# KTH-RPL/HiMo

Hardware: AMD Instinct MI355X
Metric: lidar_frames_per_sec_120k (higher is better)
Workload: dtype f16x2 (two-term split fp16, x = h + l with exact subnormals, on the matrix cores; float32 accumulate; ~22-bit products); 1 GPU; per-frame pipeline: pillarise 3 sweeps (512x512 grid) -> SeFlow++-style encoder/decoder + GRU head (random-init, self-specified: reference network source absent) -> per-point flow -> ego-motion removal + dt0 + flow2compDis -> comp_dis; points_per_frame=120000, sweeps_per_frame=3, parallelism=frames sharded x1, refined_output=False, batches_in_flight=3, matrix_arithmetic=f16x2, samples_per_backbone_launch=16, collectives=none (single process)

## Files before the change

himo_amd/csrc/conv_common.h:

```cpp
#pragma once
#include "himo_common.h"
#include "bf16x3.h"
#include <math.h>

namespace himo {

typedef float floatx16 __attribute__((ext_vector_type(16)));

enum Epilogue {
    kEpiBias = 0,
    kEpiBiasBnGelu = 1,
    kEpiBiasGelu = 2,
    kEpiGruZR = 3,
    kEpiGruQ = 4,
    kEpiBiasRelu = 5,
    kEpiReluMask = 6
};

struct ConvArgs {
    const float* x; int64_t x_batch_stride; int x_pitch;
    const float* w;
    const float* bias; const float* scale; const float* shift;
    float* y; int64_t y_batch_stride; int y_pitch;
    int N, H, W, Cin, Cout;
    int n_inner; int64_t x_outer_stride, y_outer_stride;
    int Ho, Wo;
    const float* aux_in; int aux_in_pitch;
    float* aux_out; int aux_out_pitch;
    int act_flags;
    unsigned* range_seen;
};
enum ActFlags { kActSplitIn = 1, kActSplitOut = 2, kActVecStore = 4, kActAccumulate = 8, kActStuffedIn = 16 };

__device__ inline int64_t image_offset(int img, int n_inner, int64_t batch_stride, int64_t outer_stride) {
    return (int64_t)(img % n_inner) * batch_stride + (int64_t)(img / n_inner) * outer_stride;
}

__device__ inline int xcd_block_id(int bid, int n_blocks) {
    const int per = n_blocks >> 3, rem = n_blocks & 7;
    const int xcd = bid & 7, idx = bid >> 3;
    return xcd * per + (xcd < rem ? xcd : rem) + idx;
}

__device__ inline float gelu_exact(float v) {
    const float hv = 0.5f * v;
    const float t = __builtin_amdgcn_rcpf(fmaf(0.3275911f * 0.70710678118654752440f, fabsf(v), 1.0f));
    float p = fmaf(1.061405429f, t, -1.453152027f);
    p = fmaf(p, t, 1.421413741f);
    p = fmaf(p, t, -0.284496736f);
    p = fmaf(p, t, 0.254829592f);
    const float ex = __builtin_amdgcn_exp2f((v * v) * (-0.5f * 1.44269504088896340736f));
    const float e = fmaf(-(p * t), ex, 1.0f);
    return fmaf(fabsf(hv), e, hv);
}
__device__ inline float gelu_grad_exact(float v) {
    const float t = __builtin_amdgcn_rcpf(fmaf(0.3275911f * 0.70710678118654752440f, fabsf(v), 1.0f));
    float p = fmaf(1.061405429f, t, -1.453152027f);
    p = fmaf(p, t, 1.421413741f);
    p = fmaf(p, t, -0.284496736f);
    p = fmaf(p, t, 0.254829592f);
    const float ex = __builtin_amdgcn_exp2f((v * v) * (-0.5f * 1.44269504088896340736f));
    const float e = fmaf(-(p * t), ex, 1.0f);
    return fmaf(v * 0.39894228040143267794f, ex, 0.5f + copysignf(0.5f * e, v));
}
__device__ inline float sigmoid_f(float v) { return __builtin_amdgcn_rcpf(1.0f + __expf(-v)); }
__device__ inline float tanh_f(float v) {
    const float e = __expf(-2.0f * fabsf(v));
    const float t = (1.0f - e) * __builtin_amdgcn_rcpf(1.0f + e);
    return copysignf(t, v);
}


template <int EPI> constexpr bool kEpiAffine = EPI == kEpiBias || EPI == kEpiBiasBnGelu || EPI == kEpiBiasGelu;
template <int EPI>
__device__ inline void epi_affine(float k, float bias, float sc, float sh, float& A, float& B) {
    if (EPI == kEpiBiasBnGelu) { A = k * sc; B = fmaf(bias, sc, sh); } else { A = k; B = bias; }
}
template <int EPI>
__device__ inline float epi_activate(float acc, float A, float B) {
    const float v = fmaf(acc, A, B);
    return EPI == kEpiBias ? v : gelu_exact(v);
}

template <int EPI>
__device__ inline void epilogue_store(const ConvArgs& a, float* __restrict__ yout, int64_t pix, int co, float v, float sc, float sh) {
    if (EPI == kEpiBias) {
        yout[pix * a.y_pitch + co] = v;
    } else if (EPI == kEpiBiasBnGelu) {
        v = v * sc + sh;
        yout[pix * a.y_pitch + co] = gelu_exact(v);
    } else if (EPI == kEpiBiasGelu) {
        yout[pix * a.y_pitch + co] = gelu_exact(v);
    } else if (EPI == kEpiGruZR) {
        const int half = a.Cout / 2;
        const float g = sigmoid_f(v);
        if (co < half) yout[pix * a.y_pitch + co] = g;
        else a.aux_out[pix * a.aux_out_pitch + (co - half)] = g * a.aux_in[pix * a.aux_in_pitch + (co - half)];
    } else if (EPI == kEpiBiasRelu) {
        yout[pix * a.y_pitch + co] = fmaxf(v, 0.f);
    } else if (EPI == kEpiReluMask) {
        yout[pix * a.y_pitch + co] = a.aux_in[pix * a.aux_in_pitch + co] > 0.f ? v : 0.f;
    } else if (EPI == kEpiGruQ) {
        const float q = tanh_f(v);
        const float z = a.aux_in[pix * a.aux_in_pitch + co];
        const float h = a.aux_out[pix * a.aux_out_pitch + co];
        a.aux_out[pix * a.aux_out_pitch + co] = (1.0f - z) * h + z * q;
    }
}

__device__ inline unsigned split_word(float v, bool odd);
template <int EPI, bool PAIRED>
__device__ inline void split_store(const ConvArgs& a, float* __restrict__ yout, int64_t pix, int co, float v, float sc, float sh) {
    if (EPI == kEpiBiasBnGelu) v = gelu_exact(v * sc + sh);
    else if (EPI == kEpiBiasGelu) v = gelu_exact(v);
    else if (EPI == kEpiBiasRelu) v = fmaxf(v, 0.f);
    if (PAIRED) {
        const bool odd = co & 1;
        unsigned* rec = reinterpret_cast<unsigned*>(yout + pix * a.y_pitch + (co & ~15));
        rec[(odd ? 8 : 0) + ((co & 15) >> 1)] = split_word(v, odd);
        return;
    }
    unsigned h, l;
    split2_rounded(v, h, l);
    {
        unsigned short* rec = reinterpret_cast<unsigned short*>(yout + pix * a.y_pitch + (co & ~15));
        rec[co & 15] = (unsigned short)h;
        rec[16 + (co & 15)] = (unsigned short)l;
    }
}

constexpr float kSplitRangeGuard = 0.015625f;
__device__ inline void note_range(const ConvArgs& a, float v) {
    if (a.range_seen && __ballot(fabsf(v) >= kSplitRangeGuard) != 0ull && (threadIdx.x & 63) == 0 &&
        __hip_atomic_load(a.range_seen, __ATOMIC_RELAXED, __HIP_MEMORY_SCOPE_AGENT) == 0u)
        __hip_atomic_store(a.range_seen, 1u, __ATOMIC_RELAXED, __HIP_MEMORY_SCOPE_AGENT);
}

inline bool vec_store_ok(const ConvArgs& a) {
    return (reinterpret_cast<uintptr_t>(a.y) & 15u) == 0 && !(a.y_pitch & 3) && !(a.y_batch_stride & 3) && !(a.y_outer_stride & 3) && !(a.Cout & 3) &&
           (int64_t)a.Ho * a.Wo * a.y_pitch < ((int64_t)1 << 29);
}

template <bool OSPLIT, bool MASK = false, bool ACC = false>
__device__ inline void store_block_vec(const ConvArgs& a, float* __restrict__ yout, unsigned char* stg, const unsigned (&word)[16],
                                       int lane, int64_t pix0, int n_valid_px, int ch0) {
    const int li = lane & 31, lh = lane >> 5;
    const int widx = OSPLIT ? (li >> 4) * 16 + ((li & 1) ? 8 : 0) + ((li & 15) >> 1) : li;
#pragma unroll
    for (int r = 0; r < 16; ++r) {
        const int px = (r & 3) + 8 * (r >> 2) + 4 * lh;
        const int slot = px ^ ((px >> 2) & 1);
        *reinterpret_cast<unsigned*>(stg + slot * 128 + widx * 4) = word[r];
    }
    __builtin_amdgcn_wave_barrier();
#pragma unroll
    for (int t = 0; t < 4; ++t) {
        const int q = t * 64 + lane;
        const int slot = q >> 3, piece = q & 7;
        const int px = slot ^ ((slot >> 2) & 1);
        uint4 d = *reinterpret_cast<const uint4*>(stg + q * 16);
        const int ch = ch0 + (OSPLIT ? (piece >> 2) * 16 : piece * 4);
        if (px < n_valid_px && ch < a.Cout) {
            if (MASK) {
                const float4 m = *reinterpret_cast<const float4*>(a.aux_in + (pix0 + px) * (int64_t)a.aux_in_pitch + ch0 + piece * 4);
                d.x = m.x > 0.f ? d.x : 0u; d.y = m.y > 0.f ? d.y : 0u; d.z = m.z > 0.f ? d.z : 0u; d.w = m.w > 0.f ? d.w : 0u;
            }
            float* dst = yout + (((unsigned)pix0 + (unsigned)px) * (unsigned)a.y_pitch + (unsigned)(ch0 + piece * 4));
            if (ACC) {
                const float4 o = *reinterpret_cast<const float4*>(dst);
                d.x = __builtin_bit_cast(unsigned, o.x + __builtin_bit_cast(float, d.x)); d.y = __builtin_bit_cast(unsigned, o.y + __builtin_bit_cast(float, d.y));
                d.z = __builtin_bit_cast(unsigned, o.z + __builtin_bit_cast(float, d.z)); d.w = __builtin_bit_cast(unsigned, o.w + __builtin_bit_cast(float, d.w));
            }
            *reinterpret_cast<uint4*>(dst) = d;
        }
    }
    __builtin_amdgcn_wave_barrier();
}

template <int EPI>
__device__ inline float epilogue_value(float v, float sc, float sh) {
    if (EPI == kEpiBiasBnGelu) return gelu_exact(v * sc + sh);
    if (EPI == kEpiBiasGelu) return gelu_exact(v);
    if (EPI == kEpiBiasRelu) return fmaxf(v, 0.f);
    return v;
}
__device__ inline unsigned split_word(float v, bool odd) {
    const unsigned p = split2_packed(v);
    const unsigned q = (unsigned)__builtin_amdgcn_mov_dpp((int)p, 0xB1, 0xF, 0xF, true);
    return __builtin_amdgcn_perm(q, p, odd ? 0x03020706u : 0x05040100u);
}

}
```

himo_amd/csrc/conv_plan.h:

```cpp
#pragma once
#include "conv_common.h"

namespace himo {

enum ConvFamily {
    kConvF32,
    kConvStaged,
    kConvFromL2,
    kConvPresplit3,
    kConvPresplit1
};

struct ConvPlan {
    ConvFamily family;
    ConvArgs args;
    int ks, stride, epi, fmt;
    int bn, mi, ph, nt;
    const void* w_packed;
    dim3 grid;
    const char* prof_name;
};

void launch_conv_f32(const ConvPlan& p, hipStream_t s);
void launch_conv_staged(const ConvPlan& p, hipStream_t s);
void launch_conv_from_l2(const ConvPlan& p, hipStream_t s);
void launch_conv_presplit3(const ConvPlan& p, hipStream_t s);
void launch_conv_presplit1(const ConvPlan& p, hipStream_t s);

inline int64_t blocks_for(const ConvArgs& a, int th, int tw, int bn) {
    const int64_t tiles = th ? (int64_t)((a.Ho + th - 1) / th) * ((a.Wo + tw - 1) / tw) : ((int64_t)a.Ho * a.Wo + tw - 1) / tw;
    return (int64_t)a.N * tiles * ((a.Cout + bn - 1) / bn);
}

inline bool below_2gb(int64_t pixels, int pitch) { return pixels * pitch * 4 < ((int64_t)1 << 31); }

inline const char* conv_prof_name(int ks, int stride, int fmt) {
    static const char* const names[3][4] = {
        {"conv1x1_mfma_kernel", "conv1x1_bf16x3_kernel", "conv1x1_f16x2_kernel", "conv1x1_bf16x2_kernel"},
        {"conv3x3_mfma_kernel", "conv3x3_bf16x3_kernel", "conv3x3_f16x2_kernel", "conv3x3_bf16x2_kernel"},
        {"conv3x3s2_mfma_kernel", "conv3x3s2_bf16x3_kernel", "conv3x3s2_f16x2_kernel", "conv3x3s2_bf16x2_kernel"}};
    return names[ks == 1 ? 0 : stride == 2 ? 2 : 1][fmt < 0 ? 0 : fmt == 1 ? 2 : fmt == 2 ? 3 : 1];
}

inline void plan_staged_tile(ConvPlan& p, int rows_per_mi, int tw, bool keep128, int hint) {
    const ConvArgs& a = p.args;
    auto blocks = [&](int bn, int mi) { return p.ks == 1 ? blocks_for(a, 0, 64 * mi, bn) : blocks_for(a, rows_per_mi * mi, tw, bn); };
    const bool can128 = a.Cout >= 128 && (a.Cout % 128) == 0;
    int bn = can128 ? 128 : 64, mi = 2;
    if (blocks(bn, mi) < 512) mi = 1;
    if (blocks(bn, mi) < 512 && bn == 128 && !keep128) bn = 64;
    const int hb = hint >> 4, hm = hint & 15;
    if ((hb == 64 || (hb == 128 && can128)) && (hm == 1 || hm == 2)) { bn = hb; mi = hm; }
    p.bn = bn; p.mi = mi;
    p.grid = dim3((unsigned)blocks(bn, mi));
}

inline void plan_rows_tile(ConvPlan& p, int ph, int mi, int nt) {
    p.ph = ph; p.mi = mi; p.nt = nt; p.bn = (4 / ph) * 32 * nt;
    p.grid = dim3((unsigned)(p.ks == 1 ? blocks_for(p.args, 0, mi * ph * 32, p.bn) : blocks_for(p.args, mi * ph, 32, p.bn)));
}

inline bool plan_from_l2(ConvPlan& p, int rows_hint) {
    ConvArgs& a = p.args;
    const bool vec = vec_store_ok(a);
    if (p.epi == kEpiGruZR || p.epi == kEpiGruQ) return false;
    if (p.fmt == 2 && (p.epi != kEpiBias || (a.act_flags & ~(kActAccumulate | kActStuffedIn)))) return false;
    if ((a.act_flags & kActAccumulate) && (p.fmt != 2 || !vec)) return false;
    if ((a.act_flags & kActStuffedIn) && (p.fmt != 2 || p.stride != 1)) return false;
    if (!below_2gb((int64_t)a.H * a.W, a.x_pitch)) return false;
    const bool ph_ok = p.stride == 1 && p.fmt != 0;
    const int ph_hint = (ph_ok && (rows_hint == 5 || rows_hint == 6)) ? 2 : (ph_ok && (rows_hint == 9 || rows_hint == 10)) ? 4 : 0;
    if (!ph_hint && rows_hint > 4) return false;
    const bool wide = a.Cout > 64 && ph_hint == 0;
    const int ph = ph_hint ? ph_hint : (wide ? 1 : 2);
    int mi = blocks_for(a, 4 * ph, 32, (4 / ph) * 32) >= 1024 ? 4 : 2;
    if (rows_hint == 4 || rows_hint == 2 || rows_hint == 1) mi = rows_hint;
    if (ph_hint) mi = rows_hint & 3;
    if (p.stride == 2) mi = (rows_hint == 1 || rows_hint == 2) ? rows_hint : (wide ? 2 : 1);
    p.family = kConvFromL2;
    plan_rows_tile(p, ph, mi, 1);
    p.prof_name = conv_prof_name(3, p.stride, p.fmt);
    if (vec && (!(a.act_flags & kActSplitOut) || !(a.Cout & 15))) a.act_flags |= kActVecStore;
    return true;
}

inline int plan_presplit(ConvPlan& p, int rows_hint) {
    ConvArgs& a = p.args;
    if (!below_2gb((int64_t)a.H * a.W, a.x_pitch)) return HIMO_ERR_UNSUPPORTED;
    const bool wide = a.Cout > 64, vec = vec_store_ok(a), pinned = rows_hint == 4 || rows_hint == 2 || rows_hint == 1;
    const int ph = wide ? 1 : 2;
    p.family = p.ks == 1 ? kConvPresplit1 : kConvPresplit3;
    p.prof_name = conv_prof_name(p.ks, p.stride, 1);
    if (vec) a.act_flags |= kActVecStore;
    if (p.ks == 1) {
        int mi = wide ? 4 : 2;
        while (mi > 1 && blocks_for(a, 0, mi * ph * 32, (4 / ph) * 32) < 2048) mi >>= 1;
        if (pinned) mi = rows_hint;
        plan_rows_tile(p, ph, !wide && mi == 4 ? 2 : mi, 1);
    } else if (p.stride == 2) {
        plan_rows_tile(p, ph, wide ? 2 : 1, 1);
    } else if (!wide && rows_hint == 8 && vec) {
        plan_rows_tile(p, 4, 2, 2);
    } else if (wide && rows_hint == 12 && vec) {
        plan_rows_tile(p, a.Cout % 256 == 0 ? 1 : 2, 4, 2);
    } else {
        int mi = blocks_for(a, 4 * ph, 32, (4 / ph) * 32) >= 1024 ? 4 : 2;
        if (pinned) mi = rows_hint;
        plan_rows_tile(p, ph, !wide && mi == 4 ? 2 : mi, 1);
    }
    return HIMO_OK;
}

inline int plan_conv(const himo_conv_desc& d, ConvPlan& p) {
    if (!d.x || !d.w || !d.y) return HIMO_ERR_INVALID_ARGUMENT;
    if (d.n < 1 || d.h < 1 || d.w_in < 1 || d.cin < 1 || d.cout < 1) return HIMO_ERR_INVALID_ARGUMENT;
    if (!(d.ksize == 1 || d.ksize == 3) || !(d.stride == 1 || d.stride == 2)) return HIMO_ERR_UNSUPPORTED;
    if (d.ksize == 1 && d.stride != 1) return HIMO_ERR_UNSUPPORTED;
    if (d.epilogue < 0 || d.epilogue > kEpiReluMask) return HIMO_ERR_INVALID_ARGUMENT;
    if (d.epilogue == kEpiBiasBnGelu && (!d.scale || !d.shift)) return HIMO_ERR_INVALID_ARGUMENT;
    const bool gru = d.epilogue == kEpiGruZR || d.epilogue == kEpiGruQ;
    if (gru && (!d.aux_in || !d.aux_out)) return HIMO_ERR_INVALID_ARGUMENT;
    if (d.epilogue == kEpiReluMask && !d.aux_in) return HIMO_ERR_INVALID_ARGUMENT;
    if ((d.cin & 3) || (d.cout & 3) || (d.x_pitch & 3) || (d.x_batch_stride & 3) || !aligned16(d.x) || !aligned16(d.w))
        return HIMO_ERR_UNSUPPORTED;
    const int n_outer = d.n_outer > 1 ? d.n_outer : 1;
    if (n_outer > 1 && ((d.x_outer_stride & 3) || (d.y_outer_stride & 3))) return HIMO_ERR_INVALID_ARGUMENT;
    p = ConvPlan{};
    p.ks = d.ksize; p.stride = d.stride; p.epi = d.epilogue; p.fmt = d.packed_format; p.w_packed = d.w_packed;
    ConvArgs& a = p.args;
    a.x = d.x; a.x_batch_stride = d.x_batch_stride; a.x_pitch = d.x_pitch;
    a.w = d.w; a.bias = d.bias; a.scale = d.scale; a.shift = d.shift;
    a.y = d.y; a.y_batch_stride = d.y_batch_stride; a.y_pitch = d.y_pitch;
    a.N = d.n * n_outer; a.n_inner = d.n; a.x_outer_stride = d.x_outer_stride; a.y_outer_stride = d.y_outer_stride;
    a.H = d.h; a.W = d.w_in; a.Cin = d.cin; a.Cout = d.cout;
    a.Ho = d.stride == 2 ? (d.h + 1) / 2 : d.h;
    a.Wo = d.stride == 2 ? (d.w_in + 1) / 2 : d.w_in;
    a.aux_in = d.aux_in; a.aux_in_pitch = d.aux_in_pitch; a.aux_out = d.aux_out; a.aux_out_pitch = d.aux_out_pitch;
    a.act_flags = d.act_layout;
    a.range_seen = (d.act_layout & kActSplitOut) ? d.d_range_seen : nullptr;

    const bool gemm_acc = d.act_layout == kActAccumulate && d.w_packed && d.ksize == 1 && d.epilogue == kEpiBias && (d.packed_format == 0 || d.packed_format == 2);
    if (d.act_layout & (kActAccumulate | kActStuffedIn)) {
        if (!gemm_acc && ((d.act_layout & ~(kActAccumulate | kActStuffedIn)) || !d.w_packed || d.packed_format != 2 || d.ksize != 3 ||
                          d.stride != 1 || d.epilogue != kEpiBias))
            return HIMO_ERR_UNSUPPORTED;
        if ((d.act_layout & kActStuffedIn) && ((d.h & 1) || (d.w_in & 1) || !below_2gb((int64_t)(d.h / 2) * (d.w_in / 2), d.x_pitch)))
            return HIMO_ERR_UNSUPPORTED;
    } else if (d.act_layout) {
        if ((d.act_layout & ~(kActSplitIn | kActSplitOut)) || !d.w_packed || d.packed_format != 1) return HIMO_ERR_UNSUPPORTED;
        if (d.ksize == 1 && !(d.act_layout & kActSplitIn)) return HIMO_ERR_UNSUPPORTED;
        if (d.epilogue != kEpiBias && d.epilogue != kEpiBiasBnGelu) return HIMO_ERR_UNSUPPORTED;
        if (((d.act_layout & kActSplitIn) && ((d.cin & 15) || (d.x_pitch & 15))) ||
            ((d.act_layout & kActSplitOut) && ((d.cout & 15) || (d.y_pitch & 15))))
            return HIMO_ERR_UNSUPPORTED;
    }

    const int hint = d.tile_hint, rows_hint = hint & 15;
    const bool l2_hint = hint == 0 || (hint & 0x1000);
    if (!d.w_packed || (d.stride == 2 && (gru || !l2_hint))) {
        p.family = kConvF32;
        plan_staged_tile(p, 4, 16, d.epilogue == kEpiGruZR, hint);
        p.prof_name = conv_prof_name(d.ksize, d.stride, -1);
        if (d.ksize == 1 && vec_store_ok(a) && !(a.Cout & 31) && (d.epilogue != kEpiReluMask || (aligned16(a.aux_in) && !(a.aux_in_pitch & 3))))
            a.act_flags |= kActVecStore;
        return HIMO_OK;
    }
    if (a.act_flags & kActSplitIn) return plan_presplit(p, rows_hint);
    const bool gemm_accumulate = gemm_acc && (int64_t)a.Ho * a.Wo * a.y_pitch < (1ll << 30);
    const bool from_l2 = d.ksize == 3 && l2_hint;
    if (a.act_flags && !gemm_accumulate && !from_l2) return HIMO_ERR_UNSUPPORTED;
    if (from_l2 && plan_from_l2(p, rows_hint)) return HIMO_OK;
    if (d.ksize == 3 && (hint & 0x1000) && rows_hint > 4) return HIMO_ERR_UNSUPPORTED;
    if (d.stride != 1) return HIMO_ERR_UNSUPPORTED;
    if (!below_2gb((int64_t)a.H * a.W, a.x_pitch)) return HIMO_ERR_UNSUPPORTED;
    if (d.packed_format == 2 && (d.ksize != 1 || (d.epilogue != kEpiBias && d.epilogue != kEpiReluMask) || (a.act_flags && !gemm_accumulate)))
        return HIMO_ERR_UNSUPPORTED;
    p.family = kConvStaged;
    plan_staged_tile(p, 2, 32, false, hint);
    p.prof_name = conv_prof_name(d.ksize, 1, d.packed_format);
    return HIMO_OK;
}

}
```

himo_amd/csrc/convsg.hip:

```cpp
#include "conv_plan.h"
#include "bf16x3.h"

namespace himo {

__device__ __attribute__((aligned(64))) unsigned char g_zero_page[64];


__device__ inline void glds16(const void* gsrc, unsigned lds_dst) {
    unsigned keep;
    asm volatile("s_mov_b32 %0, m0\n\ts_mov_b32 m0, %2\n\ts_nop 0\n\tglobal_load_lds_dwordx4 %1, off\n\ts_mov_b32 m0, %0"
                 : "=&s"(keep) : "v"(gsrc), "s"(lds_dst) : "memory");
}

template <int EPI, int PH, int MI, bool OSPLIT, int S, int NT = 1>
__global__ __launch_bounds__(256, NT == 2 ? (MI == 2 ? 3 : 2) : (S == 2 || MI == 4) ? 3 : 4)
void conv3_presplit_kernel(ConvArgs a, const unsigned short* __restrict__ wpk) {
    constexpr int TW = 32, TH = MI * PH, PHt = S == 1 ? TH + 2 : 2 * TH + 1, PWP = S == 1 ? 40 : 80, UPR = PWP / 16;
    constexpr int kRow = PWP * 64, kBuf = (PHt * kRow + 1023) / 1024 * 1024;
    constexpr int kUnits = S == 1 ? (PHt * PWP + 15) / 16 : PHt * UPR, kUPW = (kUnits + 3) / 4;
    constexpr int BN = (4 / PH) * 32 * NT;
    __shared__ __attribute__((aligned(1024))) unsigned char patch[2 * kBuf];

    const int n_tiles_n = (a.Cout + BN - 1) / BN;
    int bid = xcd_block_id(blockIdx.x, gridDim.x);
    const int tn = bid % n_tiles_n; bid /= n_tiles_n;
    const int tx = (a.Wo + TW - 1) / TW, ty = (a.Ho + TH - 1) / TH;
    const int ox0 = (bid % tx) * TW; bid /= tx;
    const int oy0 = (bid % ty) * TH;
    const int img = bid / ty;
    const unsigned char* __restrict__ xin = reinterpret_cast<const unsigned char*>(a.x + image_offset(img, a.n_inner, a.x_batch_stride, a.x_outer_stride));
    const int slabs = a.Cin >> 4;

    const int wave = __builtin_amdgcn_readfirstlane(threadIdx.x >> 6), lane = threadIdx.x & 63;
    const int wp = wave % PH, wc = wave / PH;
    const int li = lane & 31, lh = lane >> 5;
    const int co = tn * BN + wc * NT * 32 + li;
    const bool co_ok = co < a.Cout;
    const int iy0 = oy0 * S - 1, ix0 = ox0 * S - 1;
    const unsigned lds_base = (unsigned)(uintptr_t)(__attribute__((address_space(3))) unsigned char*)(&patch[0]);

    int src[kUPW];
#pragma unroll
    for (int k = 0; k < kUPW; ++k) {
        const int u = wave + 4 * k;
        const int q = u * 16 + (lane >> 2);
        const int row = S == 1 ? q / PWP : u / UPR, px = S == 1 ? q - row * PWP : (u % UPR) * 16 + (lane >> 2);
        const int col = S == 1 ? px : px < 48 ? 2 * px : 2 * (px - 48) + 1;
        const int iy = iy0 + row, ix = ix0 + col;
        const bool ok = u < kUnits && row < PHt && (S == 1 ? px < TW + 2 : px <= 32 || px >= 48) && iy >= 0 && iy < a.H && ix >= 0 && ix < a.W;
        const int sl = (lane & 3) ^ ((px >> 2) & 3);
        src[k] = ok ? (int)((((int64_t)iy * a.W + ix) * a.x_pitch) * 4 + sl * 16) : -1;
    }
    const unsigned char* zero = g_zero_page + (lane & 3) * 16;
    auto stage = [&](int slab, int buf) {
#pragma unroll
        for (int k = 0; k < kUPW; ++k) {
            const int u = wave + 4 * k;
            if (u < kUnits)
                glds16(src[k] >= 0 ? xin + (unsigned)(src[k] + slab * 64) : zero,
                       lds_base + buf * kBuf + (S == 1 ? u * 1024 : ((u / UPR) * PWP + (u % UPR) * 16) * 64));
        }
    };

    floatx16 acc[MI][NT];
#pragma unroll
    for (int mi = 0; mi < MI; ++mi)
#pragma unroll
        for (int nt = 0; nt < NT; ++nt)
#pragma unroll
            for (int r = 0; r < 16; ++r) acc[mi][nt][r] = 0.f;

    const unsigned char* __restrict__ wb = reinterpret_cast<const unsigned char*>(wpk);
    unsigned b_lane[NT];
#pragma unroll
    for (int nt = 0; nt < NT; ++nt) {
        const int c = co + nt * 32 < a.Cout ? co + nt * 32 : a.Cout - 1;
        b_lane[nt] = (unsigned)c * 32u + (unsigned)lh * 16u;
    }
    const unsigned b_plane = (unsigned)a.Cout * 32u, b_block = 2u * b_plane;
    auto load_b = [&](int tap, int slab, uint4 (&b)[NT][2]) {
#pragma unroll
        for (int nt = 0; nt < NT; ++nt) {
            const unsigned off = (unsigned)(tap * slabs + slab) * b_block + b_lane[nt];
            b[nt][0] = *reinterpret_cast<const uint4*>(wb + off);
            b[nt][1] = *reinterpret_cast<const uint4*>(wb + (off + b_plane));
        }
    };

    int rd[3][2];
#pragma unroll
    for (int kx = 0; kx < 3; ++kx) {
        const int p = S == 1 ? li + kx : (kx & 1) * 48 + li + (kx >> 1), f = (p >> 2) & 3;
#pragma unroll
        for (int s = 0; s < 2; ++s) rd[kx][s] = wp * MI * S * kRow + p * 64 + (((2 * s + lh) ^ f) << 4);
    }

    uint4 bq[3][NT][2];
    stage(0, 0);
    load_b(0, 0, bq[0]);
    load_b(1, 0, bq[1]);
    asm volatile("s_waitcnt vmcnt(0)" ::: "memory");
    __syncthreads();

#pragma unroll 1
    for (int slab = 0; slab < slabs; ++slab) {
        const int buf = slab & 1;
        const bool more = slab + 1 < slabs;
        const int nslab = more ? slab + 1 : slab;
        if (more) stage(slab + 1, buf ^ 1);
#pragma unroll 1
        for (int ky = 0; ky < 3; ++ky) {
            const int rowoff = buf * kBuf + ky * kRow;
#pragma unroll
            for (int kx = 0; kx < 3; ++kx) {
                const int tap = ky * 3 + kx;
                const int t2 = tap + 2;
                load_b(t2 < 9 ? t2 : t2 - 9, t2 < 9 ? slab : nslab, bq[(kx + 2) % 3]);
                f16x8 af[MI][2];
#pragma unroll
                for (int s = 0; s < 2; ++s)
#pragma unroll
                    for (int mi = 0; mi < MI; ++mi)
                        af[mi][s] = *reinterpret_cast<const f16x8*>(&patch[rd[kx][s] + rowoff + mi * S * kRow]);
                const uint4 (&bcur)[NT][2] = bq[kx];
#define HIMO_TERM16(SA, SB)                                                                                        \
    _Pragma("unroll") for (int mi = 0; mi < MI; ++mi) _Pragma("unroll") for (int nt = 0; nt < NT; ++nt)              \
        acc[mi][nt] = __builtin_amdgcn_mfma_f32_32x32x16_f16(af[mi][SA], __builtin_bit_cast(f16x8, bcur[nt][SB]), acc[mi][nt], 0, 0, 0);
                { HIMO_TERM16(1, 0) HIMO_TERM16(0, 1) HIMO_TERM16(0, 0) }
#undef HIMO_TERM16
                __builtin_amdgcn_sched_group_barrier(0x020, 2 * NT, 0);
                __builtin_amdgcn_sched_group_barrier(0x100, MI * 2, 0);
                __builtin_amdgcn_sched_group_barrier(0x008, MI * NT * 3, 0);
            }
        }
        if (more) {
            if (NT == 2) asm volatile("s_waitcnt vmcnt(8)" ::: "memory");
            else asm volatile("s_waitcnt vmcnt(4)" ::: "memory");
            __syncthreads();
        }
    }

    float* __restrict__ yout = a.y + image_offset(img, a.n_inner, a.y_batch_stride, a.y_outer_stride);
    float eA[NT], eB[NT];
#pragma unroll
    for (int nt = 0; nt < NT; ++nt) {
        const int c = co + nt * 32 < a.Cout ? co + nt * 32 : a.Cout - 1;
        epi_affine<EPI>(kF16AccScale, a.bias ? a.bias[c] : 0.f, EPI == kEpiBiasBnGelu ? a.scale[c] : 1.f, EPI == kEpiBiasBnGelu ? a.shift[c] : 0.f,
                        eA[nt], eB[nt]);
    }
    if (NT > 1 || (a.act_flags & kActVecStore)) {
        __syncthreads();
        unsigned char* stg = patch + wave * 4096;
        const int n_px = a.Wo - ox0 < 32 ? a.Wo - ox0 : 32;
#pragma unroll
        for (int mi = 0; mi < MI; ++mi) {
            const int oy = oy0 + wp * MI + mi;
#pragma unroll
            for (int nt = 0; nt < NT; ++nt) {
                unsigned word[16];
#pragma unroll
                for (int r = 0; r < 16; ++r) {
                    const float v = epi_activate<EPI>(acc[mi][nt][r], eA[nt], eB[nt]);
                    word[r] = OSPLIT ? split_word(v, li & 1) : __builtin_bit_cast(unsigned, v);
                    if (OSPLIT && mi == 0 && nt == 0 && r == 0)
                        note_range(a, (oy < a.Ho && 4 * lh < n_px && tn * BN + wc * NT * 32 + li < a.Cout) ? v : 0.f);
                }
                store_block_vec<OSPLIT>(a, yout, stg, word, lane, (int64_t)oy * a.Wo + ox0, oy < a.Ho ? n_px : 0, tn * BN + (wc * NT + nt) * 32);
            }
        }
        return;
    }
    if (!co_ok) return;
#pragma unroll
    for (int mi = 0; mi < MI; ++mi) {
        const int oy = oy0 + wp * MI + mi;
#pragma unroll
        for (int r = 0; r < 16; ++r) {
            const int ox = ox0 + (r & 3) + 8 * (r >> 2) + 4 * lh;
            if (oy < a.Ho && ox < a.Wo) {
                const float v = epi_activate<EPI>(acc[mi][0][r], eA[0], eB[0]);
                if (OSPLIT) split_store<kEpiBias, true>(a, yout, (int64_t)oy * a.Wo + ox, co, v, 1.f, 0.f);
                else yout[((int64_t)oy * a.Wo + ox) * a.y_pitch + co] = v;
            }
        }
    }
}

template <int EPI, int PH, int MI, bool OSPLIT>
__global__ __launch_bounds__(256, 4)
void conv1_presplit_kernel(ConvArgs a, const unsigned short* __restrict__ wpk) {
    constexpr int G = 2, TH = MI * PH, BM = TH * 32;
    constexpr int kSeg = 32 * 64, kSlab = TH * kSeg, kBuf = G * kSlab;
    constexpr int kUnits = G * TH * 2, kUPW = (kUnits + 3) / 4;
    constexpr int BN = (4 / PH) * 32;
    __shared__ __attribute__((aligned(1024))) unsigned char patch[2 * kBuf < 16384 ? 16384 : 2 * kBuf];

    const int n_tiles_n = (a.Cout + BN - 1) / BN;
    int bid = xcd_block_id(blockIdx.x, gridDim.x);
    const int tn = bid % n_tiles_n; bid /= n_tiles_n;
    const int64_t rows = (int64_t)a.Ho * a.Wo;
    const int tiles = (int)((rows + BM - 1) / BM);
    const int img = bid / tiles;
    const int64_t row0 = (int64_t)(bid % tiles) * BM;
    const unsigned char* __restrict__ xin = reinterpret_cast<const unsigned char*>(a.x + image_offset(img, a.n_inner, a.x_batch_stride, a.x_outer_stride));
    const int slabs = a.Cin >> 4, steps = (slabs + G - 1) / G;

    const int wave = __builtin_amdgcn_readfirstlane(threadIdx.x >> 6), lane = threadIdx.x & 63;
    const int wp = wave % PH, wc = wave / PH;
    const int li = lane & 31, lh = lane >> 5;
    const int co = tn * BN + wc * 32 + li;
    const bool co_ok = co < a.Cout;
    const unsigned lds_base = (unsigned)(uintptr_t)(__attribute__((address_space(3))) unsigned char*)(&patch[0]);

    int src[kUPW];
#pragma unroll
    for (int k = 0; k < kUPW; ++k) {
        const int u = wave + 4 * k;
        const int g = u / (2 * TH), seg = (u >> 1) % TH, px = (u & 1) * 16 + (lane >> 2);
        const int64_t pix = row0 + seg * 32 + px;
        const int sl = (lane & 3) ^ ((px >> 2) & 3);
        src[k] = (u < kUnits && pix < rows) ? (int)(pix * a.x_pitch * 4 + sl * 16 + g * 64) : -1;
    }
    const unsigned char* zero = g_zero_page + (lane & 3) * 16;
    auto stage = [&](int step, int buf) {
#pragma unroll
        for (int k = 0; k < kUPW; ++k) {
            const int u = wave + 4 * k;
            if (u < kUnits) {
                const int g = u / (2 * TH);
                const bool ok = src[k] >= 0 && step * G + g < slabs;
                glds16(ok ? xin + (unsigned)(src[k] + step * (G * 64)) : zero, lds_base + buf * kBuf + g * kSlab + ((u >> 1) % TH) * kSeg + (u & 1) * 1024);
            }
        }
    };

    floatx16 acc[MI];
#pragma unroll
    for (int mi = 0; mi < MI; ++mi)
#pragma unroll
        for (int r = 0; r < 16; ++r) acc[mi][r] = 0.f;

    const int co_ld = co_ok ? co : a.Cout - 1;
    const unsigned char* __restrict__ wb = reinterpret_cast<const unsigned char*>(wpk);
    const unsigned b_lane = (unsigned)co_ld * 32u + (unsigned)lh * 16u, b_plane = (unsigned)a.Cout * 32u;
    auto load_b = [&](int slab, uint4 (&b)[2]) {
        const unsigned off = (unsigned)slab * (2u * b_plane) + b_lane;
        b[0] = *reinterpret_cast<const uint4*>(wb + off);
        b[1] = *reinterpret_cast<const uint4*>(wb + (off + b_plane));
    };
    int rd[2];
#pragma unroll
    for (int s = 0; s < 2; ++s) rd[s] = wp * MI * kSeg + li * 64 + (((2 * s + lh) ^ ((li >> 2) & 3)) << 4);

    uint4 bq[2][2];
    stage(0, 0);
    load_b(0, bq[0]);
    asm volatile("s_waitcnt vmcnt(0)" ::: "memory");
    __syncthreads();

#pragma unroll 1
    for (int step = 0; step < steps; ++step) {
        const int buf = step & 1;
        const bool more = step + 1 < steps;
        if (more) stage(step + 1, buf ^ 1);
#pragma unroll
        for (int g = 0; g < G; ++g) {
            const int nslab = step * G + g + 1;
            load_b(nslab < slabs ? nslab : slabs - 1, bq[(g + 1) & 1]);
            f16x8 af[MI][2];
#pragma unroll
            for (int s = 0; s < 2; ++s)
#pragma unroll
                for (int mi = 0; mi < MI; ++mi)
                    af[mi][s] = *reinterpret_cast<const f16x8*>(&patch[rd[s] + buf * kBuf + g * kSlab + mi * kSeg]);
            const uint4 (&bcur)[2] = bq[g & 1];
#define HIMO_TERM16(SA, SB)                                                                                        \
    _Pragma("unroll") for (int mi = 0; mi < MI; ++mi)                                                                \
        acc[mi] = __builtin_amdgcn_mfma_f32_32x32x16_f16(af[mi][SA], __builtin_bit_cast(f16x8, bcur[SB]), acc[mi], 0, 0, 0);
            HIMO_TERM16(1, 0) HIMO_TERM16(0, 1) HIMO_TERM16(0, 0)
#undef HIMO_TERM16
        }
        if (more) {
            asm volatile("s_waitcnt vmcnt(2)" ::: "memory");
            __syncthreads();
        }
    }

    float* __restrict__ yout = a.y + image_offset(img, a.n_inner, a.y_batch_stride, a.y_outer_stride);
    float eA, eB;
    epi_affine<EPI>(kF16AccScale, a.bias ? a.bias[co_ld] : 0.f, EPI == kEpiBiasBnGelu ? a.scale[co_ld] : 1.f, EPI == kEpiBiasBnGelu ? a.shift[co_ld] : 0.f, eA, eB);
    if (a.act_flags & kActVecStore) {
        __syncthreads();
        unsigned char* stg = patch + wave * 4096;
#pragma unroll
        for (int mi = 0; mi < MI; ++mi) {
            const int64_t pix0 = row0 + (wp * MI + mi) * 32;
            const int64_t left = rows - pix0;
            unsigned word[16];
#pragma unroll
            for (int r = 0; r < 16; ++r) {
                const float v = epi_activate<EPI>(acc[mi][r], eA, eB);
                word[r] = OSPLIT ? split_word(v, li & 1) : __builtin_bit_cast(unsigned, v);
                if (OSPLIT && mi == 0 && r == 0) note_range(a, (4 * lh < left && tn * BN + wc * 32 + li < a.Cout) ? v : 0.f);
            }
            store_block_vec<OSPLIT>(a, yout, stg, word, lane, pix0, left < 0 ? 0 : left > 32 ? 32 : (int)left, tn * BN + wc * 32);
        }
        return;
    }
    if (!co_ok) return;
#pragma unroll
    for (int mi = 0; mi < MI; ++mi) {
#pragma unroll
        for (int r = 0; r < 16; ++r) {
            const int64_t pix = row0 + (wp * MI + mi) * 32 + (r & 3) + 8 * (r >> 2) + 4 * lh;
            if (pix < rows) {
                const float v = epi_activate<EPI>(acc[mi][r], eA, eB);
                if (OSPLIT) split_store<kEpiBias, true>(a, yout, pix, co, v, 1.f, 0.f);
                else yout[pix * a.y_pitch + co] = v;
            }
        }
    }
}

#define HIMO_SG(KERNEL, E, O, ...) hipLaunchKernelGGL((KERNEL<E, PH, MI, O, ##__VA_ARGS__>), p.grid, dim3(256), 0, s, p.args, (const unsigned short*)p.w_packed)
#define HIMO_SG_EPI(KERNEL, ...)                                                                                                          \
    do {                                                                                                                                  \
        const bool osplit = (p.args.act_flags & kActSplitOut) != 0;                                                                       \
        if (p.epi == kEpiBias) { if (osplit) HIMO_SG(KERNEL, kEpiBias, true, ##__VA_ARGS__); else HIMO_SG(KERNEL, kEpiBias, false, ##__VA_ARGS__); } \
        else { if (osplit) HIMO_SG(KERNEL, kEpiBiasBnGelu, true, ##__VA_ARGS__); else HIMO_SG(KERNEL, kEpiBiasBnGelu, false, ##__VA_ARGS__); }       \
    } while (0)

template <int PH, int MI>
static void launch_sg1(const ConvPlan& p, hipStream_t s) { HIMO_SG_EPI(conv1_presplit_kernel); }

template <int PH, int MI, int S = 1, int NT = 1>
static void launch_sg(const ConvPlan& p, hipStream_t s) { HIMO_SG_EPI(conv3_presplit_kernel, S, NT); }
#undef HIMO_SG_EPI
#undef HIMO_SG

void launch_conv_presplit1(const ConvPlan& p, hipStream_t s) {
    if (p.ph == 1) {
        if (p.mi == 4) launch_sg1<1, 4>(p, s);
        else if (p.mi == 2) launch_sg1<1, 2>(p, s);
        else launch_sg1<1, 1>(p, s);
    } else {
        if (p.mi == 2) launch_sg1<2, 2>(p, s);
        else launch_sg1<2, 1>(p, s);
    }
}

void launch_conv_presplit3(const ConvPlan& p, hipStream_t s) {
    if (p.stride == 2) { if (p.ph == 1) launch_sg<1, 2, 2>(p, s); else launch_sg<2, 1, 2>(p, s); }
    else if (p.nt == 2) {
        if (p.ph == 4) launch_sg<4, 2, 1, 2>(p, s);
        else if (p.ph == 1) launch_sg<1, 4, 1, 2>(p, s);
        else launch_sg<2, 4, 1, 2>(p, s);
    }
    else if (p.ph == 1) {
        if (p.mi == 4) launch_sg<1, 4>(p, s);
        else if (p.mi == 2) launch_sg<1, 2>(p, s);
        else launch_sg<1, 1>(p, s);
    } else {
        if (p.mi == 2) launch_sg<2, 2>(p, s);
        else launch_sg<2, 1>(p, s);
    }
}

}
```

himo_amd/csrc/pillar.hip:

```cpp
#include "himo_common.h"
#include "bf16x3.h"
#include <math.h>
#include <algorithm>
#include <vector>

namespace himo {

struct GridSpec {
    float xmin, ymin, zmin;
    float vx, vy, vz;
    float cx0, cy0, cz0;
    int W, H;
};

struct PillarArgs {
    int64_t n;
    const float* pts; int stride;
    float R[9], t[3];
    GridSpec g;
    const float* pfn_w;
    const float* pfn_scale;
    const float* pfn_shift;
    float* xyz_t;
    int* pid;
    float* offsets;
    float* image; int image_pitch;
    int image_split;
    int* cell_count;
    int* block_sum;
    int* cell_cursor;
    int* order2;
    float4* cell_rec;
    unsigned long long* occ;
};

constexpr int kMaxSweeps = 12;
struct PillarBatch { PillarArgs s[kMaxSweeps]; };

__global__ __launch_bounds__(256) void pillar_clear_kernel(PillarBatch m, int n_vec4) {
    int4* p = reinterpret_cast<int4*>(m.s[blockIdx.y].cell_count);
    for (int i = blockIdx.x * 256 + threadIdx.x; i < n_vec4; i += gridDim.x * 256) p[i] = make_int4(0, 0, 0, 0);
}

__global__ __launch_bounds__(256) void pillar_assign_kernel(PillarBatch m) {
    const PillarArgs& a = m.s[blockIdx.y];
    const int64_t i = (int64_t)blockIdx.x * 256 + threadIdx.x;
    if (i >= a.n) return;
    const float* p = a.pts + i * a.stride;
    const float x = p[0], y = p[1], z = p[2];
    const float tx = ((x * a.R[0] + y * a.R[1]) + z * a.R[2]) + a.t[0];
    const float ty = ((x * a.R[3] + y * a.R[4]) + z * a.R[5]) + a.t[1];
    const float tz = ((x * a.R[6] + y * a.R[7]) + z * a.R[8]) + a.t[2];
    a.xyz_t[i * 3] = tx; a.xyz_t[i * 3 + 1] = ty; a.xyz_t[i * 3 + 2] = tz;
    const float fx = floorf((tx - a.g.xmin) / a.g.vx);
    const float fy = floorf((ty - a.g.ymin) / a.g.vy);
    const float fz = floorf((tz - a.g.zmin) / a.g.vz);
    const bool ok = fx >= 0.f && fx < (float)a.g.W && fy >= 0.f && fy < (float)a.g.H && fz >= 0.f && fz < 1.f;
    int cell = -1;
    if (ok) {
        cell = (int)fy * a.g.W + (int)fx;
        a.order2[i] = atomicAdd(&a.cell_count[cell], 1);
    } else {
        a.offsets[i * 3] = 0.f; a.offsets[i * 3 + 1] = 0.f; a.offsets[i * 3 + 2] = 0.f;
    }
    a.pid[i] = cell;
}

constexpr int kScanBlock = 1024;

__global__ __launch_bounds__(256) void cell_scan_local_kernel(PillarBatch m) {
    int* v = m.s[blockIdx.y].cell_count;
    int* block_sum = m.s[blockIdx.y].block_sum;
    const int n = m.s[blockIdx.y].g.W * m.s[blockIdx.y].g.H;
    __shared__ int wsum[4];
    const int base = blockIdx.x * kScanBlock + threadIdx.x * 4;
    int x[4];
#pragma unroll
    for (int k = 0; k < 4; ++k) x[k] = base + k < n ? v[base + k] : 0;
    const int mine = x[0] + x[1] + x[2] + x[3];
    int incl = mine;
    const int lane = threadIdx.x & 63;
    for (int off = 1; off < 64; off <<= 1) {
        const int y = __shfl_up(incl, off, 64);
        if (lane >= off) incl += y;
    }
    if (lane == 63) wsum[threadIdx.x >> 6] = incl;
    __syncthreads();
    int run = incl - mine;
    for (int w = 0; w < (int)(threadIdx.x >> 6); ++w) run += wsum[w];
#pragma unroll
    for (int k = 0; k < 4; ++k) { if (base + k < n) v[base + k] = run; run += x[k]; }
    if (threadIdx.x == 255) block_sum[blockIdx.x] = run;
}

__global__ __launch_bounds__(1024) void cell_scan_top_kernel(PillarBatch m, int nblk) {
    int* block_sum = m.s[blockIdx.y].block_sum;
    __shared__ int part[1024];
    const int x = (int)threadIdx.x < nblk ? block_sum[threadIdx.x] : 0;
    part[threadIdx.x] = x;
    __syncthreads();
    for (int off = 1; off < 1024; off <<= 1) {
        const int y = threadIdx.x >= off ? part[threadIdx.x - off] : 0;
        __syncthreads();
        part[threadIdx.x] += y;
        __syncthreads();
    }
    if ((int)threadIdx.x < nblk) block_sum[threadIdx.x] = part[threadIdx.x] - x;
    if (threadIdx.x == 1023) block_sum[nblk] = part[1023];
}

__device__ inline int cell_offset(const PillarArgs& a, int cell);

__device__ inline int cell_offset(const PillarArgs& a, int cell) {
    const int n_cells = a.g.W * a.g.H;
    return cell >= n_cells ? a.block_sum[(n_cells + kScanBlock - 1) / kScanBlock]
                           : a.cell_count[cell] + a.block_sum[cell / kScanBlock];
}

__global__ __launch_bounds__(256) void pillar_fill_kernel(PillarBatch m) {
    const PillarArgs& a = m.s[blockIdx.y];
    const int64_t i = (int64_t)blockIdx.x * 256 + threadIdx.x;
    if (i >= a.n) return;
    const int cell = a.pid[i];
    if (cell < 0) return;
    const int at = cell_offset(a, cell) + a.order2[i];
    a.cell_rec[at] = make_float4(a.xyz_t[i * 3], a.xyz_t[i * 3 + 1], a.xyz_t[i * 3 + 2], __int_as_float((int)i));
}

constexpr int kCellsPerBlock = 8;

constexpr int kFeatCells = 64;

__device__ inline float shfl32(float v, int src) { return __shfl(v, src, 32); }
__device__ inline int shfl32(int v, int src) { return __shfl(v, src, 32); }

__global__ __launch_bounds__(256) void pillar_feature_kernel(PillarBatch m) {
    const PillarArgs& a = m.s[blockIdx.y];
    __shared__ int s_beg[kFeatCells + 1];
    __shared__ int s_list[kFeatCells];
    __shared__ int s_nlist;
    const int sub = threadIdx.x >> 5, c = threadIdx.x & 31;
    const int n_cells = a.g.W * a.g.H;
    const int cell0 = blockIdx.x * kFeatCells;
    static_assert(kFeatCells == 64, "one 64-bit occupancy word per block");
    const unsigned long long was = a.occ ? a.occ[blockIdx.x] : ~0ull;
    if (threadIdx.x <= kFeatCells) s_beg[threadIdx.x] = cell_offset(a, min(cell0 + (int)threadIdx.x, n_cells));
    __syncthreads();
    if (threadIdx.x < 64) {
        const int cnt = cell0 + (int)threadIdx.x < n_cells ? s_beg[threadIdx.x + 1] - s_beg[threadIdx.x] : 0;
        const unsigned long long one = __ballot(cnt == 1), many = __ballot(cnt > 1);
        const unsigned long long below = (1ull << threadIdx.x) - 1ull;
        if (cnt == 1) s_list[__popcll(one & below)] = threadIdx.x;
        if (cnt > 1) s_list[__popcll(one) + __popcll(many & below)] = threadIdx.x;
        if (threadIdx.x == 0) { s_nlist = __popcll(one | many); if (a.occ) a.occ[blockIdx.x] = one | many; }
    }
#pragma unroll
    for (int i = 0; i < kFeatCells / 32; ++i) {
        const int lc = i * 32 + (threadIdx.x >> 3);
        if (cell0 + lc < n_cells && s_beg[lc + 1] == s_beg[lc] && ((was >> lc) & 1ull))
            *reinterpret_cast<float4*>(a.image + (int64_t)(cell0 + lc) * a.image_pitch + (threadIdx.x & 7) * 4) = make_float4(0.f, 0.f, 0.f, 0.f);
    }
    __syncthreads();
    const int nlist = s_nlist;
    float w[9];
#pragma unroll
    for (int k = 0; k < 9; ++k) w[k] = a.pfn_w[k * 32 + c];
    const float scale = a.pfn_scale[c], shift = a.pfn_shift[c];

    for (int k = sub; k < nlist; k += kCellsPerBlock) {
        const int lc = s_list[k];
        const int cell = cell0 + lc;
        const int beg = s_beg[lc];
        const int cnt = s_beg[lc + 1] - beg;
        const int iy = cell / a.g.W, ix = cell - iy * a.g.W;
        const float ccx = (float)ix * a.g.vx + a.g.cx0, ccy = (float)iy * a.g.vy + a.g.cy0, ccz = 0.f * a.g.vz + a.g.cz0;
        const float fc = (float)cnt;
        float acc = 0.f;
        if (cnt == 1) {
            const float4 rc = a.cell_rec[beg];
            const int pj = __float_as_int(rc.w);
            const float x = rc.x, y = rc.y, z = rc.z;
            if (c == 0) a.order2[beg] = pj;
            const float f6[3] = {x - ccx, y - ccy, z - ccz};
            float v = x * w[0];
            v = fmaf(y, w[1], v); v = fmaf(z, w[2], v);
            v = fmaf(x - x, w[3], v); v = fmaf(y - y, w[4], v); v = fmaf(z - z, w[5], v);
            v = fmaf(f6[0], w[6], v); v = fmaf(f6[1], w[7], v); v = fmaf(f6[2], w[8], v);
            v = v * scale + shift;
            acc = 0.f + fmaxf(v, 0.f);
            if (c < 3) a.offsets[(int64_t)pj * 3 + c] = f6[c];
        } else if (cnt <= 32) {
            const bool have = c < cnt;
            const float4 rc = a.cell_rec[beg + (have ? c : 0)];
            const int idx = have ? __float_as_int(rc.w) : 0x7fffffff;
            const float ux = rc.x, uy = rc.y, uz = rc.z;
            int rank = 0;
            for (int j = 0; j < cnt; ++j) rank += shfl32(idx, j) < idx;
            int src = 0;
            for (int j = 0; j < cnt; ++j)
                if (shfl32(rank, j) == c) src = j;
            const int sidx = shfl32(idx, src);
            const float px = shfl32(ux, src), py = shfl32(uy, src), pz = shfl32(uz, src);
            if (have) a.order2[beg + c] = sidx;
            float sx = 0.f, sy = 0.f, sz = 0.f;
            for (int j = 0; j < cnt; ++j) { sx += shfl32(px, j); sy += shfl32(py, j); sz += shfl32(pz, j); }
            const float mx = sx / fc, my = sy / fc, mz = sz / fc;
            for (int j = 0; j < cnt; ++j) {
                const float x = shfl32(px, j), y = shfl32(py, j), z = shfl32(pz, j);
                const int pj = shfl32(sidx, j);
                const float f[9] = {x, y, z, x - mx, y - my, z - mz, x - ccx, y - ccy, z - ccz};
                float v = f[0] * w[0];
#pragma unroll
                for (int q = 1; q < 9; ++q) v = fmaf(f[q], w[q], v);
                v = v * scale + shift;
                acc += fmaxf(v, 0.f);
                if (c < 3) a.offsets[(int64_t)pj * 3 + c] = f[6 + c];
            }
        } else {
            for (int j0 = 0; j0 < cnt; j0 += 32) {
                const bool have = j0 + c < cnt;
                const int idx = have ? __float_as_int(a.cell_rec[beg + j0 + c].w) : 0x7fffffff;
                int rank = 0;
                for (int k0 = 0; k0 < cnt; k0 += 32) {
                    const int other = k0 + c < cnt ? __float_as_int(a.cell_rec[beg + k0 + c].w) : 0x7fffffff;
                    const int lim = min(32, cnt - k0);
                    for (int j = 0; j < lim; ++j) rank += shfl32(other, j) < idx;
                }
                if (have) a.order2[beg + rank] = idx;
            }
            __threadfence_block();
            float sx = 0.f, sy = 0.f, sz = 0.f;
            for (int j0 = 0; j0 < cnt; j0 += 32) {
                const bool have = j0 + c < cnt;
                const float* p = a.xyz_t + (int64_t)(have ? a.order2[beg + j0 + c] : 0) * 3;
                const float ux = have ? p[0] : 0.f, uy = have ? p[1] : 0.f, uz = have ? p[2] : 0.f;
                const int lim = min(32, cnt - j0);
                for (int j = 0; j < lim; ++j) { sx += shfl32(ux, j); sy += shfl32(uy, j); sz += shfl32(uz, j); }
            }
            const float mx = sx / fc, my = sy / fc, mz = sz / fc;
            for (int j0 = 0; j0 < cnt; j0 += 32) {
                const bool have = j0 + c < cnt;
                const int pidx = have ? a.order2[beg + j0 + c] : 0;
                const float* p = a.xyz_t + (int64_t)pidx * 3;
                const float ux = have ? p[0] : 0.f, uy = have ? p[1] : 0.f, uz = have ? p[2] : 0.f;
                const int lim = min(32, cnt - j0);
                for (int j = 0; j < lim; ++j) {
                    const float x = shfl32(ux, j), y = shfl32(uy, j), z = shfl32(uz, j);
                    const int pj = shfl32(pidx, j);
                    const float f[9] = {x, y, z, x - mx, y - my, z - mz, x - ccx, y - ccy, z - ccz};
                    float v = f[0] * w[0];
#pragma unroll
                    for (int q = 1; q < 9; ++q) v = fmaf(f[q], w[q], v);
                    v = v * scale + shift;
                    acc += fmaxf(v, 0.f);
                    if (c < 3) a.offsets[(int64_t)pj * 3 + c] = f[6 + c];
                }
            }
        }
        const float feat = acc / fc;
        if (a.image_split) {
            unsigned h, l;
            split2_rounded(feat, h, l);
            const bool odd = c & 1;
            const unsigned recv = (unsigned)__builtin_amdgcn_mov_dpp((int)(odd ? h : l), 0xB1, 0xF, 0xF, true);
            unsigned* rec = reinterpret_cast<unsigned*>(a.image + (int64_t)cell * a.image_pitch + (c & ~15));
            rec[(odd ? 8 : 0) + ((c & 15) >> 1)] = odd ? (recv | (l << 16)) : (h | (recv << 16));
        } else {
            a.image[(int64_t)cell * a.image_pitch + c] = feat;
        }
    }
}

struct PillarBwdArgs {
    GridSpec g;
    const int* cell_count; const int* block_sum; const int* order2;
    const float4* cell_rec;
    const float* xyz_t;
    const float* pfn_w; const float* pfn_scale; const float* pfn_shift;
    const float* d_image; int image_pitch;
    float* partial;
    const float* dhx; int dhx_pitch;
    float* d_b0; int b0_pitch; int group0, group1, n_groups;
    float* d_dec; int dec_pitch;
};

__device__ inline int cell_offset_b(const PillarBwdArgs& a, int cell) {
    const int n_cells = a.g.W * a.g.H;
    return cell >= n_cells ? a.block_sum[(n_cells + kScanBlock - 1) / kScanBlock]
                           : a.cell_count[cell] + a.block_sum[cell / kScanBlock];
}

__global__ __launch_bounds__(1024) void pfn_backward_reduce_kernel(const float* __restrict__ partial, int n_blocks, float* __restrict__ dw,
                                                                   int accumulate) {
    __shared__ float sh[32][32];
    const int c = threadIdx.x & 31, grp = threadIdx.x >> 5, k = blockIdx.x;
    {
        float t[4] = {0.f, 0.f, 0.f, 0.f};
        int b = grp;
        for (; b + 96 < n_blocks; b += 128) {
#pragma unroll
            for (int q = 0; q < 4; ++q) t[q] += partial[(int64_t)(b + 32 * q) * 288 + k * 32 + c];
        }
        for (; b < n_blocks; b += 32) t[0] += partial[(int64_t)b * 288 + k * 32 + c];
        sh[grp][c] = (t[0] + t[1]) + (t[2] + t[3]);
    }
    __syncthreads();
    if (grp == 0) {
        float r = sh[0][c];
#pragma unroll
        for (int g = 1; g < 32; ++g) r += sh[g][c];
        dw[k * 32 + c] = accumulate ? dw[k * 32 + c] + r : r;
    }
}

struct PfnBnArgs {
    PillarBwdArgs b;
    double* partial;
    const float* mean; const float* invstd;
    const float* coef;
};

struct PfnBnBatch { PfnBnArgs s[kMaxSweeps]; };
template <int KIND>
__global__ __launch_bounds__(256) void pfn_walk_kernel(PfnBnBatch m) {
    const PfnBnArgs& p = m.s[blockIdx.y];
    const PillarBwdArgs& a = p.b;
    constexpr int kChunk = 256;
    __shared__ int s_beg[kChunk + 1];
    __shared__ int s_list[kChunk];
    __shared__ int s_wn[4];
    constexpr bool kStats = KIND < 2;
    __shared__ double red_d[kStats ? 2 : 1][kStats ? kCellsPerBlock : 1][32];
    __shared__ float red_f[kStats ? 1 : kCellsPerBlock][kStats ? 1 : 9][32];
    const int sub = threadIdx.x >> 5, c = threadIdx.x & 31, wv = threadIdx.x >> 6, lane = threadIdx.x & 63;
    const int n_cells = a.g.W * a.g.H;
    float w[9], dw[9];
#pragma unroll
    for (int k = 0; k < 9; ++k) { w[k] = a.pfn_w[k * 32 + c]; dw[k] = 0.f; }
    const float scale = KIND ? a.pfn_scale[c] : 0.f, shift = KIND ? a.pfn_shift[c] : 0.f;
    const float mean = (KIND == 1 || KIND == 2) ? p.mean[c] : 0.f, invstd = (KIND == 1 || KIND == 2) ? p.invstd[c] : 0.f;
    const float k2 = KIND == 2 ? p.coef[c] : 0.f, k3 = KIND == 2 ? p.coef[32 + c] : 0.f;
    double s0 = 0.0, s1 = 0.0;
    for (int cell0 = blockIdx.x * kChunk; cell0 < n_cells; cell0 += gridDim.x * kChunk) {
        s_beg[threadIdx.x] = cell_offset_b(a, min(cell0 + (int)threadIdx.x, n_cells));
        if (threadIdx.x == 0) s_beg[kChunk] = cell_offset_b(a, min(cell0 + kChunk, n_cells));
        __syncthreads();
        const int my_cnt = cell0 + (int)threadIdx.x < n_cells ? s_beg[threadIdx.x + 1] - s_beg[threadIdx.x] : 0;
        const unsigned long long occ = __ballot(my_cnt > 0);
        if (lane == 0) s_wn[wv] = __popcll(occ);
        __syncthreads();
        int base = 0, nlist = 0;
#pragma unroll
        for (int u = 0; u < 4; ++u) { if (u < wv) base += s_wn[u]; nlist += s_wn[u]; }
        if (my_cnt > 0) s_list[base + __popcll(occ & ((1ull << lane) - 1ull))] = threadIdx.x;
        __syncthreads();
        for (int k = sub; k < nlist; k += kCellsPerBlock) {
            const int lc = s_list[k];
            const int cell = cell0 + lc;
            const int beg = s_beg[lc], cnt = s_beg[lc + 1] - beg;
            const float fc = (float)cnt;
            const float gi = KIND ? a.d_image[(int64_t)cell * a.image_pitch + c] / fc : 0.f;
            const int iy = cell / a.g.W, ix = cell - iy * a.g.W;
            const float ccx = (float)ix * a.g.vx + a.g.cx0, ccy = (float)iy * a.g.vy + a.g.cy0, ccz = 0.f * a.g.vz + a.g.cz0;
            auto point = [&](float x, float y, float z, float mx, float my, float mz) {
                const float f[9] = {x, y, z, x - mx, y - my, z - mz, x - ccx, y - ccy, z - ccz};
                float v = f[0] * w[0];
#pragma unroll
                for (int q = 1; q < 9; ++q) v = fmaf(f[q], w[q], v);
                if (KIND == 0) {
                    s0 += v; s1 += (double)v * v;
                } else if (KIND == 1) {
                    const float g = (v * scale + shift) > 0.f ? gi : 0.f;
                    s0 += g; s1 += (double)g * ((v - mean) * invstd);
                } else if (KIND == 2) {
                    const float g = (v * scale + shift) > 0.f ? gi : 0.f;
                    const float dy = scale * ((g - k2) - ((v - mean) * invstd) * k3);
#pragma unroll
                    for (int q = 0; q < 9; ++q) dw[q] += f[q] * dy;
                } else {
                    if ((v * scale + shift) > 0.f) {
                        const float g = gi * scale;
#pragma unroll
                        for (int q = 0; q < 9; ++q) dw[q] += f[q] * g;
                    }
                }
            };
            if (cnt == 1) {
                const float4 rc = a.cell_rec[beg];
                point(rc.x, rc.y, rc.z, rc.x, rc.y, rc.z);
                continue;
            }
            float sx = 0.f, sy = 0.f, sz = 0.f;
            float ux = 0.f, uy = 0.f, uz = 0.f;
            for (int j0 = 0; j0 < cnt; j0 += 32) {
                const bool have = j0 + c < cnt;
                const float* q = a.xyz_t + (int64_t)(have ? a.order2[beg + j0 + c] : 0) * 3;
                ux = have ? q[0] : 0.f; uy = have ? q[1] : 0.f; uz = have ? q[2] : 0.f;
                const int lim = min(32, cnt - j0);
                for (int j = 0; j < lim; ++j) { sx += shfl32(ux, j); sy += shfl32(uy, j); sz += shfl32(uz, j); }
            }
            const float mx = sx / fc, my = sy / fc, mz = sz / fc;
            for (int j0 = 0; j0 < cnt; j0 += 32) {
                if (cnt > 32) {
                    const bool have = j0 + c < cnt;
                    const float* q = a.xyz_t + (int64_t)(have ? a.order2[beg + j0 + c] : 0) * 3;
                    ux = have ? q[0] : 0.f; uy = have ? q[1] : 0.f; uz = have ? q[2] : 0.f;
                }
                const int lim = min(32, cnt - j0);
                for (int j = 0; j < lim; ++j) point(shfl32(ux, j), shfl32(uy, j), shfl32(uz, j), mx, my, mz);
            }
        }
        __syncthreads();
    }
    if (kStats) {
        red_d[0][sub][c] = s0; red_d[1][sub][c] = s1;
        __syncthreads();
        if (threadIdx.x < 64) {
            const int which = threadIdx.x >> 5;
            double t = red_d[which][0][c];
#pragma unroll
            for (int q = 1; q < kCellsPerBlock; ++q) t += red_d[which][q][c];
            p.partial[((int64_t)blockIdx.x * 2 + which) * 32 + c] = t;
        }
    } else {
#pragma unroll
        for (int k = 0; k < 9; ++k) red_f[sub][k][c] = dw[k];
        __syncthreads();
        for (int e = threadIdx.x; e < 9 * 32; e += 256) {
            float t = 0.f;
#pragma unroll
            for (int q = 0; q < kCellsPerBlock; ++q) t += red_f[q][e / 32][e % 32];
            a.partial[(int64_t)blockIdx.x * 288 + e] = t;
        }
    }
}

constexpr int kMaxGroup = 16;
struct PfnGroup { const double* partial[kMaxGroup]; const int* block_sum[kMaxGroup]; int n; };

template <int MODE>
__global__ __launch_bounds__(1024) void pfn_bn_finalize_kernel(PfnGroup grp_src, int n_blocks, int n_cells, const float* __restrict__ gamma,
                                                              const float* __restrict__ beta, float eps, float momentum,
                                                              float* __restrict__ running_mean, float* __restrict__ running_var,
                                                              float* __restrict__ out0, float* __restrict__ out1, float* __restrict__ out2,
                                                              float* __restrict__ out3, int accumulate) {
    __shared__ double sh[2][16][32];
    const int c = threadIdx.x & 31, which = (threadIdx.x >> 5) & 1, grp = threadIdx.x >> 6;
    {
        double all = 0.0;
        for (int m = 0; m < grp_src.n; ++m) {
            const double* __restrict__ partial = grp_src.partial[m];
            double t[4] = {0, 0, 0, 0};
            int b = grp;
            for (; b + 48 < n_blocks; b += 64) {
#pragma unroll
                for (int k = 0; k < 4; ++k) t[k] += partial[((int64_t)(b + 16 * k) * 2 + which) * 32 + c];
            }
            for (; b < n_blocks; b += 16) t[0] += partial[((int64_t)b * 2 + which) * 32 + c];
            all += (t[0] + t[1]) + (t[2] + t[3]);
        }
        sh[which][grp][c] = all;
    }
    __syncthreads();
    if (threadIdx.x >= 32) return;
    double count = 0.0;
    for (int m = 0; m < grp_src.n; ++m) count += (double)grp_src.block_sum[m][(n_cells + kScanBlock - 1) / kScanBlock];
    double a0 = 0.0, a1 = 0.0;
#pragma unroll
    for (int g = 0; g < 16; ++g) { a0 += sh[0][g][c]; a1 += sh[1][g][c]; }
    if (MODE == 0) {
        if (count < 1.0) {
            const float sc = gamma[c] / sqrtf((running_var ? running_var[c] : 1.f) + eps);
            out0[c] = sc; out1[c] = beta[c] - (running_mean ? running_mean[c] : 0.f) * sc; out2[c] = 0.f; out3[c] = 0.f;
            return;
        }
        const double mean = a0 / count;
        double var = a1 / count - mean * mean;
        if (var < 0.0) var = 0.0;
        const float invstd = (float)(1.0 / sqrt(var + (double)eps));
        const float sc = gamma[c] * invstd;
        out0[c] = sc;
        out1[c] = beta[c] - (float)mean * sc;
        out2[c] = (float)mean;
        out3[c] = invstd;
        if (running_mean) {
            const double unbiased = count > 1.0 ? var * count / (count - 1.0) : var;
            running_mean[c] = (float)((1.0 - (double)momentum) * (double)running_mean[c] + (double)momentum * mean);
            running_var[c] = (float)((1.0 - (double)momentum) * (double)running_var[c] + (double)momentum * unbiased);
        }
    } else {
        out0[c] = accumulate ? out0[c] + (float)a1 : (float)a1;
        out1[c] = accumulate ? out1[c] + (float)a0 : (float)a0;
        out2[c] = count > 0.0 ? (float)(a0 / count) : 0.f;
        out3[c] = count > 0.0 ? (float)(a1 / count) : 0.f;
    }
}

__global__ __launch_bounds__(256) void head_scatter_kernel(PillarBwdArgs a) {
    const int sub = threadIdx.x >> 5, c = threadIdx.x & 31;
    const int cell = blockIdx.x * kCellsPerBlock + sub;
    if (cell >= a.g.W * a.g.H) return;
    const int beg = cell_offset_b(a, cell);
    const int cnt = cell_offset_b(a, cell + 1) - beg;
    float s0 = 0.f, s1 = 0.f, s2 = 0.f, s3 = 0.f;
    for (int j = 0; j < cnt; ++j) {
        const float* r = a.dhx + (int64_t)a.order2[beg + j] * a.dhx_pitch;
        s0 += r[c]; s1 += r[32 + c]; s2 += r[64 + c]; s3 += r[96 + c];
    }
    float* b0 = a.d_b0 + (int64_t)cell * a.b0_pitch;
    for (int g = 0; g < a.n_groups; ++g) b0[g * 32 + c] = g == a.group0 ? s0 : g == a.group1 ? s1 : 0.f;
    float* dec = a.d_dec + (int64_t)cell * a.dec_pitch;
    dec[c] = s2; dec[32 + c] = s3;
}

}

using namespace himo;

static size_t ws_cells(int cells) { return round_up((size_t)cells * 4, 16); }
static size_t ws_blocks(int cells) { return round_up(((size_t)(cells + kScanBlock - 1) / kScanBlock + 1) * 4, 16); }
static size_t ws_points(int64_t n) { return round_up((size_t)(n > 0 ? n : 1) * 4, 16); }
static size_t pillar_ws(int64_t n, int cells) { return 2 * ws_cells(cells) + ws_blocks(cells) + 2 * ws_points(n) + 3 * ws_points(n); }
static size_t ws_occ(int cells) { return round_up(((size_t)cells + 63) / 64 * 8, 16); }

constexpr int64_t kMaxCells = (int64_t)kScanBlock * 1024;
static int64_t grid_cells(int grid_w, int grid_h) { return (int64_t)grid_w * (int64_t)grid_h; }
static int grid_status(int grid_w, int grid_h) {
    if (grid_w < 1 || grid_h < 1) return HIMO_ERR_INVALID_ARGUMENT;
    return grid_cells(grid_w, grid_h) > kMaxCells ? HIMO_ERR_UNSUPPORTED : HIMO_OK;
}

extern "C" size_t himo_pillar_workspace_bytes(int64_t max_points, int grid_w, int grid_h) {
    if (max_points < 0 || max_points > 0x7fffffff || grid_status(grid_w, grid_h) != HIMO_OK) return 0;
    const int cells = (int)grid_cells(grid_w, grid_h);
    return pillar_ws(max_points, cells) + 64 + ws_occ(cells);
}

extern "C" int himo_pillar_occupancy_reset(void* d_workspace, size_t workspace_bytes, int grid_w, int grid_h, void* stream) {
    if (!d_workspace || grid_w < 1 || grid_h < 1) return HIMO_ERR_INVALID_ARGUMENT;
    if (grid_status(grid_w, grid_h) != HIMO_OK) return HIMO_ERR_UNSUPPORTED;
    const int cells = (int)grid_cells(grid_w, grid_h);
    if (workspace_bytes < ws_occ(cells)) return HIMO_ERR_INVALID_ARGUMENT;
    const size_t nb = ws_occ(cells);
    HIMO_HIP(hipMemsetAsync(reinterpret_cast<char*>(d_workspace) + (workspace_bytes - nb), 0xFF, nb, (hipStream_t)stream));
    return HIMO_OK;
}

static int pillar_args(PillarArgs& a, int64_t n, const float* d_pts, int pc_stride, const float* h_transform, const float* h_range,
                       const float* h_voxel, const float* h_centre_offset, int grid_w, int grid_h, const float* d_pfn_weight,
                       const float* d_pfn_scale, const float* d_pfn_shift, float* d_xyz_t, int32_t* d_pid, float* d_offsets,
                       float* d_image, int image_pitch, void* d_workspace, size_t workspace_bytes, bool incremental = false) {
    if (n < 0 || pc_stride < 3 || grid_w < 1 || grid_h < 1 || !h_transform || !h_range || !h_voxel || !h_centre_offset)
        return HIMO_ERR_INVALID_ARGUMENT;
    if (!d_pfn_weight || !d_pfn_scale || !d_pfn_shift || !d_image || !d_workspace) return HIMO_ERR_INVALID_ARGUMENT;
    if (n > 0 && (!d_pts || !d_xyz_t || !d_pid || !d_offsets)) return HIMO_ERR_INVALID_ARGUMENT;
    if (n > 0x7fffffff || image_pitch < 32) return HIMO_ERR_UNSUPPORTED;
    if ((image_pitch & 3) || (reinterpret_cast<uintptr_t>(d_image) & 15)) return HIMO_ERR_UNSUPPORTED;
    if (grid_cells(grid_w, grid_h) > kMaxCells) return HIMO_ERR_UNSUPPORTED;
    const int cells = (int)grid_cells(grid_w, grid_h);
    if (workspace_bytes < pillar_ws(n, cells) || !aligned16(d_workspace)) return HIMO_ERR_WORKSPACE;
    if (incremental && ((workspace_bytes & 15) || workspace_bytes < pillar_ws(n, cells) + ws_occ(cells))) return HIMO_ERR_WORKSPACE;
    a = PillarArgs{};
    a.n = n; a.pts = d_pts; a.stride = pc_stride;
    for (int i = 0; i < 9; ++i) a.R[i] = h_transform[(i / 3) * 4 + (i % 3)];
    for (int i = 0; i < 3; ++i) a.t[i] = h_transform[i * 4 + 3];
    a.g.xmin = h_range[0]; a.g.ymin = h_range[1]; a.g.zmin = h_range[2];
    a.g.vx = h_voxel[0]; a.g.vy = h_voxel[1]; a.g.vz = h_voxel[2];
    a.g.cx0 = h_centre_offset[0]; a.g.cy0 = h_centre_offset[1]; a.g.cz0 = h_centre_offset[2];
    a.g.W = grid_w; a.g.H = grid_h;
    a.pfn_w = d_pfn_weight; a.pfn_scale = d_pfn_scale; a.pfn_shift = d_pfn_shift;
    a.xyz_t = d_xyz_t; a.pid = d_pid; a.offsets = d_offsets; a.image = d_image; a.image_pitch = image_pitch;
    char* ws = reinterpret_cast<char*>(d_workspace);
    a.cell_count = reinterpret_cast<int*>(ws);
    a.cell_cursor = reinterpret_cast<int*>(ws + ws_cells(cells));
    a.block_sum = reinterpret_cast<int*>(ws + 2 * ws_cells(cells));
    a.cell_rec = reinterpret_cast<float4*>(ws + 2 * ws_cells(cells) + ws_blocks(cells));
    a.order2 = reinterpret_cast<int*>(ws + 2 * ws_cells(cells) + ws_blocks(cells) + 4 * ws_points(n));
    if (incremental) a.occ = reinterpret_cast<unsigned long long*>(ws + (workspace_bytes - ws_occ(cells)));
    return HIMO_OK;
}

static int sweeps_status(int n_sweeps, const himo_sweep* h_sweeps, int image_pitch, int image_split, bool check_shared) {
    if (n_sweeps < 1 || n_sweeps > kMaxSweeps || !h_sweeps) return HIMO_ERR_INVALID_ARGUMENT;
    if (image_split && (image_pitch & 15)) return HIMO_ERR_INVALID_ARGUMENT;
    for (int i = 0; i < n_sweeps; ++i) {
        if (image_split && (reinterpret_cast<uintptr_t>(h_sweeps[i].d_image) & 63)) return HIMO_ERR_INVALID_ARGUMENT;
        for (int j = 0; check_shared && j < i; ++j)
            if (h_sweeps[j].d_workspace == h_sweeps[i].d_workspace) return HIMO_ERR_INVALID_ARGUMENT;
    }
    return HIMO_OK;
}

static int pillar_launch(const PillarBatch& m, int count, hipStream_t s) {
    const int cells = m.s[0].g.W * m.s[0].g.H;
    const int nblk = (cells + kScanBlock - 1) / kScanBlock;
    int64_t nmax = 0;
    for (int i = 0; i < count; ++i)
        if (m.s[i].n > nmax) nmax = m.s[i].n;
    {
        const int n_vec4 = (int)(ws_cells(cells) / 16);
        hipLaunchKernelGGL(pillar_clear_kernel, dim3(std::min((n_vec4 + 255) / 256, 512), count), dim3(256), 0, s, m, n_vec4);
    }
    HIMO_LAUNCH_CHECK("pillar_clear_kernel");
    const unsigned pblocks = (unsigned)((nmax + 255) / 256);
    if (nmax > 0) {
        ProfScope ps("pillar_assign_kernel", s);
        hipLaunchKernelGGL(pillar_assign_kernel, dim3(pblocks, count), dim3(256), 0, s, m);
    }
    HIMO_LAUNCH_CHECK("pillar_assign_kernel");
    {
        ProfScope ps("cell_scan_kernels", s);
        hipLaunchKernelGGL(cell_scan_local_kernel, dim3(nblk, count), dim3(256), 0, s, m);
        hipLaunchKernelGGL(cell_scan_top_kernel, dim3(1, count), dim3(1024), 0, s, m, nblk);
    }
    HIMO_LAUNCH_CHECK("cell_scan_kernels");
    if (nmax > 0) {
        ProfScope ps("pillar_fill_kernel", s);
        hipLaunchKernelGGL(pillar_fill_kernel, dim3(pblocks, count), dim3(256), 0, s, m);
    }
    HIMO_LAUNCH_CHECK("pillar_fill_kernel");
    {
        ProfScope ps("pillar_feature_kernel", s);
        hipLaunchKernelGGL(pillar_feature_kernel, dim3((cells + kFeatCells - 1) / kFeatCells, count), dim3(256), 0, s, m);
    }
    HIMO_LAUNCH_CHECK("pillar_feature_kernel");
    return HIMO_OK;
}

extern "C" int himo_pillarize(int64_t n, const float* d_pts, int pc_stride, const float* h_transform,
                              const float* h_range, const float* h_voxel, const float* h_centre_offset,
                              int grid_w, int grid_h,
                              const float* d_pfn_weight, const float* d_pfn_scale, const float* d_pfn_shift,
                              float* d_xyz_t, int32_t* d_pid, float* d_offsets, float* d_image, int image_pitch,
                              void* d_workspace, size_t workspace_bytes, void* stream) {
    PillarBatch m{};
    const int st = pillar_args(m.s[0], n, d_pts, pc_stride, h_transform, h_range, h_voxel, h_centre_offset, grid_w, grid_h, d_pfn_weight,
                               d_pfn_scale, d_pfn_shift, d_xyz_t, d_pid, d_offsets, d_image, image_pitch, d_workspace, workspace_bytes);
    if (st != HIMO_OK) return st;
    return pillar_launch(m, 1, (hipStream_t)stream);
}

extern "C" int himo_pillarize_multi(int n_sweeps, const himo_sweep* h_sweeps, const float* h_range, const float* h_voxel,
                                    const float* h_centre_offset, int grid_w, int grid_h, const float* d_pfn_weight,
                                    const float* d_pfn_scale, const float* d_pfn_shift, int image_pitch, size_t workspace_bytes,
                                    void* stream) {
    return himo_pillarize_multi_ex(n_sweeps, h_sweeps, h_range, h_voxel, h_centre_offset, grid_w, grid_h, d_pfn_weight, d_pfn_scale,
                                   d_pfn_shift, image_pitch, workspace_bytes, 0, stream);
}

extern "C" int himo_pillarize_multi_ex(int n_sweeps, const himo_sweep* h_sweeps, const float* h_range, const float* h_voxel,
                                       const float* h_centre_offset, int grid_w, int grid_h, const float* d_pfn_weight,
                                       const float* d_pfn_scale, const float* d_pfn_shift, int image_pitch, size_t workspace_bytes,
                                       int image_split, void* stream) {
    const bool incremental = (image_split & 2) != 0;
    image_split &= 1;
    const int st0 = sweeps_status(n_sweeps, h_sweeps, image_pitch, image_split, true);
    if (st0 != HIMO_OK) return st0;
    PillarBatch m{};
    for (int i = 0; i < n_sweeps; ++i) {
        const himo_sweep& w = h_sweeps[i];
        const int st = pillar_args(m.s[i], w.n, w.d_pts, w.pc_stride, w.transform, h_range, h_voxel, h_centre_offset, grid_w, grid_h,
                                   d_pfn_weight, d_pfn_scale, d_pfn_shift, w.d_xyz_t, w.d_pid, w.d_offsets, w.d_image, image_pitch,
                                   w.d_workspace, workspace_bytes, incremental);
        if (st != HIMO_OK) return st;
        m.s[i].image_split = image_split ? 1 : 0;
    }
    return pillar_launch(m, n_sweeps, (hipStream_t)stream);
}

static void carve_bwd(PillarBwdArgs& a, int64_t n, int cells, void* d_workspace) {
    char* ws = reinterpret_cast<char*>(d_workspace);
    a.cell_count = reinterpret_cast<const int*>(ws);
    a.block_sum = reinterpret_cast<const int*>(ws + 2 * ws_cells(cells));
    a.cell_rec = reinterpret_cast<const float4*>(ws + 2 * ws_cells(cells) + ws_blocks(cells));
    a.order2 = reinterpret_cast<const int*>(ws + 2 * ws_cells(cells) + ws_blocks(cells) + 4 * ws_points(n));
}

constexpr int kPfnBwdBlocks = 1024;

extern "C" size_t himo_pfn_backward_workspace_bytes(void) { return (size_t)kPfnBwdBlocks * 288 * 4 + 64; }

extern "C" int himo_pfn_backward(int64_t n, const float* h_voxel, const float* h_centre_offset, int grid_w, int grid_h,
                                 const float* d_pfn_weight, const float* d_pfn_scale, const float* d_pfn_shift,
                                 const float* d_xyz_t, const void* d_pillar_workspace, const float* d_dimage, int image_pitch,
                                 float* d_dweight, unsigned flags, void* d_workspace, size_t workspace_bytes, void* stream) {
    if (n < 0 || !h_voxel || !h_centre_offset || grid_w < 1 || grid_h < 1 || !d_pfn_weight || !d_pfn_scale || !d_pfn_shift ||
        !d_pillar_workspace || !d_dimage || !d_dweight || !d_workspace || image_pitch < 32)
        return HIMO_ERR_INVALID_ARGUMENT;
    if (n > 0 && !d_xyz_t) return HIMO_ERR_INVALID_ARGUMENT;
    if (n > 0x7fffffff || grid_status(grid_w, grid_h) != HIMO_OK) return HIMO_ERR_UNSUPPORTED;
    if (workspace_bytes < himo_pfn_backward_workspace_bytes()) return HIMO_ERR_WORKSPACE;
    PillarBwdArgs a{};
    a.g.vx = h_voxel[0]; a.g.vy = h_voxel[1]; a.g.vz = h_voxel[2];
    a.g.cx0 = h_centre_offset[0]; a.g.cy0 = h_centre_offset[1]; a.g.cz0 = h_centre_offset[2];
    a.g.W = grid_w; a.g.H = grid_h;
    carve_bwd(a, n, grid_w * grid_h, const_cast<void*>(d_pillar_workspace));
    a.xyz_t = d_xyz_t; a.pfn_w = d_pfn_weight; a.pfn_scale = d_pfn_scale; a.pfn_shift = d_pfn_shift;
    a.d_image = d_dimage; a.image_pitch = image_pitch;
    a.partial = reinterpret_cast<float*>(d_workspace);
    hipStream_t s = (hipStream_t)stream;
    {
        ProfScope ps("pfn_backward_kernel", s);
        PfnBnBatch m{};
        m.s[0].b = a;
        hipLaunchKernelGGL(pfn_walk_kernel<3>, dim3(kPfnBwdBlocks), dim3(256), 0, s, m);
    }
    hipLaunchKernelGGL(pfn_backward_reduce_kernel, dim3(9), dim3(1024), 0, s, a.partial, kPfnBwdBlocks, d_dweight, (flags & 1u) ? 1 : 0);
    HIMO_LAUNCH_CHECK("pfn_backward kernels");
    return HIMO_OK;
}

extern "C" size_t himo_pfn_bn_workspace_bytes(void) {
    return round_up((size_t)kPfnBwdBlocks * 288 * 4, 64) + (size_t)kPfnBwdBlocks * 2 * 32 * sizeof(double) + 64 * sizeof(float) + 64;
}

static int pfn_bn_args(PfnBnArgs& p, int64_t n, const float* h_voxel, const float* h_centre_offset, int grid_w, int grid_h,
                       const float* d_pfn_weight, const float* d_xyz_t, const void* d_pillar_workspace, void* d_workspace,
                       size_t workspace_bytes) {
    if (n < 0 || !h_voxel || !h_centre_offset || grid_w < 1 || grid_h < 1 || !d_pfn_weight || !d_pillar_workspace || !d_workspace)
        return HIMO_ERR_INVALID_ARGUMENT;
    if (n > 0 && !d_xyz_t) return HIMO_ERR_INVALID_ARGUMENT;
    if (n > 0x7fffffff || grid_status(grid_w, grid_h) != HIMO_OK) return HIMO_ERR_UNSUPPORTED;
    if (workspace_bytes < himo_pfn_bn_workspace_bytes() || !aligned16(d_workspace)) return HIMO_ERR_WORKSPACE;
    p = PfnBnArgs{};
    PillarBwdArgs& a = p.b;
    a.g.vx = h_voxel[0]; a.g.vy = h_voxel[1]; a.g.vz = h_voxel[2];
    a.g.cx0 = h_centre_offset[0]; a.g.cy0 = h_centre_offset[1]; a.g.cz0 = h_centre_offset[2];
    a.g.W = grid_w; a.g.H = grid_h;
    carve_bwd(a, n, grid_w * grid_h, const_cast<void*>(d_pillar_workspace));
    a.xyz_t = d_xyz_t; a.pfn_w = d_pfn_weight;
    a.partial = reinterpret_cast<float*>(d_workspace);
    p.partial = reinterpret_cast<double*>(reinterpret_cast<char*>(d_workspace) + round_up((size_t)kPfnBwdBlocks * 288 * 4, 64));
    return HIMO_OK;
}

extern "C" int himo_pfn_bn_stats_groups(int n_sweeps, int n_groups, const int64_t* h_n, const float* const* h_xyz_t,
                                        const void* const* h_pillar_workspace, const float* h_voxel, const float* h_centre_offset, int grid_w,
                                        int grid_h, const float* d_pfn_weight, const float* d_gamma, const float* d_beta, float eps,
                                        float momentum, float* d_running_mean, float* d_running_var, float* d_scale, float* d_shift,
                                        float* d_mean, float* d_invstd, void* d_workspace, size_t workspace_bytes, void* stream) {
    if (n_sweeps < 1 || n_groups < 1 || n_sweeps % n_groups || n_sweeps / n_groups > kMaxGroup || !h_n || !h_xyz_t || !h_pillar_workspace)
        return HIMO_ERR_INVALID_ARGUMENT;
    if (!d_gamma || !d_beta || !d_scale || !d_shift || !d_mean || !d_invstd || (d_running_mean == nullptr) != (d_running_var == nullptr))
        return HIMO_ERR_INVALID_ARGUMENT;
    if (grid_w < 1 || grid_h < 1) return HIMO_ERR_INVALID_ARGUMENT;
    if (n_groups > kMaxSweeps * kMaxGroup || grid_status(grid_w, grid_h) != HIMO_OK) return HIMO_ERR_UNSUPPORTED;
    const size_t one = himo_pfn_bn_workspace_bytes();
    if (workspace_bytes < one * n_sweeps) return HIMO_ERR_WORKSPACE;
    std::vector<PfnBnArgs> args((size_t)n_sweeps);
    PfnGroup groups[kMaxSweeps * kMaxGroup];
    for (int g = 0; g < n_groups; ++g) groups[g].n = 0;
    for (int i = 0; i < n_sweeps; ++i) {
        const int st = pfn_bn_args(args[i], h_n[i], h_voxel, h_centre_offset, grid_w, grid_h, d_pfn_weight, h_xyz_t[i], h_pillar_workspace[i],
                                   reinterpret_cast<char*>(d_workspace) + one * i, one);
        if (st != HIMO_OK) return st;
        PfnGroup& G = groups[i % n_groups];
        G.partial[G.n] = args[i].partial; G.block_sum[G.n] = args[i].b.block_sum; ++G.n;
    }
    hipStream_t s = (hipStream_t)stream;
    ProfScope ps("pfn_bn_stats_kernel", s);
    for (int lo = 0; lo < n_sweeps; lo += kMaxSweeps) {
        const int cnt = n_sweeps - lo < kMaxSweeps ? n_sweeps - lo : kMaxSweeps;
        PfnBnBatch m{};
        for (int j = 0; j < cnt; ++j) m.s[j] = args[lo + j];
        hipLaunchKernelGGL(pfn_walk_kernel<0>, dim3(kPfnBwdBlocks, cnt), dim3(256), 0, s, m);
    }
    for (int g = 0; g < n_groups; ++g)
        hipLaunchKernelGGL(pfn_bn_finalize_kernel<0>, dim3(1), dim3(1024), 0, s, groups[g], kPfnBwdBlocks, grid_w * grid_h, d_gamma, d_beta, eps,
                           momentum, d_running_mean, d_running_var, d_scale + 32 * g, d_shift + 32 * g, d_mean + 32 * g, d_invstd + 32 * g, 0);
    HIMO_LAUNCH_CHECK("pfn_bn_stats kernels");
    return HIMO_OK;
}

extern "C" int himo_pfn_bn_stats_multi(int n_sweeps, const int64_t* h_n, const float* const* h_xyz_t, const void* const* h_pillar_workspace,
                                       const float* h_voxel, const float* h_centre_offset, int grid_w, int grid_h,
                                       const float* d_pfn_weight, const float* d_gamma, const float* d_beta, float eps, float momentum,
                                       float* d_running_mean, float* d_running_var, float* d_scale, float* d_shift, float* d_mean,
                                       float* d_invstd, void* d_workspace, size_t workspace_bytes, void* stream) {
    if (n_sweeps > kMaxSweeps) return HIMO_ERR_INVALID_ARGUMENT;
    return himo_pfn_bn_stats_groups(n_sweeps, n_sweeps, h_n, h_xyz_t, h_pillar_workspace, h_voxel, h_centre_offset, grid_w, grid_h, d_pfn_weight,
                                    d_gamma, d_beta, eps, momentum, d_running_mean, d_running_var, d_scale, d_shift, d_mean, d_invstd,
                                    d_workspace, workspace_bytes, stream);
}

extern "C" int himo_pfn_bn_stats(int64_t n, const float* h_voxel, const float* h_centre_offset, int grid_w, int grid_h,
                                 const float* d_pfn_weight, const float* d_xyz_t, const void* d_pillar_workspace, const float* d_gamma,
                                 const float* d_beta, float eps, float momentum, float* d_running_mean, float* d_running_var,
                                 float* d_scale, float* d_shift, float* d_mean, float* d_invstd, void* d_workspace, size_t workspace_bytes,
                                 void* stream) {
    return himo_pfn_bn_stats_multi(1, &n, &d_xyz_t, &d_pillar_workspace, h_voxel, h_centre_offset, grid_w, grid_h, d_pfn_weight, d_gamma,
                                   d_beta, eps, momentum, d_running_mean, d_running_var, d_scale, d_shift, d_mean, d_invstd, d_workspace,
                                   workspace_bytes, stream);
}

extern "C" int himo_pillar_features_multi(int n_sweeps, const himo_sweep* h_sweeps, const float* h_range, const float* h_voxel,
                                          const float* h_centre_offset, int grid_w, int grid_h, const float* d_pfn_weight,
                                          const float* d_scale, const float* d_shift, int image_pitch, size_t workspace_bytes,
                                          int image_split, void* stream) {
    const bool incremental = (image_split & 2) != 0;
    image_split &= 1;
    if (!d_scale || !d_shift) return HIMO_ERR_INVALID_ARGUMENT;
    const int st0 = sweeps_status(n_sweeps, h_sweeps, image_pitch, image_split, false);
    if (st0 != HIMO_OK) return st0;
    PillarBatch m{};
    for (int i = 0; i < n_sweeps; ++i) {
        const himo_sweep& w = h_sweeps[i];
        const int st = pillar_args(m.s[i], w.n, w.d_pts, w.pc_stride, w.transform, h_range, h_voxel, h_centre_offset, grid_w, grid_h,
                                   d_pfn_weight, d_scale + 32 * i, d_shift + 32 * i, w.d_xyz_t, w.d_pid, w.d_offsets, w.d_image, image_pitch,
                                   w.d_workspace, workspace_bytes, incremental);
        if (st != HIMO_OK) return st;
        m.s[i].image_split = image_split ? 1 : 0;
    }
    hipStream_t s = (hipStream_t)stream;
    const int cells = grid_w * grid_h;
    {
        ProfScope ps("pillar_feature_kernel", s);
        hipLaunchKernelGGL(pillar_feature_kernel, dim3((cells + kFeatCells - 1) / kFeatCells, n_sweeps), dim3(256), 0, s, m);
    }
    HIMO_LAUNCH_CHECK("pillar_feature_kernel");
    return HIMO_OK;
}

extern "C" int himo_pfn_backward_bn_groups(int n_sweeps, int n_groups, const int64_t* h_n, const float* const* h_xyz_t,
                                           const void* const* h_pillar_workspace, const float* const* h_dimage, int image_pitch,
                                           const float* h_voxel, const float* h_centre_offset, int grid_w, int grid_h, const float* d_pfn_weight,
                                           const float* d_scale, const float* d_shift, const float* d_mean, const float* d_invstd,
                                           float* d_dweight, float* d_dgamma, float* d_dbeta, unsigned flags, void* d_workspace,
                                           size_t workspace_bytes, void* stream) {
    if (n_sweeps < 1 || n_groups < 1 || n_sweeps % n_groups || n_sweeps / n_groups > kMaxGroup || n_groups > kMaxSweeps * kMaxGroup ||
        n_sweeps > kMaxSweeps * kMaxGroup || !h_n || !h_xyz_t || !h_pillar_workspace || !h_dimage)
        return HIMO_ERR_INVALID_ARGUMENT;
    if (!d_scale || !d_shift || !d_mean || !d_invstd || !d_dweight || !d_dgamma || !d_dbeta || image_pitch < 32) return HIMO_ERR_INVALID_ARGUMENT;
    if (grid_w < 1 || grid_h < 1) return HIMO_ERR_INVALID_ARGUMENT;
    if (grid_status(grid_w, grid_h) != HIMO_OK) return HIMO_ERR_UNSUPPORTED;
    const size_t one = himo_pfn_bn_workspace_bytes();
    if (workspace_bytes < one * n_sweeps) return HIMO_ERR_WORKSPACE;
    static thread_local PfnBnArgs args[kMaxSweeps * kMaxGroup];
    PfnGroup groups[kMaxSweeps * kMaxGroup];
    for (int g = 0; g < n_groups; ++g) groups[g].n = 0;
    for (int i = 0; i < n_sweeps; ++i) {
        if (!h_dimage[i]) return HIMO_ERR_INVALID_ARGUMENT;
        PfnBnArgs& p = args[i];
        const int st = pfn_bn_args(p, h_n[i], h_voxel, h_centre_offset, grid_w, grid_h, d_pfn_weight, h_xyz_t[i], h_pillar_workspace[i],
                                   reinterpret_cast<char*>(d_workspace) + one * i, one);
        if (st != HIMO_OK) return st;
        const int g = i % n_groups;
        p.b.pfn_scale = d_scale + 32 * g; p.b.pfn_shift = d_shift + 32 * g; p.b.d_image = h_dimage[i]; p.b.image_pitch = image_pitch;
        p.mean = d_mean + 32 * g; p.invstd = d_invstd + 32 * g;
        p.coef = i < n_groups ? reinterpret_cast<float*>(p.partial + (size_t)kPfnBwdBlocks * 2 * 32) : args[g].coef;
        PfnGroup& G = groups[g];
        G.partial[G.n] = p.partial; G.block_sum[G.n] = p.b.block_sum; ++G.n;
    }
    hipStream_t s = (hipStream_t)stream;
    ProfScope ps("pfn_backward_kernel", s);
    auto walk = [&](auto kernel) {
        for (int lo = 0; lo < n_sweeps; lo += kMaxSweeps) {
            const int cnt = n_sweeps - lo < kMaxSweeps ? n_sweeps - lo : kMaxSweeps;
            PfnBnBatch m{};
            for (int j = 0; j < cnt; ++j) m.s[j] = args[lo + j];
            hipLaunchKernelGGL(kernel, dim3(kPfnBwdBlocks, cnt), dim3(256), 0, s, m);
        }
    };
    walk(pfn_walk_kernel<1>);
    for (int g = 0; g < n_groups; ++g) {
        float* coef = const_cast<float*>(args[g].coef);
        hipLaunchKernelGGL(pfn_bn_finalize_kernel<1>, dim3(1), dim3(1024), 0, s, groups[g], kPfnBwdBlocks, grid_w * grid_h, (const float*)nullptr,
                           (const float*)nullptr, 0.f, 0.f, (float*)nullptr, (float*)nullptr, d_dgamma, d_dbeta, coef, coef + 32,
                           (g > 0 || (flags & 1u)) ? 1 : 0);
    }
    walk(pfn_walk_kernel<2>);
    for (int i = 0; i < n_sweeps; ++i)
        hipLaunchKernelGGL(pfn_backward_reduce_kernel, dim3(9), dim3(1024), 0, s, args[i].b.partial, kPfnBwdBlocks, d_dweight,
                           (i > 0 || (flags & 1u)) ? 1 : 0);
    HIMO_LAUNCH_CHECK("pfn_backward_bn kernels");
    return HIMO_OK;
}

extern "C" int himo_pfn_backward_bn_multi(int n_sweeps, const int64_t* h_n, const float* const* h_xyz_t, const void* const* h_pillar_workspace,
                                          const float* const* h_dimage, int image_pitch, const float* h_voxel, const float* h_centre_offset,
                                          int grid_w, int grid_h, const float* d_pfn_weight, const float* d_scale, const float* d_shift,
                                          const float* d_mean, const float* d_invstd, float* d_dweight, float* d_dgamma, float* d_dbeta,
                                          unsigned flags, void* d_workspace, size_t workspace_bytes, void* stream) {
    if (n_sweeps > kMaxSweeps) return HIMO_ERR_INVALID_ARGUMENT;
    return himo_pfn_backward_bn_groups(n_sweeps, n_sweeps, h_n, h_xyz_t, h_pillar_workspace, h_dimage, image_pitch, h_voxel, h_centre_offset,
                                       grid_w, grid_h, d_pfn_weight, d_scale, d_shift, d_mean, d_invstd, d_dweight, d_dgamma, d_dbeta, flags,
                                       d_workspace, workspace_bytes, stream);
}

extern "C" int himo_pfn_backward_bn(int64_t n, const float* h_voxel, const float* h_centre_offset, int grid_w, int grid_h,
                                    const float* d_pfn_weight, const float* d_scale, const float* d_shift, const float* d_mean,
                                    const float* d_invstd, const float* d_xyz_t, const void* d_pillar_workspace, const float* d_dimage,
                                    int image_pitch, float* d_dweight, float* d_dgamma, float* d_dbeta, unsigned flags, void* d_workspace,
                                    size_t workspace_bytes, void* stream) {
    return himo_pfn_backward_bn_multi(1, &n, &d_xyz_t, &d_pillar_workspace, &d_dimage, image_pitch, h_voxel, h_centre_offset, grid_w, grid_h,
                                      d_pfn_weight, d_scale, d_shift, d_mean, d_invstd, d_dweight, d_dgamma, d_dbeta, flags, d_workspace,
                                      workspace_bytes, stream);
}

extern "C" int himo_head_scatter(int64_t n, int grid_w, int grid_h, const void* d_pillar_workspace, const float* d_dhx, int dhx_pitch,
                                 float* d_db0, int b0_pitch, int group0, int group1, int n_groups, float* d_ddec, int dec_pitch,
                                 void* stream) {
    if (n < 0 || grid_w < 1 || grid_h < 1 || !d_pillar_workspace || !d_db0 || !d_ddec || dhx_pitch < 128 || n_groups < 1 ||
        b0_pitch < 32 * n_groups || dec_pitch < 64 || (n > 0 && !d_dhx))
        return HIMO_ERR_INVALID_ARGUMENT;
    if (group0 < 0 || group0 >= n_groups || group1 < 0 || group1 >= n_groups || group0 == group1) return HIMO_ERR_INVALID_ARGUMENT;
    if (n > 0x7fffffff || grid_status(grid_w, grid_h) != HIMO_OK) return HIMO_ERR_UNSUPPORTED;
    PillarBwdArgs a{};
    a.g.W = grid_w; a.g.H = grid_h;
    carve_bwd(a, n, grid_w * grid_h, const_cast<void*>(d_pillar_workspace));
    a.dhx = d_dhx; a.dhx_pitch = dhx_pitch; a.d_b0 = d_db0; a.b0_pitch = b0_pitch; a.group0 = group0; a.group1 = group1;
    a.n_groups = n_groups; a.d_dec = d_ddec; a.dec_pitch = dec_pitch;
    hipStream_t s = (hipStream_t)stream;
    ProfScope ps("head_scatter_kernel", s);
    hipLaunchKernelGGL(head_scatter_kernel, dim3((grid_w * grid_h + kCellsPerBlock - 1) / kCellsPerBlock), dim3(256), 0, s, a);
    HIMO_LAUNCH_CHECK("head_scatter_kernel");
    return HIMO_OK;
}
```

himo_amd/pipeline.py:

```python
from __future__ import annotations

from dataclasses import dataclass

import numpy as np
import torch

from . import _lib
from .compdis import CompDisEngine, FrameBatch
from .seflow.model import SeFlowNet


@dataclass
class Sample:
    pch1: torch.Tensor
    pc0: torch.Tensor
    pc1: torch.Tensor
    pose_h1: np.ndarray
    pose0: np.ndarray
    pose1: np.ndarray
    lidar_dt: torch.Tensor
    scene_id: str = ""
    timestamp: int = 0

    @classmethod
    def from_frames(cls, fh: dict, f0: dict, f1: dict | None = None, device=None):
        dev = device if device is not None else _lib.require_gpu()
        up = lambda a: torch.from_numpy(np.ascontiguousarray(a, dtype=np.float32)).to(dev)
        pc1 = f1["pc0"] if f1 is not None else f0["pc1"]
        return cls(up(fh["pc0"]), up(f0["pc0"]), up(pc1), np.asarray(fh["pose0"], np.float64), np.asarray(f0["pose0"], np.float64),
                   np.asarray(f0["pose1"], np.float64), up(f0["lidar_dt"]), f0.get("scene_id", ""), int(f0.get("timestamp", 0)))


class HiMoPipeline:
    def __init__(self, net: SeFlowNet | None = None, device=None, max_points: int = 140_000, max_batch: int = 8,
                 precision: str = "auto", params: dict | None = None):
        self.device = device if device is not None else _lib.require_gpu()
        self.auto = net is None and precision == "auto"
        self._net_args = dict(params=params, device=self.device, max_points=max_points, max_batch=max_batch)
        self.net = net if net is not None else SeFlowNet(precision="f16x2" if self.auto else precision, **self._net_args)
        self.compdis = CompDisEngine(device=self.device)
        self._batch = None
        self._bufs, self._turn = {}, 0
        self._finite = None

    def _upload_small(self, host_bytes: np.ndarray) -> torch.Tensor:
        if not hasattr(self, "_pin_ring"):
            self._pin_ring, self._pin_next = [[torch.empty(1 << 16, dtype=torch.uint8, pin_memory=True), None] for _ in range(4)], 0
        n = host_bytes.size
        slot = self._pin_ring[self._pin_next]
        self._pin_next = (self._pin_next + 1) % len(self._pin_ring)
        if slot[0].numel() < n:
            slot[0] = _lib.pinned_empty(n)
        elif slot[1] is not None:
            slot[1].synchronize()
        np.copyto(slot[0].numpy()[:n], host_bytes)
        out = slot[0][:n].to(self.device, non_blocking=True)
        slot[1] = torch.cuda.Event()
        slot[1].record(torch.cuda.current_stream(self.device))
        return out

    def _rows(self, name: str, total: int, width: int | None, dtype=torch.float32) -> torch.Tensor:
        key = (name, width, self._turn)
        buf = self._bufs.get(key)
        if buf is None or buf.shape[0] < total:
            cap = max(total, int(1.25 * buf.shape[0]) if buf is not None else 0)
            buf = torch.empty((cap,) if width is None else (cap, width), dtype=dtype, device=self.device)
            self._bufs[key] = buf
        return buf[:total]

    def _batch_for(self, samples) -> FrameBatch:
        self._turn ^= 1
        counts = [int(s.pc0.shape[0]) for s in samples]
        offsets = np.zeros(len(samples) + 1, dtype=np.int64)
        np.cumsum(counts, out=offsets[1:])
        T, F = int(offsets[-1]), len(samples)
        width = int(samples[0].pc0.shape[1])
        meta = np.concatenate([offsets.view(np.uint8), np.stack([s.pose0 for s in samples]).astype(np.float64).reshape(-1).view(np.uint8),
                               np.stack([s.pose1 for s in samples]).astype(np.float64).reshape(-1).view(np.uint8)])
        meta_dev = self._upload_small(meta)
        o_end, p_len = (F + 1) * 8, F * 128
        pc0, dt = self._rows("pc0", T, width), self._rows("lidar_dt", T, None)
        if F:
            torch.cat([s.pc0 for s in samples], dim=0, out=pc0)
            torch.cat([s.lidar_dt for s in samples], dim=0, out=dt)
        self._batch = FrameBatch(
            offsets_host=offsets, offsets=meta_dev[:o_end].view(torch.int64),
            pose0=meta_dev[o_end:o_end + p_len].view(torch.float64).view(F, 4, 4),
            pose1=meta_dev[o_end + p_len:o_end + 2 * p_len].view(torch.float64).view(F, 4, 4),
            pc0=pc0, lidar_dt=dt, flow=self._rows("flow", T, 3),
            meta=[(s.scene_id, s.timestamp) for s in samples])
        return self._batch

    def _forward(self, samples, outs) -> None:
        mb = self.net.max_batch
        for lo in range(0, len(samples), mb):
            grp = samples[lo:lo + mb]
            self.net.forward_batch([(s.pch1, s.pc0, s.pc1, s.pose_h1, s.pose0, s.pose1) for s in grp], outs[lo:lo + mb])

    def _fall_back(self):
        self.net = SeFlowNet(precision="bf16x3", **self._net_args)

    def _guard_begin(self):
        if self.net.precision == "f16x2":
            if not self.net.fused_head:
                raise RuntimeError("precision='f16x2' needs the fused head: its output stage carries the finite-flow guard")
            self.net.clear_nonfinite()

    def _guard_now(self) -> bool:
        if self.net.precision != "f16x2":
            return True
        self._guard_why = self.net.guard_verdict(self.net.guard.cpu().tolist())
        return self._guard_why is None

    def _guard_later(self):
        if self.net.precision != "f16x2":
            return
        if not hasattr(self, "_flag_ring"):
            self._flag_ring, self._flag_next = [torch.zeros(self.net.guard.numel(), dtype=torch.int32).pin_memory() for _ in range(2)], 0
        host = self._flag_ring[self._flag_next]
        self._flag_next ^= 1
        host.copy_(self.net.guard, non_blocking=True)
        ev = torch.cuda.Event()
        ev.record(torch.cuda.current_stream(self.device))
        self._finite = (host, ev, self.net)

    @staticmethod
    def _guard_error(why: str) -> FloatingPointError:
        if why == "overflow":
            return FloatingPointError("non-finite flow: activations left the fp16 range of precision='f16x2'; "
                                      "use precision='bf16x3' (or 'auto') for these weights")
        return FloatingPointError("a layer's activations stayed below 2^-6, on the absolute floor (2^-25) of precision='f16x2''s "
                                  "two-term fp16 split: the flow may miss 1e-4; use precision='bf16x3' (or 'auto') for these weights")

    def flows(self, samples) -> list:
        _, outs = self._flows_launch(samples)
        return self._flows_check(samples, outs)

    def _flows_launch(self, samples):
        counts = [int(s.pc0.shape[0]) for s in samples]
        flat = torch.empty((sum(counts), 3), dtype=torch.float32, device=self.device)
        outs = list(torch.split(flat, counts)) if counts else []
        self._guard_begin()
        self._forward(samples, outs)
        return flat, outs

    def _flows_check(self, samples, outs):
        if not self._guard_now():
            if not self.auto:
                raise self._guard_error(self._guard_why)
            self._fall_back()
            self._forward(samples, outs)
        return outs

    def sync_check(self):
        if self._finite is not None:
            (host, ev, net), self._finite = self._finite, None
            ev.synchronize()
            why = net.guard_verdict(host.tolist())
            if why is not None:
                raise self._guard_error(why)

    def flow(self, s: Sample, out: torch.Tensor | None = None) -> torch.Tensor:
        return self.net.forward_device(s.pch1, s.pc0, s.pc1, s.pose_h1, s.pose0, s.pose1, out=out)

    def run(self, samples, sensor_dt: float = 0.1, refined: bool = False, copy: bool = False) -> dict:
        batch = self._batch_for(samples)
        o = batch.offsets_host
        self.sync_check()

        outs = [batch.flow[int(o[k]):int(o[k + 1])] for k in range(len(samples))]
        self._guard_begin()
        self._forward(samples, outs)
        if not self.auto:
            self._guard_later()
        elif not self._guard_now():
            self._fall_back()
            self._forward(samples, outs)
        T = batch.total_points
        out = {"comp_dis": self._rows("comp_dis", T, 3)}
        if refined:
            out["refined"] = self._rows("refined", T, 3)
        res = self.compdis.run(batch, sensor_dt=sensor_dt, refined=refined, out=out)
        out = {"flow": batch.flow, "comp_dis": res["comp_dis"], "refined": res.get("refined"), "batch": batch}
        if copy:
            out.update({k: out[k].clone() for k in ("flow", "comp_dis", "refined") if out[k] is not None})
        return out


class OverlappedPipeline:

    def __init__(self, params: dict | None = None, device=None, max_points: int = 140_000, max_batch: int = 8, precision: str = "auto",
                 in_flight: int = 3, nets=None):
        self.device = device if device is not None else _lib.require_gpu()
        if nets is not None:
            self.pipes = [HiMoPipeline(net, device=self.device) for net in nets]
        else:
            self.pipes = [HiMoPipeline(None, device=self.device, max_points=max_points, max_batch=max_batch, precision=precision, params=params)
                          for _ in range(in_flight)]
        for p in self.pipes[1:]:
            if hasattr(p.net, "tiles") and hasattr(self.pipes[0].net, "tiles"):
                p.net.tiles = self.pipes[0].net.tiles
        self.streams = _lib.shared_streams(self.device, "batch", len(self.pipes))
        self._turn = 0

    @property
    def net(self):
        return self.pipes[0].net

    def _next(self):
        i = self._turn
        self._turn = (self._turn + 1) % len(self.pipes)
        st = self.streams[i]
        st.wait_stream(torch.cuda.current_stream(self.device))
        return self.pipes[i], st

    def run(self, samples, **kw) -> dict:
        pipe, st = self._next()
        with torch.cuda.stream(st):
            out = pipe.run(samples, **kw)
            ev = torch.cuda.Event()
            ev.record(st)
        seen = set()
        for smp in samples:
            for t in (smp.pch1, smp.pc0, smp.pc1, smp.lidar_dt):
                if t.is_cuda and t.numel():
                    key = t.untyped_storage().data_ptr()
                    if key not in seen:
                        seen.add(key)
                        t.record_stream(st)
        out["ready"], out["stream"] = ev, st
        return out

    def wait(self, result: dict) -> dict:
        torch.cuda.current_stream(self.device).wait_event(result["ready"])
        return result

    def flows_stream(self, batches):
        pending = []
        for samples in batches:
            pipe, st = self._next()
            with torch.cuda.stream(st):
                flat, outs = pipe._flows_launch(samples)
            pending.append((samples, pipe, st, flat, outs))
            if len(pending) == len(self.pipes):
                done = pending.pop(0)
                yield done[0], self._flows_finish(*done)
        for done in pending:
            yield done[0], self._flows_finish(*done)

    def _flows_finish(self, samples, pipe, st, flat, outs):
        with torch.cuda.stream(st):
            outs = pipe._flows_check(samples, outs)
        cur = torch.cuda.current_stream(self.device)
        cur.wait_stream(st)
        flat.record_stream(cur)
        return outs

    def sync_check(self):
        for p in self.pipes:
            p.sync_check()
```

himo_amd/seflow/model.py:

```python
from __future__ import annotations

import ctypes

import numpy as np
import torch

from .. import _lib
from . import spec

EPI_BIAS, EPI_BIAS_BN_GELU, EPI_BIAS_GELU, EPI_GRU_ZR, EPI_GRU_Q = range(5)


class ConvDesc(ctypes.Structure):
    _fields_ = [("x", ctypes.c_void_p), ("x_batch_stride", ctypes.c_int64), ("x_pitch", ctypes.c_int),
                ("w", ctypes.c_void_p), ("bias", ctypes.c_void_p), ("scale", ctypes.c_void_p), ("shift", ctypes.c_void_p),
                ("y", ctypes.c_void_p), ("y_batch_stride", ctypes.c_int64), ("y_pitch", ctypes.c_int),
                ("n", ctypes.c_int), ("h", ctypes.c_int), ("w_in", ctypes.c_int), ("cin", ctypes.c_int),
                ("cout", ctypes.c_int), ("ksize", ctypes.c_int), ("stride", ctypes.c_int), ("epilogue", ctypes.c_int),
                ("aux_in", ctypes.c_void_p), ("aux_in_pitch", ctypes.c_int),
                ("aux_out", ctypes.c_void_p), ("aux_out_pitch", ctypes.c_int), ("w_packed", ctypes.c_void_p),
                ("tile_hint", ctypes.c_int), ("packed_format", ctypes.c_int),
                ("n_outer", ctypes.c_int), ("x_outer_stride", ctypes.c_int64), ("y_outer_stride", ctypes.c_int64),
                ("act_layout", ctypes.c_int), ("range_seen", ctypes.c_void_p)]


ACT_SPLIT_IN, ACT_SPLIT_OUT = 1, 2
ACT_ACCUMULATE = 8
ACT_STUFFED_2X = 16


_lib.register({
    "himo_pillar_workspace_bytes": (ctypes.c_size_t, [ctypes.c_int64, ctypes.c_int, ctypes.c_int]),
    "himo_pillar_occupancy_reset": (ctypes.c_int, [ctypes.c_void_p, ctypes.c_size_t, ctypes.c_int, ctypes.c_int, ctypes.c_void_p]),
    "himo_pillarize": (ctypes.c_int, [ctypes.c_int64, ctypes.c_void_p, ctypes.c_int, ctypes.POINTER(ctypes.c_float),
                                      ctypes.POINTER(ctypes.c_float), ctypes.POINTER(ctypes.c_float),
                                      ctypes.POINTER(ctypes.c_float), ctypes.c_int, ctypes.c_int,
                                      ctypes.c_void_p, ctypes.c_void_p, ctypes.c_void_p,
                                      ctypes.c_void_p, ctypes.c_void_p, ctypes.c_void_p, ctypes.c_void_p,
                                      ctypes.c_int, ctypes.c_void_p, ctypes.c_size_t, ctypes.c_void_p]),
    "himo_conv2d": (ctypes.c_int, [ctypes.POINTER(ConvDesc), ctypes.c_void_p]),
    "himo_conv_packed_weight_bytes": (ctypes.c_size_t, [ctypes.c_int, ctypes.c_int, ctypes.c_int]),
    "himo_conv_pack_weights": (ctypes.c_int, [ctypes.c_void_p, ctypes.c_int, ctypes.c_int, ctypes.c_int, ctypes.c_void_p,
                                              ctypes.c_void_p]),
    "himo_upsample2x": (ctypes.c_int, [ctypes.c_void_p, ctypes.c_int, ctypes.c_int, ctypes.c_int, ctypes.c_int,
                                       ctypes.c_void_p, ctypes.c_int, ctypes.c_void_p]),
    "himo_upsample2x_batch": (ctypes.c_int, [ctypes.c_int, ctypes.c_void_p, ctypes.c_int64, ctypes.c_int, ctypes.c_int, ctypes.c_int,
                                             ctypes.c_int, ctypes.c_void_p, ctypes.c_int64, ctypes.c_int, ctypes.c_void_p]),
    "himo_upsample2x_batch_ex": (ctypes.c_int, [ctypes.c_int, ctypes.c_void_p, ctypes.c_int64, ctypes.c_int, ctypes.c_int, ctypes.c_int,
                                                ctypes.c_int, ctypes.c_void_p, ctypes.c_int64, ctypes.c_int, ctypes.c_int, ctypes.c_void_p]),
    "himo_conv_pack_weights_ex": (ctypes.c_int, [ctypes.c_void_p, ctypes.c_int, ctypes.c_int, ctypes.c_int, ctypes.c_int, ctypes.c_void_p,
                                                 ctypes.c_void_p]),
    "himo_gru_head": (ctypes.c_int, [ctypes.c_int64] + [ctypes.c_void_p] * 4 + [ctypes.c_int, ctypes.c_void_p, ctypes.c_int]
                      + [ctypes.c_void_p] * 12 + [ctypes.c_int, ctypes.c_void_p, ctypes.c_int, ctypes.c_int, ctypes.c_void_p]),
    "himo_gru_head_batch": (ctypes.c_int, [ctypes.c_int, ctypes.c_void_p, ctypes.c_int, ctypes.c_int] + [ctypes.c_void_p] * 10
                            + [ctypes.c_int, ctypes.c_int, ctypes.c_int, ctypes.c_void_p]),
    "himo_gru_head_batch_folded": (ctypes.c_int, [ctypes.c_int, ctypes.c_void_p, ctypes.c_int, ctypes.c_int] + [ctypes.c_void_p] * 8
                                   + [ctypes.c_int, ctypes.c_int, ctypes.c_int, ctypes.c_void_p]),
    "himo_gru_head_batch_guarded": (ctypes.c_int, [ctypes.c_int, ctypes.c_void_p, ctypes.c_int, ctypes.c_int] + [ctypes.c_void_p] * 10
                                    + [ctypes.c_int, ctypes.c_int, ctypes.c_int, ctypes.c_void_p, ctypes.c_void_p]),
    "himo_clear_u32": (ctypes.c_int, [ctypes.c_void_p, ctypes.c_int, ctypes.c_void_p]),
    "himo_head_gather": (ctypes.c_int, [ctypes.c_int64, ctypes.c_void_p, ctypes.c_void_p, ctypes.c_void_p, ctypes.c_void_p,
                                        ctypes.c_int, ctypes.c_void_p, ctypes.c_int, ctypes.c_void_p, ctypes.c_void_p,
                                        ctypes.c_void_p, ctypes.c_void_p, ctypes.c_int, ctypes.c_void_p]),
    "himo_head_final": (ctypes.c_int, [ctypes.c_int64, ctypes.c_void_p, ctypes.c_int, ctypes.c_void_p, ctypes.c_void_p,
                                       ctypes.c_void_p, ctypes.c_void_p, ctypes.c_void_p, ctypes.c_int, ctypes.c_void_p,
                                       ctypes.c_void_p]),
})


class HimoHeadSample(ctypes.Structure):
    _fields_ = [("n", ctypes.c_int64), ("d_pid", ctypes.c_void_p), ("d_offsets", ctypes.c_void_p), ("d_img0", ctypes.c_void_p),
                ("d_img1", ctypes.c_void_p), ("d_dec", ctypes.c_void_p), ("d_xyz_t", ctypes.c_void_p), ("d_pts", ctypes.c_void_p),
                ("pc_stride", ctypes.c_int), ("d_flow", ctypes.c_void_p)]


class HimoSweep(ctypes.Structure):
    _fields_ = [("n", ctypes.c_int64), ("d_pts", ctypes.c_void_p), ("pc_stride", ctypes.c_int), ("transform", ctypes.c_float * 16),
                ("d_xyz_t", ctypes.c_void_p), ("d_pid", ctypes.c_void_p), ("d_offsets", ctypes.c_void_p), ("d_image", ctypes.c_void_p),
                ("d_workspace", ctypes.c_void_p)]


class HimoOp(ctypes.Structure):
    _fields_ = [("kind", ctypes.c_int), ("conv", ConvDesc),
                ("up_x", ctypes.c_void_p), ("up_x_pitch", ctypes.c_int), ("up_h", ctypes.c_int), ("up_w", ctypes.c_int),
                ("up_c", ctypes.c_int), ("up_y", ctypes.c_void_p), ("up_y_pitch", ctypes.c_int),
                ("up_n", ctypes.c_int), ("up_x_batch_stride", ctypes.c_int64), ("up_y_batch_stride", ctypes.c_int64),
                ("up_out_split", ctypes.c_int)]


_lib.register({
    "himo_pillarize_multi": (ctypes.c_int, [ctypes.c_int, ctypes.c_void_p, ctypes.c_void_p, ctypes.c_void_p, ctypes.c_void_p, ctypes.c_int,
                                            ctypes.c_int, ctypes.c_void_p, ctypes.c_void_p, ctypes.c_void_p, ctypes.c_int, ctypes.c_size_t,
                                            ctypes.c_void_p]),
    "himo_pillarize_multi_ex": (ctypes.c_int, [ctypes.c_int, ctypes.c_void_p, ctypes.c_void_p, ctypes.c_void_p, ctypes.c_void_p, ctypes.c_int,
                                               ctypes.c_int, ctypes.c_void_p, ctypes.c_void_p, ctypes.c_void_p, ctypes.c_int, ctypes.c_size_t,
                                               ctypes.c_int, ctypes.c_void_p]),
    "himo_run_ops": (ctypes.c_int, [ctypes.c_void_p, ctypes.c_int, ctypes.c_uint, ctypes.c_void_p]),
    "himo_ops_release": (None, [ctypes.c_void_p]),
})


def _f32x(values):
    return (ctypes.c_float * len(values))(*[float(v) for v in values])


def fastest_tile_hint(lib, d: "ConvDesc", hints, warmup: int) -> int:
    stream = _lib.stream_handle()
    times = {}
    for _round in range(2):
        for hint in hints:
            d.tile_hint = hint
            if lib.himo_conv2d(ctypes.byref(d), stream) != 0:
                continue
            for _ in range(warmup - 1):
                lib.himo_conv2d(ctypes.byref(d), stream)
            e0, e1 = torch.cuda.Event(enable_timing=True), torch.cuda.Event(enable_timing=True)
            e0.record()
            for _ in range(3):
                lib.himo_conv2d(ctypes.byref(d), stream)
            e1.record()
            e1.synchronize()
            times[hint] = min(times.get(hint, float("inf")), e0.elapsed_time(e1))
    return min(times, key=times.get) if times else 0


class SeFlowNet:

    def __init__(self, params: dict | None = None, device=None, max_points: int = 140_000, seed: int = 0,
                 precision: str = "bf16x3", autotune: bool = True, max_batch: int = 1):
        if precision not in ("bf16x3", "f16x2", "f32"):
            raise ValueError(precision)
        if max_batch < 1:
            raise ValueError("max_batch")
        self.max_batch = max_batch
        self.precision = precision
        self.autotune = autotune
        self.keep_cell_lists = False
        self.fused_head = precision != "f32"
        self._incremental_images = True
        self.use_plan = True
        self.use_graph = True
        self._plans = {}
        self._recording = None
        self._nb = 1
        self.packed_format = 1 if precision == "f16x2" else 0
        self._split_acts = precision == "f16x2"
        self.tiles = {}
        self.lib = _lib.load()
        self.device = device if device is not None else _lib.require_gpu()
        params = spec.init_params(seed) if params is None else params
        shapes = spec.param_shapes()
        for k, shp in shapes.items():
            if k not in params or tuple(params[k].shape) != tuple(shp):
                raise KeyError(f"parameter {k} missing or of wrong shape (want {shp})")
        cpu = {k: torch.from_numpy(np.ascontiguousarray(params[k], dtype=np.float32)) for k in shapes}
        def fold(prefix, eps):
            scale = cpu[f"{prefix}.gamma"] / torch.sqrt(cpu[f"{prefix}.var"] + eps)
            return scale, cpu[f"{prefix}.beta"] - cpu[f"{prefix}.mean"] * scale
        derived = {}
        derived["pfn.scale"], derived["pfn.shift"] = fold("pfn.bn", spec.BN_EPS_PFN)
        for name, *_ in spec.ENCODER:
            derived[f"{name}.scale"], derived[f"{name}.shift"] = fold(f"{name}.bn", spec.BN_EPS)
        self.fold_decoder = True
        for a, b in (("dec1", "dec2"), ("dec2", "dec3")):
            w5, b5 = cpu[f"{a}.u5.weight"].double().numpy(), cpu[f"{a}.u5.bias"].double().numpy()
            w1, b1 = cpu[f"{b}.u1.weight"].double().numpy()[0, 0], cpu[f"{b}.u1.bias"].double().numpy()
            derived[f"{a}.u5>{b}.u1.weight"] = torch.from_numpy(np.ascontiguousarray(w5 @ w1, dtype=np.float32))
            derived[f"{a}.u5>{b}.u1.bias"] = torch.from_numpy(np.ascontiguousarray(b5 @ w1 + b1, dtype=np.float32))
        derived["head.gru.zr.weight"] = torch.cat([cpu["head.gru.z.weight"], cpu["head.gru.r.weight"]], dim=1).contiguous()
        derived["head.gru.zr.bias"] = torch.cat([cpu["head.gru.z.bias"], cpu["head.gru.r.bias"]]).contiguous()
        self.p = {k: v.to(self.device) for k, v in {**cpu, **derived}.items()}
        self.packed = {}
        if precision != "f32":
            for k, v in self.p.items():
                if k.endswith(".weight") and k != "pfn.weight" and not k.startswith("head.offset") and k != "head.dec2.weight":
                    w = v if v.dim() == 4 else v.reshape(1, 1, *v.shape)
                    ks, _, cin, cout = w.shape
                    fmt = self.packed_format
                    buf = torch.empty(int(self.lib.himo_conv_packed_weight_bytes(ks, cin, cout)), dtype=torch.uint8, device=self.device)
                    _lib.check(self.lib.himo_conv_pack_weights_ex(w.contiguous().data_ptr(), ks, cin, cout, fmt, buf.data_ptr(),
                                                                  _lib.stream_handle()), "himo_conv_pack_weights_ex")
                    self.packed[k] = buf

        self.fold_head = precision != "f32"
        if self.fold_head:
            w_off, b_off = cpu["head.offset.weight"].double().numpy(), cpu["head.offset.bias"].double().numpy()
            for name in ("head.gru.zr", "head.gru.q", "head.dec1"):
                wfull = (derived if name.endswith("zr") else cpu)[f"{name}.weight"].double().numpy()
                wh, wx = wfull[:spec.HIDDEN], wfull[spec.HIDDEN:]
                folded = np.concatenate([wh, w_off @ wx, (b_off @ wx)[None], np.zeros((12, wfull.shape[1]))], axis=0)
                wdev = torch.from_numpy(np.ascontiguousarray(folded, dtype=np.float32)).to(self.device)
                buf = torch.empty(int(self.lib.himo_conv_packed_weight_bytes(1, 144, wdev.shape[1])), dtype=torch.uint8, device=self.device)
                _lib.check(self.lib.himo_conv_pack_weights_ex(wdev.data_ptr(), 1, 144, wdev.shape[1], self.packed_format, buf.data_ptr(),
                                                              _lib.stream_handle()), "himo_conv_pack_weights_ex")
                torch.cuda.synchronize(self.device)
                self.packed[f"{name}.weight.h"] = buf

        H, W = spec.GRID
        F = spec.NUM_FRAMES
        self.H, self.W, self.F = H, W, F
        dev = self.device
        B = self.max_batch
        buf = lambda *shape: torch.empty((B, *shape), dtype=torch.float32, device=dev)
        self._B0 = buf(H * W, 32 * F)
        self.E1 = [buf(F, (H // 2) * (W // 2), 64) for _ in range(2)]
        self.F1 = buf((H // 2) * (W // 2), 64 * F)
        self.E2 = [buf(F, (H // 4) * (W // 4), 128) for _ in range(2)]
        self.F2 = buf((H // 4) * (W // 4), 128 * F)
        self.E3 = [buf(F, (H // 8) * (W // 8), 256) for _ in range(2)]
        self.F3 = buf((H // 8) * (W // 8), 256 * F)
        self.T1 = buf((H // 8) * (W // 8), 256)
        self.CAT1 = buf((H // 4) * (W // 4), 512)
        self.S = [buf((H // 4) * (W // 4), 256) for _ in range(2)]
        self.T2 = buf((H // 4) * (W // 4), 128)
        self.CAT2 = buf((H // 2) * (W // 2), 256)
        self.T = [buf((H // 2) * (W // 2), 128) for _ in range(2)]
        self.T3 = buf((H // 2) * (W // 2), 64)
        self.CAT3 = buf(H * W, 128)
        self.U = [buf(H * W, 64) for _ in range(2)]
        self.DEC = buf(H * W, 64)
        self.max_points = 0
        self._reserve_points(max_points)
        self.guard = torch.zeros(2 + self.MAX_RANGE_SLOTS, dtype=torch.int32, device=dev)
        self.nonfinite = self.guard[:1]
        self._ran_word = self.guard[-1:]
        self._range_slots = {}
        self._range = _f32x(spec.POINT_CLOUD_RANGE[:3])
        self._voxel = _f32x(spec.VOXEL_SIZE)
        r, v = spec.POINT_CLOUD_RANGE, spec.VOXEL_SIZE
        self._centre = _f32x([v[0] / 2 + r[0], v[1] / 2 + r[1], v[2] / 2 + r[2]])

    def _reserve_points(self, n: int):
        if n <= self.max_points:
            return
        dev = self.device
        self.max_points = n
        need = int(self.lib.himo_pillar_workspace_bytes(n, self.W, self.H))
        self._pt = [{"ws_slots": [torch.empty(need + 64, dtype=torch.uint8, device=dev) for _ in range(self.F)],
                     "xyz_t": torch.empty((self.F, n, 3), dtype=torch.float32, device=dev),
                     "pid": torch.empty((self.F, n), dtype=torch.int32, device=dev),
                     "offsets": torch.empty((self.F, n, 3), dtype=torch.float32, device=dev)} for _ in range(self.max_batch)]
        for st in self._pt:
            for ws in st["ws_slots"]:
                _lib.check(self.lib.himo_pillar_occupancy_reset(ws.data_ptr(), ws.numel(), self.W, self.H, _lib.stream_handle()),
                           "himo_pillar_occupancy_reset")
        self._use_sample(0)
        self.hx = torch.empty((n, 192), dtype=torch.float32, device=dev)
        self.rhx = torch.empty((n, 192), dtype=torch.float32, device=dev)
        self.zbuf = torch.empty((n, 128), dtype=torch.float32, device=dev)
        self.y1 = torch.empty((n, 32), dtype=torch.float32, device=dev)

    @property
    def incremental_images(self) -> bool:
        return self._incremental_images

    @incremental_images.setter
    def incremental_images(self, on: bool):
        on = bool(on)
        if on != self._incremental_images:
            self._incremental_images = on
            self.reset_images()

    @property
    def split_acts(self) -> bool:
        return self._split_acts

    @split_acts.setter
    def split_acts(self, on: bool):
        on = bool(on)
        if on != self._split_acts:
            self._split_acts = on
            self.drop_plan()
            self.reset_images()

    @property
    def B0(self):
        return self._B0

    @B0.setter
    def B0(self, buf):
        self._B0 = buf
        self.drop_plan()
        self.reset_images()

    MAX_RANGE_SLOTS = 63

    def clear_nonfinite(self):
        _lib.check(self.lib.himo_clear_u32(self.guard.data_ptr(), self.guard.numel(), _lib.stream_handle()), "himo_clear_u32")

    def _range_word(self, wname: str) -> int:
        k = self._range_slots.setdefault(wname, len(self._range_slots))
        if k >= self.MAX_RANGE_SLOTS:
            raise RuntimeError("more split-output layers than guard words")
        return self.guard.data_ptr() + 4 * (1 + k)

    def guard_verdict(self, words) -> str | None:
        w = [int(v) for v in words]
        if w[0] != 0:
            return "overflow"
        if w[-1] != 0 and any(w[1 + k] == 0 for k in self._range_slots.values()):
            return "underflow"
        return None

    def reset_images(self):
        for st in getattr(self, "_pt", ()):
            for ws in st["ws_slots"]:
                _lib.check(self.lib.himo_pillar_occupancy_reset(ws.data_ptr(), ws.numel(), self.W, self.H, _lib.stream_handle()),
                           "himo_pillar_occupancy_reset")

    def _use_sample(self, i: int):
        st = self._pt[i]
        self._sample = i
        self.ws_slots, self.xyz_t, self.pid, self.offsets = st["ws_slots"], st["xyz_t"], st["pid"], st["offsets"]

    def _conv(self, x, x_bs, x_pitch, wname, y, y_bs, y_pitch, n, h, w, cin, cout, ks, stride, epi, x_off=0, y_off=0,
              scale=None, shift=None, aux_in=None, aux_in_pitch=0, aux_out=None, aux_out_pitch=0, bias=None, batched=True,
              act=0):
        d = ConvDesc()
        d.x = x.data_ptr() + 4 * x_off; d.x_batch_stride = x_bs; d.x_pitch = x_pitch
        if batched and self._nb > 1:
            d.n_outer, d.x_outer_stride, d.y_outer_stride = self._nb, x.stride(0), y.stride(0)
        d.w = self.p[f"{wname}.weight"].data_ptr()
        d.bias = (self.p[f"{wname}.bias"] if bias is None else bias).data_ptr()
        d.scale = None if scale is None else scale.data_ptr()
        d.shift = None if shift is None else shift.data_ptr()
        d.y = y.data_ptr() + 4 * y_off; d.y_batch_stride = y_bs; d.y_pitch = y_pitch
        d.n, d.h, d.w_in, d.cin, d.cout, d.ksize, d.stride, d.epilogue = n, h, w, cin, cout, ks, stride, epi
        d.aux_in = None if aux_in is None else aux_in.data_ptr(); d.aux_in_pitch = aux_in_pitch
        d.aux_out = None if aux_out is None else aux_out.data_ptr(); d.aux_out_pitch = aux_out_pitch
        pk = self.packed.get(f"{wname}.weight")
        d.w_packed = None if pk is None else pk.data_ptr()
        d.packed_format = self.packed_format
        d.act_layout = act if self.split_acts else 0
        if (d.act_layout & ACT_SPLIT_OUT) and self.packed_format == 1 and epi in (EPI_BIAS, EPI_BIAS_BN_GELU):
            d.range_seen = self._range_word(wname)
        key = (n * max(d.n_outer, 1), h, w, cin, cout, ks, stride, epi, pk is not None, d.act_layout)
        if self.autotune and key not in self.tiles:
            self.tiles[key] = self._tune(d)
        d.tile_hint = self.tiles.get(key, 0)
        if self._recording is not None and epi not in (EPI_GRU_ZR, EPI_GRU_Q):
            op = HimoOp(); op.kind = 0; op.conv = d
            self._recording.append(op)
        _lib.check(self.lib.himo_conv2d(ctypes.byref(d), _lib.stream_handle()), f"himo_conv2d({wname})")

    def _tune(self, d: "ConvDesc") -> int:
        if d.epilogue in (EPI_GRU_ZR, EPI_GRU_Q):
            return 0
        cands = [(bn << 4) | mi for bn in (128, 64) if not (bn == 128 and d.cout % 128) for mi in (2, 1)]
        if d.act_layout:
            if d.stride == 2 and (d.act_layout & ACT_SPLIT_IN):
                return 0
            cands = [0x1000 | 4, 0x1000 | 2, 0x1000 | 1] if d.ksize == 1 else []
        if d.w_packed and d.ksize == 3:
            cands += [0x1000 | 4, 0x1000 | 2, 0x1000 | 1] if d.stride == 1 else [0x1000 | 2, 0x1000 | 1]
            if d.stride == 1 and (d.act_layout & ACT_SPLIT_IN) and self.packed_format == 1:
                cands.append(0x1000 | (8 if d.cout <= 64 else 12))
        if len(cands) < 2:
            return cands[0] if cands else 0
        return fastest_tile_hint(self.lib, d, cands, warmup=2)

    def _up(self, x, x_pitch, h, w, c, y, y_pitch, out_split=False):
        nb = self._nb
        osp = 1 if (out_split and self.split_acts) else 0
        if self._recording is not None:
            op = HimoOp(); op.kind = 1
            op.up_x, op.up_x_pitch, op.up_h, op.up_w, op.up_c, op.up_y, op.up_y_pitch = x.data_ptr(), x_pitch, h, w, c, y.data_ptr(), y_pitch
            op.up_n, op.up_x_batch_stride, op.up_y_batch_stride = nb, x.stride(0), y.stride(0)
            op.up_out_split = osp
            self._recording.append(op)
        _lib.check(self.lib.himo_upsample2x_batch_ex(nb, x.data_ptr(), x.stride(0) if nb > 1 else 0, x_pitch, h, w, c, y.data_ptr(),
                                                     y.stride(0) if nb > 1 else 0, y_pitch, osp, _lib.stream_handle()), "himo_upsample2x_batch_ex")

    def backbone(self, n_samples: int = 1):
        if not 1 <= n_samples <= self.max_batch:
            raise ValueError(f"n_samples must be in 1..{self.max_batch}")
        self._nb = n_samples
        if self.packed_format == 1:
            self._ran_word.fill_(1)
        plan = self._plans.get(n_samples)
        if self.use_plan and plan is not None:
            ops, n = plan
            _lib.check(self.lib.himo_run_ops(ctypes.addressof(ops), n, 1 if self.use_graph else 0, _lib.stream_handle()), "himo_run_ops")
            return self.DEC
        self._recording = [] if self.use_plan else None
        self.encoder()
        self.decoder()
        if self._recording is not None:
            rec, self._recording = self._recording, None
            self._plans[n_samples] = ((HimoOp * len(rec))(*rec), len(rec))
        return self.DEC

    def __del__(self):
        try:
            self.drop_plan()
        except Exception:
            pass

    def drop_plan(self):
        for plan in self._plans.values():
            self.lib.himo_ops_release(ctypes.addressof(plan[0]))
        self._plans = {}

    def encoder(self):
        H, W, F = self.H, self.W, self.F
        p = self.p
        stages = [("enc1", 4, 32, 64, H, W, self.E1, self.F1), ("enc2", 6, 64, 128, H // 2, W // 2, self.E2, self.F2),
                  ("enc3", 6, 128, 256, H // 4, W // 4, self.E3, self.F3)]
        src, src_bs, src_pitch = self.B0, 32, 32 * F
        for stage, n_conv, cin, cout, h, w, pingpong, catbuf in stages:
            ho, wo = h // 2, w // 2
            for i in range(n_conv):
                name = f"{stage}.{i}"
                last = i == n_conv - 1
                dst = catbuf if last else pingpong[i % 2]
                dst_bs, dst_pitch = (cout, cout * F) if last else (ho * wo * cout, cout)
                act = ACT_SPLIT_IN | ACT_SPLIT_OUT
                if i == 0:
                    self._conv(src, src_bs, src_pitch, name, dst, dst_bs, dst_pitch, F, h, w, cin, cout, 3, 2,
                               EPI_BIAS_BN_GELU, scale=p[f"{name}.scale"], shift=p[f"{name}.shift"], act=act)
                else:
                    self._conv(src, src_bs, src_pitch, name, dst, dst_bs, dst_pitch, F, ho, wo, cout, cout, 3, 1,
                               EPI_BIAS_BN_GELU, scale=p[f"{name}.scale"], shift=p[f"{name}.shift"], act=act)
                src, src_bs, src_pitch = dst, dst_bs, dst_pitch

    def decoder(self):
        H, W, F = self.H, self.W, self.F
        IN, IO = ACT_SPLIT_IN, ACT_SPLIT_IN | ACT_SPLIT_OUT
        fold = self.fold_decoder
        def block(name, coarse, c_in, ch, cw, tmp, cat, skip, skip_c, lat, out, work, nxt=None):
            if coarse is not None:
                self._conv(coarse, 0, c_in, f"{name}.u1", tmp, 0, lat, 1, 1, ch * cw, c_in, lat, 1, 1, EPI_BIAS, act=IN)
            self._up(tmp, lat, ch, cw, lat, cat, 2 * lat, out_split=True)
            self._conv(skip, 0, skip_c, f"{name}.u3", cat, 0, 2 * lat, 1, 1, 4 * ch * cw, skip_c, lat, 1, 1, EPI_BIAS, y_off=lat, act=IO)
            self._conv(cat, 0, 2 * lat, f"{name}.u4", work[0], 0, out, 1, 2 * ch, 2 * cw, 2 * lat, out, 3, 1, EPI_BIAS, act=IO)
            if fold and nxt is not None:
                nname, ntmp, nlat = nxt
                self._conv(work[0], 0, out, f"{name}.u5>{nname}.u1", ntmp, 0, nlat, 1, 2 * ch, 2 * cw, out, nlat, 3, 1, EPI_BIAS, act=IN)
                return None
            self._conv(work[0], 0, out, f"{name}.u5", work[1], 0, out, 1, 2 * ch, 2 * cw, out, out, 3, 1, EPI_BIAS, act=IO)
            return work[1]
        s = block("dec1", self.F3, 256 * F, H // 8, W // 8, self.T1, self.CAT1, self.F2, 128 * F, 256, 256, self.S, ("dec2", self.T2, 128))
        t = block("dec2", s, 256, H // 4, W // 4, self.T2, self.CAT2, self.F1, 64 * F, 128, 128, self.T, ("dec3", self.T3, 64))
        u = block("dec3", t, 128, H // 2, W // 2, self.T3, self.CAT3, self.B0, 32 * F, 64, 64, self.U)
        self._conv(u, 0, 64, "dec4", self.DEC, 0, 64, 1, H, W, 64, 64, 3, 1, EPI_BIAS, act=IN)
        return self.DEC

    def head(self, pc0: torch.Tensor, slot0: int = 1, slot1: int = 2, out: torch.Tensor | None = None) -> torch.Tensor:
        n = pc0.shape[0]
        p = self.p
        F = self.F
        B0, DEC = self.B0[self._sample], self.DEC[self._sample]
        if self.fused_head:
            flow = out if out is not None else torch.empty((n, 3), dtype=torch.float32, device=self.device)
            if flow.shape != (n, 3) or flow.dtype != torch.float32 or not flow.is_contiguous():
                raise ValueError("out must be a contiguous (N0,3) float32 tensor")
            self.head_batch([pc0], [flow], slot0, slot1, samples=[self._sample])
            return flow
        if self.split_acts:
            raise RuntimeError("the multi-launch head reads float32 pillar images: set split_acts = False (or use the fused head)")
        st = self.lib.himo_head_gather(n, self.pid[slot0].data_ptr(), self.offsets[slot0].data_ptr(),
                                       B0.data_ptr() + 4 * 32 * slot0, B0.data_ptr() + 4 * 32 * slot1, 32 * F,
                                       DEC.data_ptr(), 64, p["head.offset.weight"].data_ptr(),
                                       p["head.offset.bias"].data_ptr(), self.hx.data_ptr(), self.rhx.data_ptr(), 192,
                                       _lib.stream_handle())
        _lib.check(st, "himo_head_gather")
        for _ in range(spec.GRU_ITERS):
            self._conv(self.hx, 0, 192, "head.gru.zr", self.zbuf, 0, 128, 1, 1, n, 192, 256, 1, 1, EPI_GRU_ZR,
                       aux_in=self.hx, aux_in_pitch=192, aux_out=self.rhx, aux_out_pitch=192, batched=False)
            self._conv(self.rhx, 0, 192, "head.gru.q", self.zbuf, 0, 128, 1, 1, n, 192, 128, 1, 1, EPI_GRU_Q,
                       aux_in=self.zbuf, aux_in_pitch=128, aux_out=self.hx, aux_out_pitch=192, batched=False)
        self._conv(self.hx, 0, 192, "head.dec1", self.y1, 0, 32, 1, 1, n, 192, 32, 1, 1, EPI_BIAS_GELU, batched=False)
        flow = out if out is not None else torch.empty((n, 3), dtype=torch.float32, device=self.device)
        if flow.shape != (n, 3) or flow.dtype != torch.float32 or not flow.is_contiguous():
            raise ValueError("out must be a contiguous (N0,3) float32 tensor")
        st = self.lib.himo_head_final(n, self.y1.data_ptr(), 32, p["head.dec2.weight"].data_ptr(),
                                      p["head.dec2.bias"].data_ptr(), self.pid[slot0].data_ptr(),
                                      self.xyz_t[slot0].data_ptr(), pc0.data_ptr(), pc0.shape[1], flow.data_ptr(),
                                      _lib.stream_handle())
        _lib.check(st, "himo_head_final")
        return flow

    def forward(self, pch1, pc0, pc1, pose_h1, pose0, pose1) -> torch.Tensor:
        dev = self.device
        to_dev = lambda a: (a if isinstance(a, torch.Tensor) else torch.from_numpy(np.ascontiguousarray(a, dtype=np.float32))).to(dev, torch.float32).contiguous()
        return self.forward_device(to_dev(pch1), to_dev(pc0), to_dev(pc1), pose_h1, pose0, pose1)

    def forward_device(self, pch1, pc0, pc1, pose_h1, pose0, pose1, out: torch.Tensor | None = None) -> torch.Tensor:
        inv1 = np.linalg.inv(np.asarray(pose1, np.float64))
        T0 = inv1 @ np.asarray(pose0, np.float64)
        Th = inv1 @ np.asarray(pose_h1, np.float64)
        self._use_sample(0)
        self.pillarize_all((pch1, pc0, pc1), (Th, T0, np.eye(4)))
        self.backbone(1)
        return self.head(pc0, out=out)

    def forward_batch(self, samples, outs) -> None:
        if not 1 <= len(samples) <= self.max_batch:
            raise ValueError(f"forward_batch takes 1..{self.max_batch} samples")
        jobs = []
        for k, (pch1, pc0, pc1, pose_h1, pose0, pose1) in enumerate(samples):
            inv1 = np.linalg.inv(np.asarray(pose1, np.float64))
            jobs.append((k, (pch1, pc0, pc1), (inv1 @ np.asarray(pose_h1, np.float64), inv1 @ np.asarray(pose0, np.float64), np.eye(4))))
        self.pillarize_many(jobs)
        self.backbone(len(samples))
        if self.fused_head:
            self.head_batch([smp[1] for smp in samples], outs)
            return
        for k, smp in enumerate(samples):
            self._use_sample(k)
            self.head(smp[1], out=outs[k])

    MAX_HEAD_SAMPLES = 16

    def head_batch(self, pc0s, outs, slot0: int = 1, slot1: int = 2, samples=None) -> None:
        p, pk, F = self.p, self.packed, self.F
        samples = list(range(len(pc0s))) if samples is None else list(samples)
        for lo in range(0, len(pc0s), self.MAX_HEAD_SAMPLES):
            grp = range(lo, min(lo + self.MAX_HEAD_SAMPLES, len(pc0s)))
            arr = (HimoHeadSample * len(grp))()
            for j, i in enumerate(grp):
                k = samples[i]
                pc0, flow, st = pc0s[i], outs[i], self._pt[k]
                n = pc0.shape[0]
                if flow.shape != (n, 3) or flow.dtype != torch.float32 or not flow.is_contiguous():
                    raise ValueError("out must be a contiguous (N0,3) float32 tensor")
                h = arr[j]
                h.n, h.d_pid, h.d_offsets = n, st["pid"][slot0].data_ptr(), st["offsets"][slot0].data_ptr()
                h.d_img0, h.d_img1 = self.B0[k].data_ptr() + 4 * 32 * slot0, self.B0[k].data_ptr() + 4 * 32 * slot1
                h.d_dec, h.d_xyz_t = self.DEC[k].data_ptr(), st["xyz_t"][slot0].data_ptr()
                h.d_pts, h.pc_stride, h.d_flow = pc0.data_ptr(), pc0.shape[1], flow.data_ptr()
            tail = (p["head.dec2.weight"].data_ptr(), p["head.dec2.bias"].data_ptr(),
                    spec.GRU_ITERS, self.packed_format, 1 if self.split_acts else 0, self.nonfinite.data_ptr(), _lib.stream_handle())
            if self.fold_head:
                st = self.lib.himo_gru_head_batch_guarded(len(arr), ctypes.addressof(arr), 32 * F, 64, None, None,
                                                          pk["head.gru.zr.weight.h"].data_ptr(), p["head.gru.zr.bias"].data_ptr(),
                                                          pk["head.gru.q.weight.h"].data_ptr(), p["head.gru.q.bias"].data_ptr(),
                                                          pk["head.dec1.weight.h"].data_ptr(), p["head.dec1.bias"].data_ptr(), *tail)
            else:
                st = self.lib.himo_gru_head_batch_guarded(len(arr), ctypes.addressof(arr), 32 * F, 64,
                                                          p["head.offset.weight"].data_ptr(), p["head.offset.bias"].data_ptr(),
                                                          pk["head.gru.zr.weight"].data_ptr(), p["head.gru.zr.bias"].data_ptr(),
                                                          pk["head.gru.q.weight"].data_ptr(), p["head.gru.q.bias"].data_ptr(),
                                                          pk["head.dec1.weight"].data_ptr(), p["head.dec1.bias"].data_ptr(), *tail)
            _lib.check(st, "himo_gru_head_batch")

    def pillarize_all(self, sweeps, transforms):
        self.pillarize_many([(self._sample, sweeps, transforms)])

    MAX_SWEEPS = 12

    def pillarize_many(self, jobs):
        for _, sweeps, _ in jobs:
            for t in sweeps:
                self._reserve_points(t.shape[0])
        per_call = self.MAX_SWEEPS // self.F
        for lo in range(0, len(jobs), per_call):
            grp = jobs[lo:lo + per_call]
            arr = (HimoSweep * (len(grp) * self.F))()
            for j, (sample, sweeps, transforms) in enumerate(grp):
                st = self._pt[sample]
                for slot, (pts, T) in enumerate(zip(sweeps, transforms)):
                    w = arr[j * self.F + slot]
                    w.n, w.d_pts, w.pc_stride = pts.shape[0], pts.data_ptr(), pts.shape[1]
                    w.transform = _f32x(np.asarray(T, dtype=np.float32).reshape(-1))
                    w.d_xyz_t, w.d_pid, w.d_offsets = st["xyz_t"][slot].data_ptr(), st["pid"][slot].data_ptr(), st["offsets"][slot].data_ptr()
                    w.d_image = self.B0[sample].data_ptr() + 4 * 32 * slot
                    w.d_workspace = st["ws_slots"][slot].data_ptr()
            status = self.lib.himo_pillarize_multi_ex(len(arr), ctypes.addressof(arr), self._range, self._voxel, self._centre, self.W, self.H,
                                                      self.p["pfn.weight"].data_ptr(), self.p["pfn.scale"].data_ptr(),
                                                      self.p["pfn.shift"].data_ptr(), 32 * self.F, self._pt[0]["ws_slots"][0].numel(),
                                                      (1 if self.split_acts else 0) | (2 if self.incremental_images else 0), _lib.stream_handle())
            _lib.check(status, "himo_pillarize_multi_ex")

    def pillar_features(self, sweeps, transforms, scale: torch.Tensor, shift: torch.Tensor):
        arr = (HimoSweep * self.F)()
        st = self._pt[self._sample]
        for slot, (pts, T) in enumerate(zip(sweeps, transforms)):
            w = arr[slot]
            w.n, w.d_pts, w.pc_stride = pts.shape[0], pts.data_ptr(), pts.shape[1]
            w.transform = _f32x(np.asarray(T, dtype=np.float32).reshape(-1))
            w.d_xyz_t, w.d_pid, w.d_offsets = st["xyz_t"][slot].data_ptr(), st["pid"][slot].data_ptr(), st["offsets"][slot].data_ptr()
            w.d_image = self.B0[self._sample].data_ptr() + 4 * 32 * slot
            w.d_workspace = st["ws_slots"][slot].data_ptr()
        status = self.lib.himo_pillar_features_multi(self.F, ctypes.addressof(arr), self._range, self._voxel, self._centre, self.W, self.H,
                                                     self.p["pfn.weight"].data_ptr(), scale.data_ptr(), shift.data_ptr(), 32 * self.F,
                                                     st["ws_slots"][0].numel(),
                                                     (1 if self.split_acts else 0) | (2 if self.incremental_images else 0), _lib.stream_handle())
        _lib.check(status, "himo_pillar_features_multi")

    def pillarize_into(self, slot: int, pts: torch.Tensor, transform):
        n = pts.shape[0]
        self._reserve_points(n)
        arr = (HimoSweep * 1)()
        w = arr[0]
        w.n, w.d_pts, w.pc_stride = n, pts.data_ptr(), pts.shape[1]
        w.transform = _f32x(np.asarray(transform, dtype=np.float32).reshape(-1))
        w.d_xyz_t, w.d_pid, w.d_offsets = self.xyz_t[slot].data_ptr(), self.pid[slot].data_ptr(), self.offsets[slot].data_ptr()
        w.d_image = self.B0[self._sample].data_ptr() + 4 * 32 * slot
        w.d_workspace = self.ws_slots[slot].data_ptr()
        st = self.lib.himo_pillarize_multi_ex(1, ctypes.addressof(arr), self._range, self._voxel, self._centre, self.W, self.H,
                                              self.p["pfn.weight"].data_ptr(), self.p["pfn.scale"].data_ptr(),
                                              self.p["pfn.shift"].data_ptr(), 32 * self.F, self.ws_slots[slot].numel(),
                                              (1 if self.split_acts else 0) | (2 if self.incremental_images else 0), _lib.stream_handle())
        _lib.check(st, "himo_pillarize_multi_ex")


def conv2d_nhwc(x: torch.Tensor, weight: torch.Tensor, bias: torch.Tensor, stride: int = 1, epilogue: int = EPI_BIAS,
                scale: torch.Tensor | None = None, shift: torch.Tensor | None = None, precision: str = "f32",
                tile_hint: int = 0, act_layout: int = 0, out: torch.Tensor | None = None) -> torch.Tensor:
    lib = _lib.load()
    n, h, w, cin = x.shape
    k, _, _, cout = weight.shape
    stuffed = bool(act_layout & ACT_STUFFED_2X)
    if stuffed:
        h, w = 2 * h, 2 * w
    ho, wo = ((h + 1) // 2, (w + 1) // 2) if stride == 2 else (h, w)
    y = torch.empty((n, ho, wo, cout), dtype=torch.float32, device=x.device) if out is None else out
    d = ConvDesc()
    d.x = x.data_ptr(); d.x_batch_stride = (h * w * cin) // (4 if stuffed else 1); d.x_pitch = cin
    d.w = weight.data_ptr(); d.bias = bias.data_ptr()
    d.scale = None if scale is None else scale.data_ptr(); d.shift = None if shift is None else shift.data_ptr()
    d.y = y.data_ptr(); d.y_batch_stride = ho * wo * cout; d.y_pitch = cout
    if k == 1:
        d.n, d.h, d.w_in = n, 1, h * w
    else:
        d.n, d.h, d.w_in = n, h, w
    d.cin, d.cout, d.ksize, d.stride, d.epilogue = cin, cout, k, stride, epilogue
    d.tile_hint = tile_hint
    d.act_layout = act_layout
    if precision in ("bf16x3", "f16x2", "bf16x2") and (stride == 1 or k == 3):
        fmt = {"bf16x3": 0, "f16x2": 1, "bf16x2": 2}[precision]
        pk = torch.empty(int(lib.himo_conv_packed_weight_bytes(k, cin, cout)), dtype=torch.uint8, device=x.device)
        _lib.check(lib.himo_conv_pack_weights_ex(weight.contiguous().data_ptr(), k, cin, cout, fmt, pk.data_ptr(), _lib.stream_handle()),
                   "himo_conv_pack_weights_ex")
        d.w_packed = pk.data_ptr(); d.packed_format = fmt
    _lib.check(lib.himo_conv2d(ctypes.byref(d), _lib.stream_handle()), "himo_conv2d")
    return y


def upsample2x_nhwc(x: torch.Tensor) -> torch.Tensor:
    lib = _lib.load()
    h, w, c = x.shape
    y = torch.empty((2 * h, 2 * w, c), dtype=torch.float32, device=x.device)
    _lib.check(lib.himo_upsample2x(x.data_ptr(), c, h, w, c, y.data_ptr(), c, _lib.stream_handle()), "himo_upsample2x")
    return y
```

include/himo_amd.h:

```cpp
#ifndef HIMO_AMD_H
#define HIMO_AMD_H

#include <stddef.h>
#include <stdint.h>

#ifdef __cplusplus
extern "C" {
#endif

#define HIMO_ABI_VERSION 1

typedef enum himo_status {
    HIMO_OK = 0,
    HIMO_ERR_INVALID_ARGUMENT = 1,
    HIMO_ERR_EMPTY_FRAME = 2,
    HIMO_ERR_WORKSPACE = 3,
    HIMO_ERR_SINGULAR_POSE = 4,
    HIMO_ERR_HIP = 5,
    HIMO_ERR_UNSUPPORTED = 6
} himo_status;

#define HIMO_FLAG_F32_CHAIN 0x1u
#define HIMO_FLAG_RAW 0x2u
#define HIMO_FLAG_SCANIA 0x4u
#define HIMO_FLAG_POSE_IS_EGO 0x8u

int himo_abi_version(void);
size_t himo_abi_sizeof(const char* struct_name);
const char* himo_status_string(int status);
const char* himo_last_hip_error(void);

void himo_prof_enable(int on);
void himo_prof_filter(const char* substr);
void himo_prof_reset(void);
size_t himo_prof_summary(char* buf, size_t cap);
int himo_mfma_sustained_tflops(int kind, int zero_operands, double min_seconds, double* tflops, void* stream);

size_t himo_compdis_workspace_bytes(int n_frames);

int himo_compdis_batch(int n_frames, int64_t total_points,
                       const int64_t* d_offsets, const double* d_pose0, const double* d_pose1,
                       const float* d_pc0, int pc_stride, const float* d_flow, const float* d_lidar_dt,
                       double sensor_dt, unsigned flags,
                       float* d_comp_dis, float* d_refined,
                       uint8_t* d_eval_mask, const uint8_t* d_gm0, const uint8_t* d_flow_is_valid,
                       const float* h_mask_bounds, float close_distance,
                       void* d_workspace, size_t workspace_bytes, void* stream);

int himo_compdis_frame(int64_t n_points, const double* h_pose0, const double* h_pose1,
                       const float* d_pc0, int pc_stride, const float* d_flow, const float* d_lidar_dt,
                       double sensor_dt, unsigned flags,
                       float* d_comp_dis, float* d_refined,
                       void* d_workspace, size_t workspace_bytes, void* stream);

#define HIMO_GT_HAS_CATEGORY 0x1u
#define HIMO_GT_HAS_INSTANCE 0x2u
#define HIMO_GT_MAX_COLUMNS 10

size_t himo_gt_body_bytes(int64_t n_points, unsigned columns);
size_t himo_gt_column_starts(int64_t n_points, unsigned columns, int64_t* h_starts);

int himo_compdis_gt_batch(int n_frames, int64_t total_points,
                          const int64_t* d_offsets, const double* d_pose0, const double* d_pose1,
                          const float* d_pc0, int pc_stride, const float* d_flow, const float* d_lidar_dt,
                          double sensor_dt, unsigned flags,
                          const uint8_t* d_gm0, const uint8_t* d_flow_is_valid,
                          const uint8_t* d_category, const uint32_t* d_instance, unsigned columns,
                          const float* h_mask_bounds, float close_distance,
                          const int64_t* d_body_offsets, uint8_t* d_body,
                          void* d_workspace, size_t workspace_bytes, void* stream);

int himo_flow2compdis(int64_t n, const void* d_flow, const void* d_dt0, double sensor_dt,
                      int dtype_flags, void* d_out, void* stream);
int himo_refine_pts(int64_t n, const float* d_pc, int pc_stride, const void* d_ds,
                    int dtype_is_f64, void* d_out, void* stream);
int himo_ego_pts_mask(int64_t n, const float* d_pts, int pc_stride, const float* h_bounds,
                      uint8_t* d_out, void* stream);
int himo_dt0(int64_t n, const float* d_lidar_dt, float* d_dt0, void* d_workspace, void* stream);

int himo_nn_search(int n_segments, const int64_t* d_q_offsets, const int64_t* d_r_offsets,
                   int64_t nq, int64_t nr, const void* d_q, const void* d_r, int dtype_is_f64,
                   void* d_dist2, int32_t* d_idx, void* stream);
int himo_sqrt_inplace(int64_t n, void* d_values, int dtype_is_f64, void* stream);

typedef struct himo_instance_record {
    int32_t frame;
    int32_t group;
    int64_t instance;
    int64_t num_pts;
    double vel;
    double dis;
    double mpe;
    double cham;
} himo_instance_record;

#define HIMO_EVAL_FLOW 0
#define HIMO_EVAL_COMPDIS 1
#define HIMO_EVAL_RAW 2
#define HIMO_EVAL_SCORE 3

#define HIMO_EVAL_DIRECT 4
#define HIMO_EVAL_DIRECT_EST_IS_DIS 0x100u

size_t himo_eval_workspace_bytes(int n_frames, int64_t total_points, int64_t max_records);

int himo_eval_instances(int n_frames, int64_t total_points,
                        const int64_t* d_offsets, const double* d_pose0, const double* d_pose1,
                        const float* d_pc0, int pc_stride, const void* d_gt, const void* d_est,
                        const float* d_lidar_dt, const uint8_t* d_category, const int64_t* d_instance,
                        const uint8_t* d_eval_mask, const uint8_t* h_class_lut,
                        double sensor_dt, int mode, unsigned flags,
                        himo_instance_record* d_records, int64_t max_records, int64_t* d_counts,
                        void* d_workspace, size_t workspace_bytes, void* stream);

#define HIMO_SEG_MAX_RESULTS 8
int himo_seg_confusion(int64_t total_points, const uint8_t* d_gt, const uint8_t* const* h_pred, int n_results,
                       const uint8_t* d_seg_valid, const uint8_t* h_class_lut, int64_t* d_conf, void* stream);

#define HIMO_FLOWM_MAX_RESULTS 8
#define HIMO_FLOWM_CLASSES 5
#define HIMO_FLOWM_BUCKETS 51
size_t himo_flow_metrics_workspace_bytes(int n_frames);
int himo_flow_metrics_batch(int n_frames, int64_t total_points, const int64_t* d_offsets,
                            const double* d_pose0, const double* d_pose1, const float* d_pc0, int pc_stride,
                            const float* d_gt, const float* const* h_est, int n_results,
                            const uint8_t* d_category, const uint8_t* d_ground, const uint8_t* d_valid,
                            const uint8_t* h_class_lut, double sensor_dt, unsigned flags,
                            int64_t* d_buckets, int64_t* d_threeway, int64_t* d_rejected,
                            void* d_workspace, void* stream);

int himo_box_label_batch(int n_frames, int64_t total_points, const int64_t* h_offsets, const int64_t* d_offsets,
                         const double* d_ego1_SE3_ego0, const float* d_pc, int n_boxes, const int* h_box_offsets,
                         const int* d_box_offsets, const double* d_box_geom, const float* d_box_flow,
                         const uint8_t* d_box_class, const uint8_t* d_box_vel_finite, int background_class,
                         float* d_flow, uint8_t* d_flow_is_valid, uint8_t* d_category, uint32_t* d_instance, void* stream);

typedef struct himo_ground_params {
    float sensor_height;
    float r_min;
    float bin_size;
    int32_t n_bins;
    int32_t K;
    float max_slope;
    float step_tol;
    float ground_thresh;
} himo_ground_params;

size_t himo_ground_seg_workspace_bytes(int n_frames, const himo_ground_params* params);
int himo_ground_seg_batch(int n_frames, int64_t total_points, const int64_t* h_offsets, const int64_t* d_offsets,
                          const float* d_xyz, int pitch, const himo_ground_params* params, uint8_t* d_mask,
                          float* d_cell_ground, void* d_workspace, size_t workspace_bytes, void* stream);

typedef struct himo_raymap_params {
    float x0, y0, z0;
    float voxel;
    float scale;
    int32_t nx, ny, nz;
    int32_t guard;
    int32_t min_votes;
} himo_raymap_params;

size_t himo_raymap_map_bytes(const himo_raymap_params* params);
int himo_raymap_carve(int64_t n_rays, const float* d_pts, int pitch, const unsigned char* d_slot, const float* d_origins,
                      const himo_raymap_params* params, uint32_t* d_map, void* stream);
int himo_raymap_query(int64_t n, const float* d_pts, int pitch, const unsigned char* d_skip, const himo_raymap_params* params,
                      const uint32_t* d_map, unsigned char* d_free_votes, unsigned char* d_hit_votes, unsigned char* d_dynamic,
                      void* stream);
int himo_raymap_status(void* stream);

typedef struct himo_camera {
    float m[12];
    int32_t ortho;
    float fx, fy, cx, cy;
    float znear, zfar;
    float inv_range;
    int32_t width, height;
} himo_camera;

typedef struct himo_shade {
    int32_t mode;
    int32_t palette_n;
    const uint32_t* rgba;
    const float* scalar;
    const int32_t* ids;
    const uint32_t* lut;
    const uint32_t* palette;
    int64_t n_attr;
    float lo, scale;
    uint32_t background, neutral;
    float edl_strength;
    int32_t edl_px;
} himo_shade;

int himo_render_clear(uint64_t* d_vis, int width, int height, void* stream);
int himo_render_splat(int64_t n, const float* d_pts, int pitch, const float* d_offset, const unsigned char* d_skip,
                      const himo_camera* cam, int radius, uint32_t index_base, uint64_t* d_vis, void* stream);
int himo_render_resolve(const uint64_t* d_vis, int width, int height, const himo_shade* shade, unsigned char* d_rgb, void* stream);

typedef struct himo_icp_params {
    float bin;
    int32_t half;
    float z_gate;
    float max_dist;
    int32_t min_inliers;
    float min_ratio;
    int32_t iters;
} himo_icp_params;

#define HIMO_ICP_ACCEPTED 0
#define HIMO_ICP_FAILED 1
#define HIMO_ICP_REJECTED 2
#define HIMO_ICP_MOVED 0
#define HIMO_ICP_FLOW 1

size_t himo_icp_workspace_bytes(int64_t n_target, int n_clusters);
int himo_icp_vote(int64_t n, const float* d_pts, int pitch, int n_clusters, const int64_t* h_offsets, const int64_t* d_offsets,
                  int64_t n_target, const float* d_target, const himo_icp_params* params, int32_t* d_counts, int32_t* d_peak,
                  double* d_transform, int32_t* d_status, void* d_workspace, size_t workspace_bytes, void* stream);
int himo_icp_step(int64_t n, const float* d_moved, int n_clusters, const int64_t* h_offsets, const int64_t* d_offsets,
                  int64_t n_target, const float* d_target, const int32_t* d_nn_idx, const float* d_nn_dist2,
                  const himo_icp_params* params, int final_pass, double* d_transform, int32_t* d_status, uint8_t* d_inlier,
                  void* d_workspace, size_t workspace_bytes, void* stream);
int himo_icp_apply(int64_t n, const float* d_pts, int pitch, const int32_t* d_labels, int n_clusters, const double* d_transform,
                   const int32_t* d_status, int mode, const float* d_base, int base_pitch, float* d_out, void* stream);

size_t himo_pillar_workspace_bytes(int64_t max_points, int grid_w, int grid_h);
int himo_pillarize(int64_t n, const float* d_pts, int pc_stride, const float* h_transform,
                   const float* h_range, const float* h_voxel, const float* h_centre_offset,
                   int grid_w, int grid_h,
                   const float* d_pfn_weight, const float* d_pfn_scale, const float* d_pfn_shift,
                   float* d_xyz_t, int32_t* d_pid, float* d_offsets, float* d_image, int image_pitch,
                   void* d_workspace, size_t workspace_bytes, void* stream);
typedef struct himo_sweep {
    int64_t n; const float* d_pts; int pc_stride;
    float transform[16];
    float* d_xyz_t; int32_t* d_pid; float* d_offsets;
    float* d_image;
    void* d_workspace;
} himo_sweep;
int himo_pillarize_multi(int n_sweeps, const himo_sweep* h_sweeps, const float* h_range, const float* h_voxel,
                         const float* h_centre_offset, int grid_w, int grid_h, const float* d_pfn_weight,
                         const float* d_pfn_scale, const float* d_pfn_shift, int image_pitch, size_t workspace_bytes,
                         void* stream);
#define HIMO_IMAGE_SPLIT 1
#define HIMO_IMAGE_INCREMENTAL 2
int himo_pillar_occupancy_reset(void* d_workspace, size_t workspace_bytes, int grid_w, int grid_h, void* stream);
int himo_pillarize_multi_ex(int n_sweeps, const himo_sweep* h_sweeps, const float* h_range, const float* h_voxel,
                         const float* h_centre_offset, int grid_w, int grid_h, const float* d_pfn_weight,
                         const float* d_pfn_scale, const float* d_pfn_shift, int image_pitch, size_t workspace_bytes, int image_split,
                         void* stream);

#define HIMO_EPI_BIAS 0
#define HIMO_EPI_BIAS_BN_GELU 1
#define HIMO_EPI_BIAS_GELU 2
#define HIMO_EPI_GRU_ZR 3
#define HIMO_EPI_GRU_Q 4
#define HIMO_EPI_BIAS_RELU 5
#define HIMO_EPI_RELU_MASK 6
typedef struct himo_conv_desc {
    const float* x; int64_t x_batch_stride; int x_pitch;
    const float* w;
    const float* bias; const float* scale; const float* shift;
    float* y; int64_t y_batch_stride; int y_pitch;
    int n, h, w_in, cin, cout, ksize, stride, epilogue;
    const float* aux_in; int aux_in_pitch;
    float* aux_out; int aux_out_pitch;
    const void* w_packed;
    int tile_hint;
    int packed_format;
    int n_outer;
    int64_t x_outer_stride, y_outer_stride;
    int act_layout;
    uint32_t* d_range_seen;
} himo_conv_desc;
#define HIMO_ACT_SPLIT_IN 1
#define HIMO_ACT_SPLIT_OUT 2
#define HIMO_ACT_ACCUMULATE 8
#define HIMO_ACT_STUFFED_2X 16
int himo_conv2d(const himo_conv_desc* h_desc, void* stream);
size_t himo_conv_packed_weight_bytes(int ksize, int cin, int cout);
int himo_conv_pack_weights(const float* d_w, int ksize, int cin, int cout, void* d_packed, void* stream);
#define HIMO_PACK_BF16X3 0
#define HIMO_PACK_F16X2 1
#define HIMO_PACK_BF16X2 2
int himo_conv_pack_weights_ex(const float* d_w, int ksize, int cin, int cout, int format, void* d_packed, void* stream);

int himo_upsample2x(const float* d_x, int x_pitch, int h, int w, int c, float* d_y, int y_pitch, void* stream);
int himo_upsample2x_batch(int n, const float* d_x, int64_t x_batch_stride, int x_pitch, int h, int w, int c, float* d_y,
                          int64_t y_batch_stride, int y_pitch, void* stream);
int himo_upsample2x_batch_ex(int n, const float* d_x, int64_t x_batch_stride, int x_pitch, int h, int w, int c, float* d_y,
                             int64_t y_batch_stride, int y_pitch, int out_split, void* stream);

#define HIMO_OP_CONV 0
#define HIMO_OP_UPSAMPLE2X 1
#define HIMO_OPS_GRAPH 0x1u
typedef struct himo_op {
    int kind;
    himo_conv_desc conv;
    const float* up_x; int up_x_pitch, up_h, up_w, up_c;
    float* up_y; int up_y_pitch;
    int up_n; int64_t up_x_batch_stride, up_y_batch_stride;
    int up_out_split;
} himo_op;
int himo_run_ops(const himo_op* h_ops, int n_ops, unsigned flags, void* stream);
void himo_ops_release(const himo_op* h_ops);

int himo_gru_head(int64_t n, const int32_t* d_pid, const float* d_offsets, const float* d_img0, const float* d_img1,
                  int img_pitch, const float* d_dec, int dec_pitch, const float* d_w_off, const float* d_b_off,
                  const void* d_wzr_packed, const float* d_bzr, const void* d_wq_packed, const float* d_bq,
                  const void* d_w1_packed, const float* d_b1, const float* d_w2, const float* d_b2,
                  const float* d_xyz_t, const float* d_pts, int pc_stride, float* d_flow, int iters, int packed_format,
                  void* stream);
typedef struct himo_head_sample {
    int64_t n;
    const int32_t* d_pid; const float* d_offsets; const float* d_img0; const float* d_img1; const float* d_dec;
    const float* d_xyz_t; const float* d_pts; int pc_stride; float* d_flow;
} himo_head_sample;
int himo_gru_head_batch(int n_samples, const himo_head_sample* h_samples, int img_pitch, int dec_pitch,
                        const float* d_w_off, const float* d_b_off,
                        const void* d_wzr_packed, const float* d_bzr, const void* d_wq_packed, const float* d_bq,
                        const void* d_w1_packed, const float* d_b1, const float* d_w2, const float* d_b2,
                        int iters, int packed_format, int img_split, void* stream);
int himo_gru_head_batch_folded(int n_samples, const himo_head_sample* h_samples, int img_pitch, int dec_pitch,
                               const void* d_wzr_packed, const float* d_bzr, const void* d_wq_packed, const float* d_bq,
                               const void* d_w1_packed, const float* d_b1, const float* d_w2, const float* d_b2,
                               int iters, int packed_format, int img_split, void* stream);
int himo_gru_head_batch_guarded(int n_samples, const himo_head_sample* h_samples, int img_pitch, int dec_pitch,
                                const float* d_w_off, const float* d_b_off,
                                const void* d_wzr_packed, const float* d_bzr, const void* d_wq_packed, const float* d_bq,
                                const void* d_w1_packed, const float* d_b1, const float* d_w2, const float* d_b2,
                                int iters, int packed_format, int img_split, uint32_t* d_nonfinite, void* stream);
typedef struct himo_head_saved {
    int64_t rows;
    float* d_hx;
    float* d_rhx;
    float* d_z; float* d_r; float* d_q;
    float* d_pre1; float* d_y1;
    float* d_res;
} himo_head_saved;
int himo_gru_head_train(int64_t n, const int32_t* d_pid, const float* d_offsets, const float* d_img0, const float* d_img1,
                        int img_pitch, const float* d_dec, int dec_pitch, const float* d_w_off, const float* d_b_off,
                        const void* d_wzr_packed, const float* d_bzr, const void* d_wq_packed, const float* d_bq,
                        const void* d_w1_packed, const float* d_b1, const float* d_w2, int w2_pitch, const float* d_b2,
                        int iters, int packed_format, const himo_head_saved* h_saved, uint32_t* d_nonfinite, void* stream);
int himo_gru_head_backward(int64_t n, int iters, const float* d_dhx_last, const himo_head_saved* h_saved,
                           const void* d_wq_t_packed, const void* d_wzr_t_packed, int packed_format, float* d_daq,
                           float* d_dazr, float* d_dhx0, void* stream);
int himo_clear_u32(uint32_t* d_words, int n, void* stream);

int himo_head_gather(int64_t n, const int32_t* d_pid, const float* d_offsets, const float* d_img0,
                     const float* d_img1, int img_pitch, const float* d_dec, int dec_pitch,
                     const float* d_w_off, const float* d_b_off, float* d_hx, float* d_rhx, int pitch, void* stream);
int himo_head_final(int64_t n, const float* d_y1, int y1_pitch, const float* d_w2, const float* d_b2,
                    const int32_t* d_pid, const float* d_xyz_t, const float* d_pts, int pc_stride,
                    float* d_flow, void* stream);

size_t himo_nn_grid_workspace_bytes(int64_t n_max, int grid_w, int grid_h);
int himo_nn_grid(int64_t nq, const float* d_q, int64_t nr, const float* d_r, float x0, float y0, float cell,
                 int grid_w, int grid_h, float* d_dist2, int32_t* d_idx, void* d_workspace,
                 size_t workspace_bytes, void* stream);
size_t himo_ssl_loss_workspace_bytes(int n0, int n1, int n_labels, int grid_w, int grid_h);
int himo_ssl_loss(int n0, int n1, const float* d_pc0, const float* d_pc1, const float* d_flow,
                  const int32_t* d_label0, const int32_t* d_label1, int n_labels,
                  float grid_x0, float grid_y0, float grid_cell, int grid_w, int grid_h,
                  double* d_loss, float* d_grad_flow, void* d_workspace, size_t workspace_bytes, void* stream);
int himo_ssl_loss_ex(int n0, int n1, const float* d_pc0, const float* d_pc1, const float* d_flow,
                     const int32_t* d_label0, const int32_t* d_label1, int n_labels,
                     float grid_x0, float grid_y0, float grid_cell, int grid_w, int grid_h,
                     const float* d_raw_dist2, const int32_t* d_raw_idx,
                     double* d_loss, float* d_grad_flow, void* d_workspace, size_t workspace_bytes, void* stream);
int himo_ssl_dyn_sizes(int n0, const int32_t* d_label0, int n1, const int32_t* d_label1, int32_t* d_counts, void* stream);
int himo_ssl_loss_presized(int n0, int n1, const float* d_pc0, const float* d_pc1, const float* d_flow,
                           const int32_t* d_label0, const int32_t* d_label1, int n_labels,
                           float grid_x0, float grid_y0, float grid_cell, int grid_w, int grid_h,
                           const float* d_raw_dist2, const int32_t* d_raw_idx, int n_dyn0, int n_dyn1,
                           double* d_loss, float* d_grad_flow, void* d_workspace, size_t workspace_bytes, void* stream);

size_t himo_deflow_loss_workspace_bytes(int64_t n);
int himo_deflow_loss(int64_t n, const float* d_pc0, int pc0_pitch, const float* d_moved, const float* d_gt,
                     const float* d_est, int est_pitch, const int32_t* d_pid ,
                     const uint8_t* d_valid , float sensor_dt, double* d_loss ,
                     int64_t* d_counts , float* d_grad , void* d_workspace, size_t workspace_bytes,
                     void* stream);

size_t himo_wgrad_workspace_bytes(int64_t n_rows);
int himo_linear_wgrad(int64_t n, const float* d_x, int x_pitch, int cin, const float* d_dz, int z_pitch, int cout,
                      float* d_dw, float* d_db, void* d_workspace, size_t workspace_bytes, void* stream);
size_t himo_wgrad_workspace_bytes_ex(int64_t n_rows, int cin, int cout);
int himo_linear_wgrad_ex(int64_t n, const float* d_x, int x_pitch, int cin, const float* d_dz, int z_pitch, int cout,
                         float* d_dw, float* d_db, unsigned flags, void* d_workspace, size_t workspace_bytes, void* stream);
int himo_transpose(const float* d_w, int rows, int cols, float* d_wt, void* stream);
int himo_adam_step(int64_t n, float* d_param, const float* d_grad, float* d_m, float* d_v, float lr, float beta1,
                   float beta2, float eps, int step, void* stream);
size_t himo_chamfer_trunc_workspace_bytes(int n0, int n1);
int himo_chamfer_trunc(int n0, int n1, const float* d_moved, const float* d_pc1, const float* d_dist_a,
                       const int32_t* d_idx_a, const float* d_dist_b, const int32_t* d_idx_b, float trunc_dist,
                       double* d_loss, float* d_grad_moved, void* d_workspace, size_t workspace_bytes, void* stream);
int himo_rows_add(int64_t n, int cols, const float* d_a, int a_pitch, const float* d_b, int b_pitch, float b_scale,
                  float* d_y, int y_pitch, int zero_tail, void* stream);
int himo_rigid_transform(int64_t n, const float* d_pts, int pc_stride, const float* d_transform, float* d_out,
                         int out_pitch, void* stream);

int himo_gru_gates_fwd(int64_t n, int which, const float* d_pre, const float* d_z_in, const float* d_hx,
                       float* d_z, float* d_r, float* d_q, float* d_out, void* stream);
int himo_gru_bwd1(int64_t n, const float* d_dh_next, const float* d_z, const float* d_q, const float* d_hx,
                  float* d_daq, float* d_dz, float* d_dhp, void* stream);
int himo_gru_bwd2(int64_t n, const float* d_d_rhx, const float* d_hx, const float* d_z, const float* d_r,
                  const float* d_dz, float* d_dhp, float* d_dazr, float* d_dx, void* stream);
int himo_gru_bwd3(int64_t n, const float* d_d_hx, const float* d_dhp, float* d_dh, float* d_dx, void* stream);
int himo_affine_gelu_fwd(int64_t rows, int ch, const float* d_x, int x_pitch, const float* d_scale, const float* d_shift,
                         float* d_pre, int pre_pitch, float* d_y, int y_pitch, void* stream);
int himo_affine_gelu_bwd(int64_t rows, int ch, const float* d_dy, int dy_pitch, const float* d_pre, int pre_pitch,
                         const float* d_scale, float* d_dx, int dx_pitch, void* stream);
int himo_mask_rows(int64_t n, int cols, const int32_t* d_pid, float* d_v, int pitch, void* stream);
int himo_weight_flip(const float* d_w, int ksize, int cin, int cout, float* d_wf, void* stream);
int himo_zero_stuff2x(int n_img, int h, int w, int c, const float* d_dy, int64_t dy_batch_stride, int dy_pitch,
                      float* d_z, int64_t z_batch_stride, int z_pitch, void* stream);
int himo_upsample2x_bwd(const float* d_dy, int dy_pitch, int h, int w, int c, float* d_dx, int dx_pitch, void* stream);
int himo_add2d(int64_t rows, int cols, const float* d_b, int b_pitch, float* d_y, int y_pitch, void* stream);
int himo_colsum(int64_t n, const float* d_z, int z_pitch, int cout, float* d_out, unsigned flags, void* d_workspace,
                size_t workspace_bytes, void* stream);
size_t himo_pfn_backward_workspace_bytes(void);
int himo_pfn_backward(int64_t n, const float* h_voxel, const float* h_centre_offset, int grid_w, int grid_h,
                      const float* d_pfn_weight, const float* d_pfn_scale, const float* d_pfn_shift,
                      const float* d_xyz_t, const void* d_pillar_workspace, const float* d_dimage, int image_pitch,
                      float* d_dweight, unsigned flags, void* d_workspace, size_t workspace_bytes, void* stream);
int himo_head_scatter(int64_t n, int grid_w, int grid_h, const void* d_pillar_workspace, const float* d_dhx, int dhx_pitch,
                      float* d_db0, int b0_pitch, int group0, int group1, int n_groups, float* d_ddec, int dec_pitch,
                      void* stream);

typedef struct himo_weight_job {
    const float* w;
    void* packed;
    int ksize, cin, cout;
    int format;
    int flip;
    int first_block;
} himo_weight_job;
int himo_weight_job_blocks(int ksize, int cin, int cout, int flip);
int himo_weight_prepare_batch(const himo_weight_job* d_jobs, int n_jobs, int total_blocks, void* stream);

int himo_mlp_repack(int n_layers, const float* const* h_w, const int* h_cin, const int* h_cout, void* const* h_fwd_packed,
                    void* const* h_bwd_packed, void* stream);

size_t himo_dbscan_workspace_bytes(int n, int grid_w, int grid_h);
int himo_dbscan(int n, const float* d_xyz, int pitch, const unsigned char* d_skip, float eps, int min_pts, float x0, float y0, float cell,
                int grid_w, int grid_h, int32_t* d_labels, int32_t* d_n_clusters, void* d_workspace, size_t workspace_bytes, void* stream);

int64_t himo_nsf_padded_rows(int64_t n);
size_t himo_nsf_spill_bytes(int64_t n, int n_hidden);
int himo_nsf_backward_blocks(int64_t n);
int himo_nsf_forward(int64_t n, const float* d_x0, int n_hidden, const float* d_w_first, const float* d_b_first,
                     const void* const* h_w_hidden_packed, const float* const* h_b_hidden, const float* d_w_last, const float* d_b_last,
                     void* d_spill, float* d_out, const float* h_origin, float cell, const int* h_dims, int window, const void* d_volume,
                     float trunc_dist, float* d_dout, double* d_loss_partial, int* d_count_partial, void* stream);
int himo_nsf_backward(int64_t n, const float* d_x0, const float* d_dout, int n_hidden, const void* const* h_wT_hidden_packed,
                      const float* d_w_last, const void* d_spill, const int* h_off_w, const int* h_off_b, int64_t partial_stride,
                      float* d_partial, void* stream);
int himo_nsf_update(int total, int n_partials, int64_t partial_stride, const float* d_partial, int n_fwd_blocks,
                    const double* d_loss_partial, const int* d_count_partial, float* d_param, float* d_grad, float* d_m, float* d_v,
                    float lr, float beta1, float beta2, float eps, int step, int n_hidden, const int* h_off_w, void* const* h_fwd_packed,
                    void* const* h_bwd_packed, double* d_loss, int* d_count, void* stream);

int himo_nsf_forward_keep(int64_t n, const float* d_x0, int n_hidden, const float* d_w_first, const float* d_b_first,
                          const void* const* h_w_hidden_packed, const float* const* h_b_hidden, const float* d_w_last,
                          const float* d_b_last, void* d_spill, float* d_out, void* stream);
int himo_nsf_last_grad(int64_t n, int n_hidden, const float* d_dout, void* d_spill, void* stream);
size_t himo_nsfp_workspace_bytes(int64_t n0, int64_t n1, int grid_w, int grid_h);
int64_t himo_nsfp_partials(int64_t n0, int64_t n1);
int himo_nsfp_prepare(int64_t n0, int64_t n1, const float* d_pc1, float x0, float y0, float cell, int grid_w, int grid_h,
                      void* d_workspace, size_t workspace_bytes, void* stream);
int himo_nsfp_objective(int64_t n0, int64_t n1, const float* d_x0, const float* d_out, const float* d_pc1, float x0, float y0,
                        float cell, int grid_w, int grid_h, float trunc_dist, float* d_moved, float* d_dist_a, int32_t* d_idx_a,
                        float* d_dist_b, int32_t* d_idx_b, float* d_dout, double* d_loss_partial, int* d_count_partial,
                        void* d_workspace, size_t workspace_bytes, void* stream);
int himo_nsfp_keep_best(int64_t n, const float* d_out, float* d_best_out, const double* d_loss, double* d_state, int step,
                        int patience, double min_delta, void* stream);

int himo_mlp_forward_fused(int64_t n, const float* d_x0, int n_hidden, const float* d_w_first, const float* d_b_first,
                           const void* const* h_w_hidden_packed, const float* const* h_b_hidden, const float* d_w_last,
                           const float* d_b_last, float* const* h_H, float* d_out, void* stream);
int himo_mlp_backward_fused(int64_t n, const float* d_dout, int n_hidden, const void* const* h_wT_hidden_packed,
                            const float* d_w_last, float* const* h_H, float* const* h_dZ, void* stream);
size_t himo_mlp_bias_workspace_bytes(int64_t n, int n_hidden);
int himo_mlp_backward_fused_bias(int64_t n, const float* d_dout, int n_hidden, const void* const* h_wT_hidden_packed,
                                 const float* d_w_last, float* const* h_H, float* const* h_dZ, float* const* h_db,
                                 void* d_workspace, size_t workspace_bytes, void* stream);

size_t himo_dt_volume_bytes(const int* h_dims);
int himo_dt_build(int n1, const float* d_pc1, const float* h_origin, float cell, const int* h_dims, int window,
                  void* d_volume, size_t volume_bytes, void* stream);
size_t himo_dt_loss_workspace_bytes(int n);
int himo_dt_loss(int n, const float* d_moved, const float* h_origin, float cell, const int* h_dims, int window,
                 const void* d_volume, float trunc_dist, double* d_loss, float* d_grad_moved, void* d_workspace,
                 size_t workspace_bytes, void* stream);

size_t himo_bn_workspace_bytes(int64_t total_rows, int ch);
int himo_bn_train_fwd(int n_img, int64_t rows, int ch, const float* d_x, int64_t x_img_stride, int x_pitch,
                      const float* d_gamma, const float* d_beta, float eps, float momentum, float* d_running_mean,
                      float* d_running_var, float* d_mean, float* d_invstd, float* d_xhat, int64_t xhat_img_stride, int xhat_pitch,
                      float* d_y, int64_t y_img_stride, int y_pitch, void* d_workspace, size_t workspace_bytes, void* stream);
int himo_bn_train_bwd(int n_img, int64_t rows, int ch, const float* d_dy, int64_t dy_img_stride, int dy_pitch,
                      const float* d_xhat, int64_t xhat_img_stride, int xhat_pitch, const float* d_gamma, const float* d_beta,
                      const float* d_invstd, float* d_dx, int64_t dx_img_stride, int dx_pitch, float* d_dgamma, float* d_dbeta,
                      unsigned flags, void* d_workspace, size_t workspace_bytes, void* stream);
int himo_bn_train_bwd_x(int n_img, int64_t rows, int ch, const float* d_dy, int64_t dy_img_stride, int dy_pitch,
                        const float* d_x, int64_t x_img_stride, int x_pitch, const float* d_gamma, const float* d_beta,
                        const float* d_mean, const float* d_invstd, float* d_dx, int64_t dx_img_stride, int dx_pitch,
                        float* d_dgamma, float* d_dbeta, unsigned flags, void* d_workspace, size_t workspace_bytes, void* stream);
int himo_bn_fold(int ch, const float* d_gamma, const float* d_beta, const float* d_mean, const float* d_var, float eps,
                 float* d_scale, float* d_shift, void* stream);
size_t himo_pfn_bn_workspace_bytes(void);
int himo_pfn_bn_stats_groups(int n_sweeps, int n_groups, const int64_t* h_n, const float* const* h_xyz_t,
                             const void* const* h_pillar_workspace, const float* h_voxel, const float* h_centre_offset, int grid_w,
                             int grid_h, const float* d_pfn_weight, const float* d_gamma, const float* d_beta, float eps, float momentum,
                             float* d_running_mean, float* d_running_var, float* d_scale, float* d_shift, float* d_mean, float* d_invstd,
                             void* d_workspace, size_t workspace_bytes, void* stream);
int himo_pfn_backward_bn_groups(int n_sweeps, int n_groups, const int64_t* h_n, const float* const* h_xyz_t,
                                const void* const* h_pillar_workspace, const float* const* h_dimage, int image_pitch, const float* h_voxel,
                                const float* h_centre_offset, int grid_w, int grid_h, const float* d_pfn_weight, const float* d_scale,
                                const float* d_shift, const float* d_mean, const float* d_invstd, float* d_dweight, float* d_dgamma,
                                float* d_dbeta, unsigned flags, void* d_workspace, size_t workspace_bytes, void* stream);
int himo_pfn_bn_stats_multi(int n_sweeps, const int64_t* h_n, const float* const* h_xyz_t, const void* const* h_pillar_workspace,
                            const float* h_voxel, const float* h_centre_offset, int grid_w, int grid_h,
                            const float* d_pfn_weight, const float* d_gamma, const float* d_beta, float eps, float momentum,
                            float* d_running_mean, float* d_running_var, float* d_scale, float* d_shift, float* d_mean,
                            float* d_invstd, void* d_workspace, size_t workspace_bytes, void* stream);
int himo_pfn_backward_bn_multi(int n_sweeps, const int64_t* h_n, const float* const* h_xyz_t, const void* const* h_pillar_workspace,
                               const float* const* h_dimage, int image_pitch, const float* h_voxel, const float* h_centre_offset,
                               int grid_w, int grid_h, const float* d_pfn_weight, const float* d_scale, const float* d_shift,
                               const float* d_mean, const float* d_invstd, float* d_dweight, float* d_dgamma, float* d_dbeta,
                               unsigned flags, void* d_workspace, size_t workspace_bytes, void* stream);
int himo_pfn_bn_stats(int64_t n, const float* h_voxel, const float* h_centre_offset, int grid_w, int grid_h,
                      const float* d_pfn_weight, const float* d_xyz_t, const void* d_pillar_workspace, const float* d_gamma,
                      const float* d_beta, float eps, float momentum, float* d_running_mean, float* d_running_var,
                      float* d_scale, float* d_shift, float* d_mean, float* d_invstd, void* d_workspace, size_t workspace_bytes,
                      void* stream);
int himo_pillar_features_multi(int n_sweeps, const himo_sweep* h_sweeps, const float* h_range, const float* h_voxel,
                               const float* h_centre_offset, int grid_w, int grid_h, const float* d_pfn_weight,
                               const float* d_scale, const float* d_shift, int image_pitch, size_t workspace_bytes,
                               int image_split, void* stream);
int himo_pfn_backward_bn(int64_t n, const float* h_voxel, const float* h_centre_offset, int grid_w, int grid_h,
                         const float* d_pfn_weight, const float* d_scale, const float* d_shift, const float* d_mean,
                         const float* d_invstd, const float* d_xyz_t, const void* d_pillar_workspace, const float* d_dimage,
                         int image_pitch, float* d_dweight, float* d_dgamma, float* d_dbeta, unsigned flags, void* d_workspace,
                         size_t workspace_bytes, void* stream);
size_t himo_conv_wgrad_batch_workspace_bytes(int n_img, int h, int w, int cin, int cout, int stride);
int himo_conv3x3_wgrad_batch(int n_img, const float* d_x, int64_t x_batch_stride, int x_pitch, int h, int w, int cin,
                             const float* d_dy, int64_t dy_batch_stride, int dy_pitch, int cout, int stride, float* d_dw,
                             unsigned flags, void* d_workspace, size_t workspace_bytes, void* stream);
int himo_conv3x3_wgrad_batch_bias(int n_img, const float* d_x, int64_t x_batch_stride, int x_pitch, int h, int w, int cin,
                                  const float* d_dy, int64_t dy_batch_stride, int dy_pitch, int cout, int stride, float* d_dw,
                                  float* d_db, unsigned flags, void* d_workspace, size_t workspace_bytes, void* stream);
size_t himo_conv_wgrad_workspace_bytes(int ho, int wo, int cin, int cout);
int himo_conv3x3_wgrad(const float* d_x, int x_pitch, int h, int w, int cin, const float* d_dy, int dy_pitch, int cout,
                       int stride, float* d_dw, unsigned flags, void* d_workspace, size_t workspace_bytes, void* stream);

int64_t himo_lz4_frame_decompress(const void* h_src, int64_t n, void* h_dst, int64_t capacity);

#ifdef __cplusplus
}
#endif
#endif
```

Before: 736.5 frames/s.

## Compute final decoder conv only at occupied pillar cells via occupancy mask

The pillariser now writes a per-cell occupancy bitmask for the head frame slot. A new masked 3x3 conv kernel reads that mask per 8x32 tile, compacts the occupied pixels into a list, and runs MFMA only on those pixels. Tiles with no occupied cells exit early. The final decoder conv (dec4) is routed to this kernel by default in f16x2 mode, so the dense full-grid 512x512 conv work is skipped for empty cells. DEC becomes undefined at unoccupied cells, which is safe only if the head samples it at occupied pillars of that slot. A guard enforces the slot.

Measured after the change: 747.4 frames/s (median of 6 runs). 1.5% higher.

```diff
diff --git a/himo_amd/csrc/conv_common.h b/himo_amd/csrc/conv_common.h
--- a/himo_amd/csrc/conv_common.h
+++ b/himo_amd/csrc/conv_common.h
@@ -29,8 +29,10 @@
     float* aux_out; int aux_out_pitch;
     int act_flags;
     unsigned* range_seen;
+    const unsigned long long* mask;
+    int64_t mask_batch_stride, mask_outer_stride;
 };
-enum ActFlags { kActSplitIn = 1, kActSplitOut = 2, kActVecStore = 4, kActAccumulate = 8, kActStuffedIn = 16 };
+enum ActFlags { kActSplitIn = 1, kActSplitOut = 2, kActVecStore = 4, kActAccumulate = 8, kActStuffedIn = 16, kActRowMask = 32 };
 
 __device__ inline int64_t image_offset(int img, int n_inner, int64_t batch_stride, int64_t outer_stride) {
     return (int64_t)(img % n_inner) * batch_stride + (int64_t)(img / n_inner) * outer_stride;
diff --git a/himo_amd/csrc/conv_plan.h b/himo_amd/csrc/conv_plan.h
--- a/himo_amd/csrc/conv_plan.h
+++ b/himo_amd/csrc/conv_plan.h
@@ -87,6 +87,12 @@
 inline int plan_presplit(ConvPlan& p, int rows_hint) {
     ConvArgs& a = p.args;
     if (!below_2gb((int64_t)a.H * a.W, a.x_pitch)) return HIMO_ERR_UNSUPPORTED;
+    if (a.act_flags & kActRowMask) {
+        p.family = kConvPresplit3;
+        p.prof_name = "conv3x3_masked_f16x2_kernel";
+        plan_rows_tile(p, 4, 2, 2);
+        return HIMO_OK;
+    }
     const bool wide = a.Cout > 64, vec = vec_store_ok(a), pinned = rows_hint == 4 || rows_hint == 2 || rows_hint == 1;
     const int ph = wide ? 1 : 2;
     p.family = p.ks == 1 ? kConvPresplit1 : kConvPresplit3;
@@ -139,6 +145,14 @@
     a.act_flags = d.act_layout;
     a.range_seen = (d.act_layout & kActSplitOut) ? d.d_range_seen : nullptr;
 
+    if (d.act_layout & kActRowMask) {
+        if (!d.d_mask || (reinterpret_cast<uintptr_t>(d.d_mask) & 7u)) return HIMO_ERR_INVALID_ARGUMENT;
+        if (d.act_layout != (kActRowMask | kActSplitIn) || !d.w_packed || d.packed_format != 1 || d.ksize != 3 || d.stride != 1 ||
+            d.cout > 64 || (d.w_in & 31) || (d.epilogue != kEpiBias && d.epilogue != kEpiBiasBnGelu) || (d.cin & 15) || (d.x_pitch & 15))
+            return HIMO_ERR_UNSUPPORTED;
+        a.mask = reinterpret_cast<const unsigned long long*>(d.d_mask);
+        a.mask_batch_stride = d.mask_batch_stride; a.mask_outer_stride = d.mask_outer_stride;
+    }
     const bool gemm_acc = d.act_layout == kActAccumulate && d.w_packed && d.ksize == 1 && d.epilogue == kEpiBias && (d.packed_format == 0 || d.packed_format == 2);
     if (d.act_layout & (kActAccumulate | kActStuffedIn)) {
         if (!gemm_acc && ((d.act_layout & ~(kActAccumulate | kActStuffedIn)) || !d.w_packed || d.packed_format != 2 || d.ksize != 3 ||
@@ -146,7 +160,7 @@
             return HIMO_ERR_UNSUPPORTED;
         if ((d.act_layout & kActStuffedIn) && ((d.h & 1) || (d.w_in & 1) || !below_2gb((int64_t)(d.h / 2) * (d.w_in / 2), d.x_pitch)))
             return HIMO_ERR_UNSUPPORTED;
-    } else if (d.act_layout) {
+    } else if (d.act_layout && !(d.act_layout & kActRowMask)) {
         if ((d.act_layout & ~(kActSplitIn | kActSplitOut)) || !d.w_packed || d.packed_format != 1) return HIMO_ERR_UNSUPPORTED;
         if (d.ksize == 1 && !(d.act_layout & kActSplitIn)) return HIMO_ERR_UNSUPPORTED;
         if (d.epilogue != kEpiBias && d.epilogue != kEpiBiasBnGelu) return HIMO_ERR_UNSUPPORTED;
diff --git a/himo_amd/csrc/convsg.hip b/himo_amd/csrc/convsg.hip
--- a/himo_amd/csrc/convsg.hip
+++ b/himo_amd/csrc/convsg.hip
@@ -1,5 +1,6 @@
 #include "conv_plan.h"
 #include "bf16x3.h"
+#include <type_traits>
 
 namespace himo {
 
@@ -186,6 +187,204 @@
     }
 }
 
+template <int EPI>
+__global__ __launch_bounds__(256, 3)
+void conv3_rowmask_kernel(ConvArgs a, const unsigned short* __restrict__ wpk) {
+    constexpr int TW = 32, TH = 8, PHt = TH + 2, PWP = 40;
+    constexpr int kRow = PWP * 64, kBuf = (PHt * kRow + 1023) / 1024 * 1024;
+    static_assert(PHt * PWP == 25 * 16 && kBuf == 25 * 1024, "25 DMA units of 16 slots fill a patch buffer exactly");
+    __shared__ __attribute__((aligned(1024))) unsigned char patch[2 * kBuf];
+    __shared__ __attribute__((aligned(16))) unsigned char s_list[TH * TW];
+
+    const int tile = xcd_block_id(blockIdx.x, gridDim.x);
+    int bid = tile;
+    const int tx = a.Wo / TW, ty = (a.Ho + TH - 1) / TH;
+    const int ox0 = __builtin_amdgcn_readfirstlane((bid % tx) * TW); bid /= tx;
+    const int oy0 = __builtin_amdgcn_readfirstlane((bid % ty) * TH);
+    const int img = __builtin_amdgcn_readfirstlane(bid / ty);
+    const int wave = __builtin_amdgcn_readfirstlane(threadIdx.x >> 6), lane = threadIdx.x & 63;
+    const int li = lane & 31, lh = lane >> 5;
+
+    const unsigned* __restrict__ mrow = reinterpret_cast<const unsigned*>(a.mask + image_offset(img, a.n_inner, a.mask_batch_stride, a.mask_outer_stride));
+    unsigned mine = 0u;
+    if (lane < TH && oy0 + lane < a.Ho) mine = mrow[((unsigned)(oy0 + lane) * (unsigned)a.Wo + (unsigned)ox0) >> 5];
+    int n_occ = 0, before = 0;
+#pragma unroll
+    for (int i = 0; i < TH; ++i) {
+        const int c = __builtin_popcount(__builtin_amdgcn_readlane(mine, i));
+        n_occ += c;
+        before += i < 2 * wave ? c : 0;
+    }
+    if (n_occ == 0) return;
+    {
+        const unsigned r0 = __builtin_amdgcn_readlane(mine, 2 * wave), r1 = __builtin_amdgcn_readlane(mine, 2 * wave + 1);
+        const unsigned bits = lh ? r1 : r0, below = (1u << li) - 1u;
+        if ((bits >> li) & 1u) s_list[before + (lh ? __builtin_popcount(r0) : 0) + __builtin_popcount(bits & below)] = (unsigned char)threadIdx.x;
+    }
+    const int role = (wave + tile) & 3, ct = role & 1;
+    const int n_frag = (n_occ + 31) >> 5;
+    const int half = (n_frag + 1) >> 1, n0 = n_frag < 2 ? n_frag : (half > 2 ? half : 2);
+    const int first = (role >> 1) ? n0 : 0;
+    const int mine_n = ct * 32 < a.Cout ? ((role >> 1) ? n_frag - n0 : n0) : 0;
+
+    const unsigned char* __restrict__ xin = reinterpret_cast<const unsigned char*>(a.x + image_offset(img, a.n_inner, a.x_batch_stride, a.x_outer_stride));
+    const int slabs = a.Cin >> 4;
+    const int iy0 = oy0 - 1, ix0 = ox0 - 1;
+    const unsigned lds_base = (unsigned)(uintptr_t)(__attribute__((address_space(3))) unsigned char*)(&patch[0]);
+
+    unsigned offA, offB, vm = 0u;
+    const unsigned rs2 = (unsigned)(2 * a.W) * (unsigned)a.x_pitch * 4u;
+    {
+        const int q = wave * 16 + (lane >> 2), row = q / PWP, px = q - row * PWP, ix = ix0 + px;
+        const bool col_ok = px < TW + 2 && ix >= 0 && ix < a.W;
+        offA = (((unsigned)((iy0 + row) * a.W + ix) * (unsigned)a.x_pitch) << 2) | (unsigned)(((lane & 3) ^ ((px >> 2) & 3)) << 4);
+#pragma unroll
+        for (int j = 0; j < 5; ++j) vm |= (col_ok && iy0 + row + 2 * j >= 0 && iy0 + row + 2 * j < a.H) ? 1u << j : 0u;
+    }
+    {
+        const int q = 4 * 16 + (lane >> 2), row = q / PWP + 2 * wave, px = q % PWP, ix = ix0 + px;
+        const bool col_ok = px < TW + 2 && ix >= 0 && ix < a.W;
+        offB = (((unsigned)((iy0 + row) * a.W + ix) * (unsigned)a.x_pitch) << 2) | (unsigned)(((lane & 3) ^ ((px >> 2) & 3)) << 4);
+        vm |= (col_ok && iy0 + row >= 0 && iy0 + row < a.H) ? 1u << 5 : 0u;
+        vm |= (wave == 0 && col_ok && iy0 + row + 8 >= 0 && iy0 + row + 8 < a.H) ? 1u << 6 : 0u;
+    }
+    auto stage = [&](int slab, int buf) {
+        int ln = threadIdx.x;
+        unsigned oa = offA, ob = offB, m = vm;
+        asm volatile("" : "+v"(ln), "+v"(oa), "+v"(ob), "+v"(m));
+        const unsigned char* zero = g_zero_page + (ln & 3) * 16;
+        const unsigned dst = lds_base + buf * kBuf;
+#pragma unroll
+        for (int j = 0; j < 5; ++j)
+            glds16((m >> j) & 1u ? xin + (oa + j * rs2 + (unsigned)slab * 64u) : zero, dst + (wave + 5 * j) * 1024);
+        glds16((m >> 5) & 1u ? xin + (ob + (unsigned)slab * 64u) : zero, dst + (4 + 5 * wave) * 1024);
+        if (wave == 0) glds16((m >> 6) & 1u ? xin + (ob + 4 * rs2 + (unsigned)slab * 64u) : zero, dst + 24 * 1024);
+    };
+    stage(0, 0);
+    __syncthreads();
+
+    if (mine_n <= 0) {
+        asm volatile("s_waitcnt vmcnt(0)" ::: "memory");
+        __syncthreads();
+#pragma unroll 1
+        for (int slab = 0; slab + 1 < slabs; ++slab) {
+            stage(slab + 1, (slab & 1) ^ 1);
+            asm volatile("s_waitcnt vmcnt(0)" ::: "memory");
+            __syncthreads();
+        }
+        return;
+    }
+
+    const unsigned char* __restrict__ wb = reinterpret_cast<const unsigned char*>(wpk);
+    unsigned b_lane;
+    {
+        const int c = ct * 32 + li < a.Cout ? ct * 32 + li : a.Cout - 1;
+        b_lane = (unsigned)c * 32u + (unsigned)lh * 16u;
+        asm volatile("" : "+v"(b_lane));
+    }
+    const unsigned b_plane = (unsigned)a.Cout * 32u, b_block = 2u * b_plane;
+    auto load_b = [&](int tap, int slab, uint4 (&b)[2]) {
+        const unsigned off = (unsigned)(tap * slabs + slab) * b_block + b_lane;
+        b[0] = *reinterpret_cast<const uint4*>(wb + off);
+        b[1] = *reinterpret_cast<const uint4*>(wb + (off + b_plane));
+    };
+    float* __restrict__ yout = a.y + image_offset(img, a.n_inner, a.y_batch_stride, a.y_outer_stride);
+
+    auto run = [&](auto miw) {
+        constexpr int MIW = decltype(miw)::value;
+        int rd[MIW][3];
+        int lw = threadIdx.x;
+        asm volatile("" : "+v"(lw) :: "memory");
+        const int li = lw & 31, lh = (lw >> 5) & 1;
+#pragma unroll
+        for (int mi = 0; mi < MIW; ++mi) {
+            const int e = (first + mi) * 32 + li;
+            int pxl = s_list[e < n_occ ? e : n_occ - 1];
+            asm volatile("" : "+v"(pxl));
+            const int r = pxl >> 5, c = pxl & 31;
+#pragma unroll
+            for (int kx = 0; kx < 3; ++kx) {
+                const int p = c + kx, f = (p >> 2) & 3;
+                rd[mi][kx] = r * kRow + p * 64 + ((lh ^ f) << 4);
+                asm volatile("" : "+v"(rd[mi][kx]));
+            }
+        }
+        floatx16 acc[MIW];
+#pragma unroll
+        for (int mi = 0; mi < MIW; ++mi)
+#pragma unroll
+            for (int r = 0; r < 16; ++r) acc[mi][r] = 0.f;
+
+        uint4 bq[3][2];
+        load_b(0, 0, bq[0]);
+        load_b(1, 0, bq[1]);
+        asm volatile("s_waitcnt vmcnt(0)" ::: "memory");
+        __syncthreads();
+
+#pragma unroll 1
+        for (int slab = 0; slab < slabs; ++slab) {
+            const int buf = slab & 1;
+            const bool more = slab + 1 < slabs;
+            const int nslab = more ? slab + 1 : slab;
+            if (more) stage(slab + 1, buf ^ 1);
+#pragma unroll 1
+            for (int ky = 0; ky < 3; ++ky) {
+                const int rowoff = buf * kBuf + ky * kRow;
+#pragma unroll
+                for (int kx = 0; kx < 3; ++kx) {
+                    const int tap = ky * 3 + kx;
+                    const int t2 = tap + 2;
+                    load_b(t2 < 9 ? t2 : t2 - 9, t2 < 9 ? slab : nslab, bq[(kx + 2) % 3]);
+                    f16x8 af[MIW][2];
+#pragma unroll
+                    for (int s = 0; s < 2; ++s)
+#pragma unroll
+                        for (int mi = 0; mi < MIW; ++mi)
+                            af[mi][s] = *reinterpret_cast<const f16x8*>(&patch[(rd[mi][kx] ^ (s << 5)) + rowoff]);
+                    const uint4 (&bcur)[2] = bq[kx];
+#define HIMO_TERM16(SA, SB)                                                                                        \
+    _Pragma("unroll") for (int mi = 0; mi < MIW; ++mi)                                                               \
+        acc[mi] = __builtin_amdgcn_mfma_f32_32x32x16_f16(af[mi][SA], __builtin_bit_cast(f16x8, bcur[SB]), acc[mi], 0, 0, 0);
+                    { HIMO_TERM16(1, 0) HIMO_TERM16(0, 1) HIMO_TERM16(0, 0) }
+#undef HIMO_TERM16
+                    __builtin_amdgcn_sched_group_barrier(0x020, 2, 0);
+                    __builtin_amdgcn_sched_group_barrier(0x100, MIW * 2, 0);
+                    __builtin_amdgcn_sched_group_barrier(0x008, MIW * 3, 0);
+                }
+            }
+            if (more) {
+                asm volatile("s_waitcnt vmcnt(4)" ::: "memory");
+                __syncthreads();
+            }
+        }
+
+        int ln = threadIdx.x;
+        asm volatile("" : "+v"(ln));
+        const int co = ct * 32 + (ln & 31), lhe = (ln >> 5) & 1;
+        const int cl = co < a.Cout ? co : a.Cout - 1;
+        float eA, eB;
+        epi_affine<EPI>(kF16AccScale, a.bias ? a.bias[cl] : 0.f, EPI == kEpiBiasBnGelu ? a.scale[cl] : 1.f, EPI == kEpiBiasBnGelu ? a.shift[cl] : 0.f, eA, eB);
+#pragma unroll
+        for (int mi = 0; mi < MIW; ++mi) {
+            const int e0 = (first + mi) * 32 + 4 * lhe;
+#pragma unroll
+            for (int g = 0; g < 4; ++g) {
+                const unsigned four = *reinterpret_cast<const unsigned*>(&s_list[e0 + 8 * g]);
+#pragma unroll
+                for (int j = 0; j < 4; ++j) {
+                    const int pxl = (four >> (8 * j)) & 255;
+                    if (e0 + 8 * g + j < n_occ && co < a.Cout)
+                        yout[((int64_t)(oy0 + (pxl >> 5)) * a.Wo + (ox0 + (pxl & 31))) * a.y_pitch + co] = epi_activate<EPI>(acc[mi][4 * g + j], eA, eB);
+                }
+            }
+        }
+    };
+    if (mine_n == 1) { run(std::integral_constant<int, 1>{}); return; }
+    if (mine_n == 2) { run(std::integral_constant<int, 2>{}); return; }
+    if (mine_n == 3) { run(std::integral_constant<int, 3>{}); return; }
+    run(std::integral_constant<int, 4>{});
+}
+
 template <int EPI, int PH, int MI, bool OSPLIT>
 __global__ __launch_bounds__(256, 4)
 void conv1_presplit_kernel(ConvArgs a, const unsigned short* __restrict__ wpk) {
@@ -350,6 +549,11 @@
 }
 
 void launch_conv_presplit3(const ConvPlan& p, hipStream_t s) {
+    if (p.args.act_flags & kActRowMask) {
+        if (p.epi == kEpiBias) hipLaunchKernelGGL((conv3_rowmask_kernel<kEpiBias>), p.grid, dim3(256), 0, s, p.args, (const unsigned short*)p.w_packed);
+        else hipLaunchKernelGGL((conv3_rowmask_kernel<kEpiBiasBnGelu>), p.grid, dim3(256), 0, s, p.args, (const unsigned short*)p.w_packed);
+        return;
+    }
     if (p.stride == 2) { if (p.ph == 1) launch_sg<1, 2, 2>(p, s); else launch_sg<2, 1, 2>(p, s); }
     else if (p.nt == 2) {
         if (p.ph == 4) launch_sg<4, 2, 1, 2>(p, s);
diff --git a/himo_amd/csrc/pillar.hip b/himo_amd/csrc/pillar.hip
--- a/himo_amd/csrc/pillar.hip
+++ b/himo_amd/csrc/pillar.hip
@@ -32,6 +32,7 @@
     int* order2;
     float4* cell_rec;
     unsigned long long* occ;
+    unsigned long long* occ_out;
 };
 
 constexpr int kMaxSweeps = 12;
@@ -152,7 +153,11 @@
         const unsigned long long below = (1ull << threadIdx.x) - 1ull;
         if (cnt == 1) s_list[__popcll(one & below)] = threadIdx.x;
         if (cnt > 1) s_list[__popcll(one) + __popcll(many & below)] = threadIdx.x;
-        if (threadIdx.x == 0) { s_nlist = __popcll(one | many); if (a.occ) a.occ[blockIdx.x] = one | many; }
+        if (threadIdx.x == 0) {
+            s_nlist = __popcll(one | many);
+            if (a.occ) a.occ[blockIdx.x] = one | many;
+            if (a.occ_out) a.occ_out[blockIdx.x] = one | many;
+        }
     }
 #pragma unroll
     for (int i = 0; i < kFeatCells / 32; ++i) {
@@ -585,6 +590,7 @@
     if (image_split && (image_pitch & 15)) return HIMO_ERR_INVALID_ARGUMENT;
     for (int i = 0; i < n_sweeps; ++i) {
         if (image_split && (reinterpret_cast<uintptr_t>(h_sweeps[i].d_image) & 63)) return HIMO_ERR_INVALID_ARGUMENT;
+        if (reinterpret_cast<uintptr_t>(h_sweeps[i].d_occupancy) & 7) return HIMO_ERR_INVALID_ARGUMENT;
         for (int j = 0; check_shared && j < i; ++j)
             if (h_sweeps[j].d_workspace == h_sweeps[i].d_workspace) return HIMO_ERR_INVALID_ARGUMENT;
     }
@@ -664,6 +670,7 @@
                                    w.d_workspace, workspace_bytes, incremental);
         if (st != HIMO_OK) return st;
         m.s[i].image_split = image_split ? 1 : 0;
+        m.s[i].occ_out = reinterpret_cast<unsigned long long*>(w.d_occupancy);
     }
     return pillar_launch(m, n_sweeps, (hipStream_t)stream);
 }
@@ -810,6 +817,7 @@
                                    w.d_workspace, workspace_bytes, incremental);
         if (st != HIMO_OK) return st;
         m.s[i].image_split = image_split ? 1 : 0;
+        m.s[i].occ_out = reinterpret_cast<unsigned long long*>(w.d_occupancy);
     }
     hipStream_t s = (hipStream_t)stream;
     const int cells = grid_w * grid_h;
diff --git a/himo_amd/pipeline.py b/himo_amd/pipeline.py
--- a/himo_amd/pipeline.py
+++ b/himo_amd/pipeline.py
@@ -38,6 +38,7 @@
         self.auto = net is None and precision == "auto"
         self._net_args = dict(params=params, device=self.device, max_points=max_points, max_batch=max_batch)
         self.net = net if net is not None else SeFlowNet(precision="f16x2" if self.auto else precision, **self._net_args)
+        self._set_sparse_dec4()
         self.compdis = CompDisEngine(device=self.device)
         self._batch = None
         self._bufs, self._turn = {}, 0
@@ -97,8 +98,14 @@
             grp = samples[lo:lo + mb]
             self.net.forward_batch([(s.pch1, s.pc0, s.pc1, s.pose_h1, s.pose0, s.pose1) for s in grp], outs[lo:lo + mb])
 
+    def _set_sparse_dec4(self):
+        net = self.net
+        if hasattr(net, "sparse_dec4"):
+            net.sparse_dec4 = bool(net.precision == "f16x2" and net.fused_head and net.split_acts)
+
     def _fall_back(self):
         self.net = SeFlowNet(precision="bf16x3", **self._net_args)
+        self._set_sparse_dec4()
 
     def _guard_begin(self):
         if self.net.precision == "f16x2":
diff --git a/himo_amd/seflow/model.py b/himo_amd/seflow/model.py
--- a/himo_amd/seflow/model.py
+++ b/himo_amd/seflow/model.py
@@ -21,10 +21,12 @@
                 ("aux_out", ctypes.c_void_p), ("aux_out_pitch", ctypes.c_int), ("w_packed", ctypes.c_void_p),
                 ("tile_hint", ctypes.c_int), ("packed_format", ctypes.c_int),
                 ("n_outer", ctypes.c_int), ("x_outer_stride", ctypes.c_int64), ("y_outer_stride", ctypes.c_int64),
-                ("act_layout", ctypes.c_int), ("range_seen", ctypes.c_void_p)]
+                ("act_layout", ctypes.c_int), ("range_seen", ctypes.c_void_p),
+                ("mask", ctypes.c_void_p), ("mask_batch_stride", ctypes.c_int64), ("mask_outer_stride", ctypes.c_int64)]
 
 
 ACT_SPLIT_IN, ACT_SPLIT_OUT = 1, 2
+ACT_ROW_MASK = 32
 ACT_ACCUMULATE = 8
 ACT_STUFFED_2X = 16
 
@@ -77,7 +79,7 @@
 class HimoSweep(ctypes.Structure):
     _fields_ = [("n", ctypes.c_int64), ("d_pts", ctypes.c_void_p), ("pc_stride", ctypes.c_int), ("transform", ctypes.c_float * 16),
                 ("d_xyz_t", ctypes.c_void_p), ("d_pid", ctypes.c_void_p), ("d_offsets", ctypes.c_void_p), ("d_image", ctypes.c_void_p),
-                ("d_workspace", ctypes.c_void_p)]
+                ("d_workspace", ctypes.c_void_p), ("d_occupancy", ctypes.c_void_p)]
 
 
 class HimoOp(ctypes.Structure):
@@ -145,6 +147,7 @@
         self._nb = 1
         self.packed_format = 1 if precision == "f16x2" else 0
         self._split_acts = precision == "f16x2"
+        self._sparse_dec4 = False
         self.tiles = {}
         self.lib = _lib.load()
         self.device = device if device is not None else _lib.require_gpu()
@@ -219,6 +222,7 @@
         self.CAT3 = buf(H * W, 128)
         self.U = [buf(H * W, 64) for _ in range(2)]
         self.DEC = buf(H * W, 64)
+        self.occ0 = torch.zeros((B, (H * W + 63) // 64), dtype=torch.int64, device=dev)
         self.max_points = 0
         self._reserve_points(max_points)
         self.guard = torch.zeros(2 + self.MAX_RANGE_SLOTS, dtype=torch.int32, device=dev)
@@ -270,8 +274,25 @@
         on = bool(on)
         if on != self._split_acts:
             self._split_acts = on
+            if not on:
+                self._sparse_dec4 = False
             self.drop_plan()
             self.reset_images()
+
+    HEAD_SLOT = 1
+
+    @property
+    def sparse_dec4(self) -> bool:
+        return self._sparse_dec4
+
+    @sparse_dec4.setter
+    def sparse_dec4(self, on: bool):
+        on = bool(on)
+        if on and not (self.packed_format == 1 and self._split_acts and self.fused_head):
+            raise ValueError("sparse_dec4 needs precision='f16x2' with split activations and the fused head")
+        if on != self._sparse_dec4:
+            self._sparse_dec4 = on
+            self.drop_plan()
 
     @property
     def B0(self):
@@ -315,7 +336,7 @@
 
     def _conv(self, x, x_bs, x_pitch, wname, y, y_bs, y_pitch, n, h, w, cin, cout, ks, stride, epi, x_off=0, y_off=0,
               scale=None, shift=None, aux_in=None, aux_in_pitch=0, aux_out=None, aux_out_pitch=0, bias=None, batched=True,
-              act=0):
+              act=0, mask=None):
         d = ConvDesc()
         d.x = x.data_ptr() + 4 * x_off; d.x_batch_stride = x_bs; d.x_pitch = x_pitch
         if batched and self._nb > 1:
@@ -332,6 +353,9 @@
         d.w_packed = None if pk is None else pk.data_ptr()
         d.packed_format = self.packed_format
         d.act_layout = act if self.split_acts else 0
+        if mask is not None:
+            d.act_layout |= ACT_ROW_MASK
+            d.mask, d.mask_batch_stride, d.mask_outer_stride = mask.data_ptr(), 0, mask.stride(0)
         if (d.act_layout & ACT_SPLIT_OUT) and self.packed_format == 1 and epi in (EPI_BIAS, EPI_BIAS_BN_GELU):
             d.range_seen = self._range_word(wname)
         key = (n * max(d.n_outer, 1), h, w, cin, cout, ks, stride, epi, pk is not None, d.act_layout)
@@ -344,7 +368,7 @@
         _lib.check(self.lib.himo_conv2d(ctypes.byref(d), _lib.stream_handle()), f"himo_conv2d({wname})")
 
     def _tune(self, d: "ConvDesc") -> int:
-        if d.epilogue in (EPI_GRU_ZR, EPI_GRU_Q):
+        if d.epilogue in (EPI_GRU_ZR, EPI_GRU_Q) or (d.act_layout & ACT_ROW_MASK):
             return 0
         cands = [(bn << 4) | mi for bn in (128, 64) if not (bn == 128 and d.cout % 128) for mi in (2, 1)]
         if d.act_layout:
@@ -442,7 +466,8 @@
         s = block("dec1", self.F3, 256 * F, H // 8, W // 8, self.T1, self.CAT1, self.F2, 128 * F, 256, 256, self.S, ("dec2", self.T2, 128))
         t = block("dec2", s, 256, H // 4, W // 4, self.T2, self.CAT2, self.F1, 64 * F, 128, 128, self.T, ("dec3", self.T3, 64))
         u = block("dec3", t, 128, H // 2, W // 2, self.T3, self.CAT3, self.B0, 32 * F, 64, 64, self.U)
-        self._conv(u, 0, 64, "dec4", self.DEC, 0, 64, 1, H, W, 64, 64, 3, 1, EPI_BIAS, act=IN)
+        self._conv(u, 0, 64, "dec4", self.DEC, 0, 64, 1, H, W, 64, 64, 3, 1, EPI_BIAS, act=IN,
+                   mask=self.occ0 if self._sparse_dec4 else None)
         return self.DEC
 
     def head(self, pc0: torch.Tensor, slot0: int = 1, slot1: int = 2, out: torch.Tensor | None = None) -> torch.Tensor:
@@ -514,6 +539,8 @@
 
     def head_batch(self, pc0s, outs, slot0: int = 1, slot1: int = 2, samples=None) -> None:
         p, pk, F = self.p, self.packed, self.F
+        if self._sparse_dec4 and slot0 != self.HEAD_SLOT:
+            raise ValueError("sparse_dec4: DEC is defined at the cells of frame slot HEAD_SLOT only")
         samples = list(range(len(pc0s))) if samples is None else list(samples)
         for lo in range(0, len(pc0s), self.MAX_HEAD_SAMPLES):
             grp = range(lo, min(lo + self.MAX_HEAD_SAMPLES, len(pc0s)))
@@ -566,6 +593,7 @@
                     w.d_xyz_t, w.d_pid, w.d_offsets = st["xyz_t"][slot].data_ptr(), st["pid"][slot].data_ptr(), st["offsets"][slot].data_ptr()
                     w.d_image = self.B0[sample].data_ptr() + 4 * 32 * slot
                     w.d_workspace = st["ws_slots"][slot].data_ptr()
+                    w.d_occupancy = self.occ0[sample].data_ptr() if slot == self.HEAD_SLOT else None
             status = self.lib.himo_pillarize_multi_ex(len(arr), ctypes.addressof(arr), self._range, self._voxel, self._centre, self.W, self.H,
                                                       self.p["pfn.weight"].data_ptr(), self.p["pfn.scale"].data_ptr(),
                                                       self.p["pfn.shift"].data_ptr(), 32 * self.F, self._pt[0]["ws_slots"][0].numel(),
@@ -598,6 +626,7 @@
         w.d_xyz_t, w.d_pid, w.d_offsets = self.xyz_t[slot].data_ptr(), self.pid[slot].data_ptr(), self.offsets[slot].data_ptr()
         w.d_image = self.B0[self._sample].data_ptr() + 4 * 32 * slot
         w.d_workspace = self.ws_slots[slot].data_ptr()
+        w.d_occupancy = self.occ0[self._sample].data_ptr() if slot == self.HEAD_SLOT else None
         st = self.lib.himo_pillarize_multi_ex(1, ctypes.addressof(arr), self._range, self._voxel, self._centre, self.W, self.H,
                                               self.p["pfn.weight"].data_ptr(), self.p["pfn.scale"].data_ptr(),
                                               self.p["pfn.shift"].data_ptr(), 32 * self.F, self.ws_slots[slot].numel(),
diff --git a/include/himo_amd.h b/include/himo_amd.h
--- a/include/himo_amd.h
+++ b/include/himo_amd.h
@@ -237,6 +237,7 @@
     float* d_xyz_t; int32_t* d_pid; float* d_offsets;
     float* d_image;
     void* d_workspace;
+    uint64_t* d_occupancy;
 } himo_sweep;
 int himo_pillarize_multi(int n_sweeps, const himo_sweep* h_sweeps, const float* h_range, const float* h_voxel,
                          const float* h_centre_offset, int grid_w, int grid_h, const float* d_pfn_weight,
@@ -272,9 +273,12 @@
     int64_t x_outer_stride, y_outer_stride;
     int act_layout;
     uint32_t* d_range_seen;
+    const uint64_t* d_mask;
+    int64_t mask_batch_stride, mask_outer_stride;
 } himo_conv_desc;
 #define HIMO_ACT_SPLIT_IN 1
 #define HIMO_ACT_SPLIT_OUT 2
+#define HIMO_ACT_ROW_MASK 32
 #define HIMO_ACT_ACCUMULATE 8
 #define HIMO_ACT_STUFFED_2X 16
 int himo_conv2d(const himo_conv_desc* h_desc, void* stream);
```
